# QuentinFuxa/WhisperLiveKit

Hardware: AMD Instinct MI355X
Metric: audio seconds transcribed per second (1/RTF), Whisper-base EN simul_whisper AlignAtt, 0.5 s chunks (higher is better)
Workload: dtype f32; 1 GPU; base.en simul_whisper, 1 stream(s) over 1 GPU(s) (1 per GPU), 30 s 16 kHz speech-like stream, 0.5 s chunks, beam 1, frame_threshold 25, seeded random weights, synthetic vocabulary; model=base.en, streams_total=1

## Files before the change

whisperlivekit_amd/csrc/api.hip:

```cpp
#include <cmath>
#include <cstdio>
#include <cstdlib>
#include <atomic>
#include <chrono>
#include <cstring>
#include <map>
#include <memory>
#include <mutex>
#include <string>
#include <vector>

#include "../../include/wlk_hip.h"
#include "common.h"
#include "internal.h"

namespace wlk {

namespace {
struct UtilStream {
    std::mutex mu;
    hipStream_t stream = nullptr;
};
UtilStream g_util[64];
UtilStream& util_of_current_device() {
// ... 284 lines not shown
        for (int i = 0; i < m->D.n_audio_layer; ++i) m->enc_layers.push_back(layer_weights(m, "enc", i, false));
        for (int i = 0; i < m->D.n_text_layer; ++i) m->dec_layers.push_back(layer_weights(m, "dec", i, true));
        {
            const size_t d = m->D.n_text_state, da = m->D.n_audio_state, Ld = m->D.n_text_layer;
            if (!m->xkv_all_w) m->xkv_all_w = dev_alloc<float>(Ld * 2 * d * da);
            if (!m->xkv_all_b) m->xkv_all_b = dev_alloc<float>(Ld * 2 * d);
            for (size_t i = 0; i < Ld; ++i) {
                copy_sync(m->xkv_all_w + i * 2 * d * da, m->dec_layers[i].xkvw, 2 * d * da * sizeof(float),
                                  hipMemcpyDeviceToDevice);
                copy_sync(m->xkv_all_b + i * 2 * d, m->dec_layers[i].xkvb, 2 * d * sizeof(float),
                                  hipMemcpyDeviceToDevice);
            }
        }
        {
            for (unsigned short* p : m->x3_owned) (void)hipFree(p);
            m->x3_owned.clear();
            m->xkv_all_w3 = nullptr;
            const int da = m->D.n_audio_state, T = m->D.n_audio_ctx;
            LaunchCtx c;
            c.stream = nullptr;
            hipStream_t st;
            WLK_HIP(hipStreamCreateWithFlags(&st, hipStreamNonBlocking));
            struct StreamGuard {
                hipStream_t s;
                ~StreamGuard() { (void)hipStreamDestroy(s); }
            } st_guard{st};
            c.stream = st;
            auto pack = [&](const float* w, int n_rows, int k = 0) -> unsigned short* {
                if (k == 0) k = da;
                unsigned short* p3 = dev_alloc<unsigned short>(x3_w_elems(n_rows, k));
                m->x3_owned.push_back(p3);
                launch_x3_pack_w(c, w, k, p3, n_rows, k);
                return p3;
            };
            static const bool narrow = [] { const char* e = getenv("WLK_X3_NARROW"); return !(e && e[0] == '0'); }();
            for (auto& L : m->enc_layers) {
                L.qkvw3 = gemm_x3_wide_applicable(T, 3 * da, da, da) ? pack(L.qkvw, 3 * da) : nullptr;
                L.fc1w3 = gemm_x3_wide_applicable(T, 4 * da, da, da) ? pack(L.fc1w, 4 * da) : nullptr;
                L.outw3 = narrow && gemm_x3_wide_applicable(T, da, da, da) ? pack(L.outw, da) : nullptr;
                L.fc2w3 = narrow && gemm_x3_wide_applicable(T, da, 4 * da, 4 * da) ? pack(L.fc2w, da, 4 * da) : nullptr;
            }
            const int n_xkv = m->D.n_text_layer * 2 * m->D.n_text_state;
            if (gemm_x3_wide_applicable(T, n_xkv, da, da)) m->xkv_all_w3 = pack(m->xkv_all_w, n_xkv);
            WLK_HIP(hipStreamSynchronize(st));
        }
        m->w_tok_emb = m->w("dec.tok_emb");
        m->w_dec_pos = m->w("dec.pos");
        m->w_ln_w = m->w("dec.ln.w");
        m->w_ln_b = m->w("dec.ln.b");
        m->finalized = true;
        return WLK_OK;
    });
}

int wlk_model_destroy(wlk_model* m) {
    if (!m) return WLK_OK;
    wlk_engine_destroy_for_model(m);
    (void)hipSetDevice(m->device);
    if (m->owns_arena) (void)hipFree(m->arena);
    if (m->xkv_all_w) (void)hipFree(m->xkv_all_w);
    if (m->xkv_all_b) (void)hipFree(m->xkv_all_b);
    for (unsigned short* p : m->x3_owned) (void)hipFree(p);
    (void)hipFree(m->twiddle);
    (void)hipFree(m->filt_lo);
    (void)hipFree(m->filt_hi);
    (void)hipFree(m->head_rank);
    (void)hipFree(m->layer_heads);
    (void)hipFree(m->layer_ranks);
    (void)hipFree(m->all_ranks);
    delete m;
    return WLK_OK;
}

int wlk_session_create(wlk_model* m, int beam, int max_audio_samples, wlk_session** out) {
    if (!m || !out) return fail(WLK_ERR_ARG, "NULL argument");
    if (!m->finalized) return fail(WLK_ERR_STATE, "model not finalized");
    if (beam < 1 || beam > 7) return fail(WLK_ERR_ARG, "beam must be in [1, 7]");
    if (max_audio_samples < kHop) return fail(WLK_ERR_ARG, "max_audio_samples too small");
    return guarded([&]() {
        WLK_HIP(hipSetDevice(m->device));
        auto s = std::make_unique<wlk_session>();
        s->m = m;
        s->beam = beam;
        s->audio_cap = max_audio_samples;
        WLK_HIP(hipStreamCreateWithFlags(&s->stream, hipStreamNonBlocking));
        if (const char* e = std::getenv("WLK_NO_GRAPH")) s->use_graph = !(e[0] == '1');
        hipStream_t st = s->stream;
        const wlk_dims& D = m->D;
        const size_t d = D.n_audio_state, T = D.n_audio_ctx, ctx = D.n_text_ctx, V = D.n_vocab;
        s->audio[0] = dev_alloc_zero<float>(s->audio_cap, st);
        s->audio[1] = dev_alloc_zero<float>(s->audio_cap, st);
        s->frame_cap = s->audio_cap / kHop + 4;
        s->logmel = dev_alloc<float>((size_t)s->frame_cap * D.n_mels);
        s->frame_max = dev_alloc<float>(s->frame_cap);
        s->logmel_alt = dev_alloc<float>((size_t)s->frame_cap * D.n_mels);
        s->frame_max_alt = dev_alloc<float>(s->frame_cap);
        if (const char* e = std::getenv("WLK_MEL_INCREMENTAL")) s->mel_incremental = !(e[0] == '0');
        s->mel_t = dev_alloc_zero<float>((size_t)(kMelFrames + 2) * D.n_mels, st);
        s->x1p = dev_alloc_zero<float>((size_t)(kMelFrames + 1) * d, st);
        s->ex = dev_alloc<float>(T * d);
        s->eh = dev_alloc<float>(T * d);
        s->eqkv = dev_alloc<float>(T * 3 * d);
        s->eatt = dev_alloc<float>(T * d);
        s->emlp = dev_alloc<float>(T * 4 * d);
        s->enc_out = dev_alloc<float>(T * d);
        {
            bool any_x3 = m->xkv_all_w3 != nullptr, qkv_x3 = false;
            bool fc2_x3 = false;
            for (const auto& L : m->enc_layers) {
                any_x3 |= L.qkvw3 || L.fc1w3 || L.outw3;
                qkv_x3 |= L.qkvw3 != nullptr;
                fc2_x3 |= L.fc2w3 != nullptr;
            }
            if (fc2_x3) s->emlp3 = dev_alloc<unsigned short>(T * 3 * 4 * d);
            const bool attn_x3 = qkv_x3 && enc_attention_x3_enabled() && d == (size_t)D.n_audio_head * 64 && T >= 64 && (2 * d) % 128 == 0;
            if (any_x3) s->eh3 = dev_alloc<unsigned short>(T * 3 * d);
            if (attn_x3) s->eqkv3 = dev_alloc_zero<unsigned short>(x3_attn_image_elems((int)T, (int)d), st);
            if (m->xkv_all_w3) s->enc_out3 = dev_alloc<unsigned short>(T * 3 * d);
        }
        s->cross_kv = dev_alloc<float>((size_t)D.n_text_layer * T * 2 * d);

        s->max_rows = beam * (int)ctx;
        const size_t R = s->max_rows;
        s->step_in = dev_alloc<int>(3 * R + 4);
        s->tokens_dev = s->step_in;
        s->dx = dev_alloc<float>(R * d);
        s->dh = dev_alloc<float>(R * d);
        s->dqkv = dev_alloc<float>(R * 3 * d);
        s->datt = dev_alloc<float>(R * d);
        s->dq = dev_alloc<float>(R * d);
        s->dmlp = dev_alloc<float>(R * 4 * d);
        const size_t cache = (size_t)D.n_text_layer * beam * ctx * d;
        s->kcache[0] = dev_alloc<float>(cache);
        s->vcache[0] = dev_alloc<float>(cache);
        s->hsel = dev_alloc<float>((size_t)2 * beam * d);
        s->logits_last = dev_alloc<float>((size_t)2 * beam * V);
        s->logits_sot = s->logits_last + (size_t)beam * V;
        s->ring_row = s->step_in + R;
        s->beam_of_row = s->step_in + 2 * R;
        s->d_offset = s->step_in + 3 * R;
        s->ring_rows = (int)ctx + kAlignWindow;
        if (m->n_align > 0) s->ring = dev_alloc<float>((size_t)m->n_align * beam * s->ring_rows * T);
        s->xsplit = dev_alloc<float>(cross_split_scratch_floats(8, D.n_text_head, (int)T));
        s->fsplit = dev_alloc<float>(flash_split_scratch_floats(s->max_rows, D.n_text_head, wlk_session::kFlashSplitsMax));
        s->z = dev_alloc<float>((size_t)beam * std::max(m->n_align, 1) * T + (size_t)beam * 128);
        s->attn_last = dev_alloc_zero<float>((size_t)beam * T, st);
        s->adj_row = dev_alloc<int>(3 * wlk_session::kAdjCap);
        s->src_rows = dev_alloc<int>(8);
        if (beam >= 2 && beam <= 7) s->anc = dev_alloc_zero<unsigned char>((size_t)beam * ctx, st);
        s->top_vals = dev_alloc<float>((size_t)beam * 18);
        s->top_ids = reinterpret_cast<int*>(s->top_vals) + (size_t)beam * 8;
        s->frames = s->top_ids + (size_t)beam * 8;
        WLK_HIP(hipMalloc(&s->topk_scratch, topk_scratch_bytes(beam)));
        s->probs = dev_alloc<float>(beam);
        WLK_HIP(hipHostMalloc(&s->pinned, wlk_session::kPinnedBytes, hipHostMallocDefault));
        WLK_HIP(hipHostMalloc(&s->dec_stage, 65536, hipHostMallocDefault));
        WLK_HIP(hipHostMalloc(&s->audio_stage, wlk_session::kPinnedBytes, hipHostMallocDefault));
        WLK_HIP(hipEventCreateWithFlags(&s->audio_stage_ev, hipEventDisableTiming));
        WLK_HIP(hipEventCreateWithFlags(&s->dec_stage_ev, hipEventDisableTiming));
        if (beam == 1) {
            void* hp = nullptr;
            WLK_HIP(hipHostMalloc(&hp, 4096, hipHostMallocMapped | hipHostMallocCoherent));
            std::memset(hp, 0, 4096);
            s->step_host = static_cast<StepBlock*>(hp);
            s->result_host = reinterpret_cast<StepResult*>(static_cast<char*>(hp) + 2048);
            void* dp = nullptr;
            WLK_HIP(hipHostGetDevicePointer(&dp, hp, 0));
            s->step_host_dev = static_cast<StepBlock*>(dp);
            s->result_host_dev = reinterpret_cast<StepResult*>(static_cast<char*>(dp) + 2048);
            s->step_dev = reinterpret_cast<StepBlock*>(dev_alloc<int>(sizeof(StepBlock) / 4));
        }
        WLK_HIP(hipStreamSynchronize(st));
        *out = s.release();
        return WLK_OK;
    });
}

int wlk_session_destroy(wlk_session* s) {
    if (!s) return WLK_OK;
    if (s->step_count && getenv("WLK_STEP_TIMING"))
        fprintf(stderr, "[wlk] one-replay steps: %llu, mean %.1f us per step (graph launch call %.1f us)\n",
                (unsigned long long)s->step_count, s->step_ns / 1e3 / s->step_count, s->step_launch_ns / 1e3 / s->step_count);
    (void)wlk_engine_detach(s);
    (void)hipSetDevice(s->m->device);
    (void)hipStreamSynchronize(s->stream);
    float* fl[] = {s->audio[0], s->audio[1], s->logmel, s->frame_max, s->logmel_alt, s->frame_max_alt, s->mel_t, s->x1p, s->ex, s->eh, s->eqkv,
                   s->eatt, s->emlp, s->enc_out, s->cross_kv, s->dx, s->dh, s->dqkv, s->datt, s->dq, s->dmlp,
                   s->kcache[0], s->kcache[1], s->vcache[0], s->vcache[1], s->hsel, s->logits_last,
                   s->ring, s->z, s->attn_last, s->qk_debug, s->xsplit, s->fsplit, s->top_vals, s->probs};
    for (float* p : fl)
        if (p) (void)hipFree(p);
    int* il[] = {s->step_in, s->adj_row, s->src_rows};
    for (int* p : il)
        if (p) (void)hipFree(p);
    for (auto& e : s->step_exec)
        if (e) (void)hipGraphExecDestroy(e);
    for (auto& e : s->bstep_exec)
        if (e) (void)hipGraphExecDestroy(e);
    if (s->anc) (void)hipFree(s->anc);
    if (s->topk_scratch) (void)hipFree(s->topk_scratch);
    if (s->pcm16_dev) (void)hipFree(s->pcm16_dev);
    if (s->eh3) (void)hipFree(s->eh3);
    if (s->eqkv3) (void)hipFree(s->eqkv3);
    if (s->enc_out3) (void)hipFree(s->enc_out3);
    if (s->emlp3) (void)hipFree(s->emlp3);
    if (s->wa_buf) (void)hipFree(s->wa_buf);
    if (s->pinned) (void)hipHostFree(s->pinned);
    if (s->dec_stage) (void)hipHostFree(s->dec_stage);
    if (s->audio_stage) (void)hipHostFree(s->audio_stage);
    if (s->rules_mask) (void)hipFree(s->rules_mask);
    if (s->pick_out) (void)hipFree(s->pick_out);
    if (s->audio_stage_ev) (void)hipEventDestroy(s->audio_stage_ev);
    if (s->dec_stage_ev) (void)hipEventDestroy(s->dec_stage_ev);
    if (s->step_host) (void)hipHostFree(s->step_host);
    if (s->step_dev) (void)hipFree(s->step_dev);
    if (s->step_align_dev) (void)hipFree(s->step_align_dev);
    for (auto& e : s->fstep_exec)
        if (e) (void)hipGraphExecDestroy(e);
    for (auto& r : s->prof.recs) {
        (void)hipEventDestroy(r.a);
        (void)hipEventDestroy(r.b);
    }
    for (auto e : s->prof.pool) (void)hipEventDestroy(e);
    (void)hipStreamDestroy(s->stream);
    delete s;
    return WLK_OK;
}

int wlk_session_set_debug(wlk_session* s, int on) {
    if (!s) return fail(WLK_ERR_ARG, "session is NULL");
    return guarded([&]() {
        WLK_HIP(hipSetDevice(s->m->device));
        s->debug = on != 0;
        if (s->debug && !s->qk_debug) {
            const wlk_dims& D = s->m->D;
            s->qk_debug = dev_alloc<float>((size_t)D.n_text_layer * s->max_rows * D.n_text_head * D.n_audio_ctx);
        }
        return WLK_OK;
    });
}

static bool drain_staging() {
    static const bool on = [] {
        const char* e = getenv("WLK_DRAIN_STAGING");
        return e && e[0] == '1';
    }();
    return on;
}

int wlk_audio_append(wlk_session* s, const float* pcm_host, int n) {
    if (!s || (n > 0 && !pcm_host) || n < 0) return fail(WLK_ERR_ARG, "bad audio chunk");
    if (s->audio_len + n > s->audio_cap)
        return fail(WLK_ERR_CAPACITY, "audio buffer capacity exceeded (" + std::to_string(s->audio_len + n) + " > " +
                                          std::to_string(s->audio_cap) + " samples)");
    if (n == 0) return WLK_OK;
    return guarded([&]() {
        WLK_HIP(hipSetDevice(s->m->device));
        float* dst = s->audio[s->audio_cur] + s->audio_len;
        size_t done = 0;
        while (done < (size_t)n) {
            const size_t chunk = std::min((size_t)n - done, wlk_session::kPinnedBytes / sizeof(float));
            if (s->audio_stage_used) WLK_HIP(hipEventSynchronize(s->audio_stage_ev));
            std::memcpy(s->audio_stage, pcm_host + done, chunk * sizeof(float));
            WLK_HIP(hipMemcpyAsync(dst + done, s->audio_stage, chunk * sizeof(float), hipMemcpyHostToDevice, s->stream));
            WLK_HIP(hipEventRecord(s->audio_stage_ev, s->stream));
            s->audio_stage_used = true;
            done += chunk;
        }
        if (drain_staging()) WLK_HIP(hipStreamSynchronize(s->stream));
        s->audio_len += n;
        s->encoded = false;
        return WLK_OK;
    });
}

int wlk_audio_append_pcm16(wlk_session* s, const int16_t* pcm_host, int n) {
    if (!s || (n > 0 && !pcm_host) || n < 0) return fail(WLK_ERR_ARG, "bad audio chunk");
    if (s->audio_len + n > s->audio_cap)
        return fail(WLK_ERR_CAPACITY, "audio buffer capacity exceeded (" + std::to_string(s->audio_len + n) + " > " +
                                          std::to_string(s->audio_cap) + " samples)");
    if (n == 0) return WLK_OK;
    return guarded([&]() {
        WLK_HIP(hipSetDevice(s->m->device));
        constexpr size_t kMax = wlk_session::kPinnedBytes / sizeof(int16_t);
        if (!s->pcm16_dev) WLK_HIP(hipMalloc(reinterpret_cast<void**>(&s->pcm16_dev), kMax * sizeof(int16_t)));
        float* dst = s->audio[s->audio_cur] + s->audio_len;
        const LaunchCtx c = s->ctx();
        size_t done = 0;
        while (done < (size_t)n) {
            const size_t chunk = std::min((size_t)n - done, kMax);
            if (s->audio_stage_used) WLK_HIP(hipEventSynchronize(s->audio_stage_ev));
            std::memcpy(s->audio_stage, pcm_host + done, chunk * sizeof(int16_t));
            WLK_HIP(hipMemcpyAsync(s->pcm16_dev, s->audio_stage, chunk * sizeof(int16_t), hipMemcpyHostToDevice, s->stream));
            launch_pcm16_to_float(c, s->pcm16_dev, dst + done, (int)chunk);
            WLK_HIP(hipEventRecord(s->audio_stage_ev, s->stream));
            s->audio_stage_used = true;
            done += chunk;
        }
        if (drain_staging()) WLK_HIP(hipStreamSynchronize(s->stream));
        s->audio_len += n;
        s->encoded = false;
        return WLK_OK;
    });
}

int wlk_audio_append_zeros(wlk_session* s, int n) {
    if (!s || n < 0) return fail(WLK_ERR_ARG, "bad zero run");
    if (s->audio_len + n > s->audio_cap) return fail(WLK_ERR_CAPACITY, "audio buffer capacity exceeded");
    if (n == 0) return WLK_OK;
    return guarded([&]() {
        WLK_HIP(hipSetDevice(s->m->device));
        WLK_HIP(hipMemsetAsync(s->audio[s->audio_cur] + s->audio_len, 0, (size_t)n * sizeof(float), s->stream));
        s->audio_len += n;
        s->encoded = false;
        return WLK_OK;
    });
}

int wlk_audio_drop_front(wlk_session* s, int n) {
    if (!s || n < 0 || n > s->audio_len) return fail(WLK_ERR_ARG, "bad eviction length");
    if (n == 0) return WLK_OK;
    return guarded([&]() {
        WLK_HIP(hipSetDevice(s->m->device));
        const int keep = s->audio_len - n;
        if (keep > 0)
            WLK_HIP(hipMemcpyAsync(s->audio[s->audio_cur ^ 1], s->audio[s->audio_cur] + n, (size_t)keep * sizeof(float),
                                   hipMemcpyDeviceToDevice, s->stream));
        s->audio_cur ^= 1;
        s->audio_len = keep;
        s->encoded = false;
        const int shift = n / kHop;
        if (s->mel_incremental && n % kHop == 0 && s->mel_cached_samples > n && shift < s->mel_cached_frames) {
            const int rows = s->mel_cached_frames - shift;
            const int nm = s->m->D.n_mels;
            WLK_HIP(hipMemcpyAsync(s->logmel_alt, s->logmel + (size_t)shift * nm, (size_t)rows * nm * sizeof(float),
// ... 145 lines not shown
                                    [](wlk_session* s) { return reinterpret_cast<float*>(s->eh3); }, none);
    const PtrTable z_eh3_qkv = table([](wlk_session* s) { return reinterpret_cast<const float*>(s->eh3); },
                                     [](wlk_session* s) { return s->eqkv; }, none);
    const PtrTable z_eh3_mlp = table([](wlk_session* s) { return reinterpret_cast<const float*>(s->eh3); },
                                     [](wlk_session* s) { return s->emlp; }, none);
    const PtrTable z_eh3_qkv3 = table([](wlk_session* s) { return reinterpret_cast<const float*>(s->eh3); },
                                      [](wlk_session* s) { return reinterpret_cast<float*>(s->eqkv3); }, none);
    const PtrTable z_qkv3_att = table([](wlk_session* s) { return reinterpret_cast<const float*>(s->eqkv3); },
                                      [](wlk_session* s) { return s->eatt; }, none);
    const PtrTable z_qkv3_eh3 = table([](wlk_session* s) { return reinterpret_cast<const float*>(s->eqkv3); },
                                      [](wlk_session* s) { return reinterpret_cast<float*>(s->eh3); }, none);
    const PtrTable z_eh3_ex_res = table([](wlk_session* s) { return reinterpret_cast<const float*>(s->eh3); }, [](wlk_session* s) { return s->ex; },
                                        [](wlk_session* s) { return (const float*)s->ex; });
    const PtrTable z_eh3_mlp3 = table([](wlk_session* s) { return reinterpret_cast<const float*>(s->eh3); },
                                      [](wlk_session* s) { return reinterpret_cast<float*>(s->emlp3); }, none);
    const PtrTable z_mlp3_ex_res = table([](wlk_session* s) { return reinterpret_cast<const float*>(s->emlp3); }, [](wlk_session* s) { return s->ex; },
                                         [](wlk_session* s) { return (const float*)s->ex; });
    const bool attn_x3 = enc_attention_x3_enabled() && d == D.n_audio_head * 64 && T >= 64 && (2 * d) % 128 == 0;
    auto gemm_x3 = [&](const GemmArgs& g, const unsigned short* w3, const PtrTable& z, const char* tag) {
        X3GemmArgs x;
        x.lda = g.lda; x.W3 = w3; x.bias = g.bias; x.ldc = g.ldc; x.ldr = g.ldr; x.M = g.M; x.N = g.N; x.K = g.K;
        x.flags = g.flags; x.scale = g.scale; x.scale_cols = g.scale_cols; x.scale_period = g.scale_period;
        x.batch = B;
        x.z = z;
        launch_gemm_x3(c, x, tag);
    };
    for (int i = 0; i < D.n_audio_layer; ++i) {
        const LayerW& L = m->enc_layers[i];
        GemmArgs g;
        g.lda = d; g.W = L.qkvw; g.bias = L.qkvb; g.ldc = 3 * d; g.M = T; g.N = 3 * d;
        g.K = d; g.flags = kGemmScaleCols; g.scale = scale; g.scale_cols = 2 * d;
        bool att_is_x3 = false;
        if (L.qkvw3 && attn_x3) {
            launch_layernorm_x3_batched(c, z_ex_eh3, B, d, L.ln1w, L.ln1b, d, T, d, "enc_ln1");
            X3GemmArgs x;
            x.lda = d; x.W3 = L.qkvw3; x.bias = g.bias; x.M = T; x.N = 3 * d; x.K = d; x.flags = g.flags; x.scale = g.scale;
            x.scale_cols = g.scale_cols; x.batch = B; x.z = z_eh3_qkv3;
            x.x3_out = true; x.ldc3 = 2 * d; x.vt_col0 = 2 * d; x.vt_off = x3_attn_vt_off(T, d); x.vt_ld = x3_attn_vt_ld(T);
            launch_gemm_x3(c, x, "enc_qkv_x3");
            att_is_x3 = L.outw3 != nullptr;
            launch_encoder_attention_x3(c, nullptr, 2L * d, x3_attn_vt_off(T, d), x3_attn_vt_ld(T), nullptr, d, T, d, D.n_audio_head,
                                        att_is_x3 ? &z_qkv3_eh3 : &z_qkv3_att, B, att_is_x3);
        } else {
            if (L.qkvw3) {
                launch_layernorm_x3_batched(c, z_ex_eh3, B, d, L.ln1w, L.ln1b, d, T, d, "enc_ln1");
                gemm_x3(g, L.qkvw3, z_eh3_qkv, "enc_qkv_x3");
            } else {
                launch_layernorm_batched(c, z_ex_eh, B, d, L.ln1w, L.ln1b, d, T, d, "enc_ln1");
                gemm(g, z_eh_qkv, "enc_qkv");
            }
            launch_encoder_attention_batched(c, z_qkv_att, B, T, d, D.n_audio_head);
        }
        GemmArgs o;
        o.lda = d; o.W = L.outw; o.bias = L.outb; o.ldc = d; o.M = T; o.N = d; o.K = d;
        o.flags = kGemmResidual; o.ldr = d;
        if (L.outw3) {
            if (!att_is_x3)
                for (int i = 0; i < B; ++i) launch_x3_pack(c, group[i]->eatt, d, group[i]->eh3, d, T, d);
            gemm_x3(o, L.outw3, z_eh3_ex_res, "enc_out_x3");
        } else {
            gemm(o, z_att_ex, "enc_out");
        }
        GemmArgs f1;
        f1.lda = d; f1.W = L.fc1w; f1.bias = L.fc1b; f1.ldc = 4 * d; f1.M = T; f1.N = 4 * d; f1.K = d; f1.flags = kGemmGelu;
        const bool mlp_x3 = L.fc1w3 && L.fc2w3 && (4 * d) % 128 == 0;
        if (mlp_x3) {
            launch_layernorm_x3_batched(c, z_ex_eh3, B, d, L.ln2w, L.ln2b, d, T, d, "enc_ln2");
            X3GemmArgs x;
            x.lda = d; x.W3 = L.fc1w3; x.bias = f1.bias; x.M = T; x.N = 4 * d; x.K = d; x.flags = kGemmGelu; x.batch = B; x.z = z_eh3_mlp3;
            x.x3_out = true; x.ldc3 = 4 * d; x.vt_col0 = 4 * d; x.vt_off = 0; x.vt_ld = (T + 31) / 32 * 32;
            launch_gemm_x3(c, x, "enc_fc1_x3");
        } else if (L.fc1w3) {
            launch_layernorm_x3_batched(c, z_ex_eh3, B, d, L.ln2w, L.ln2b, d, T, d, "enc_ln2");
            gemm_x3(f1, L.fc1w3, z_eh3_mlp, "enc_fc1_x3");
        } else {
            launch_layernorm_batched(c, z_ex_eh, B, d, L.ln2w, L.ln2b, d, T, d, "enc_ln2");
            gemm(f1, z_eh_mlp, "enc_fc1");
        }
        GemmArgs f2;
        f2.lda = 4 * d; f2.W = L.fc2w; f2.bias = L.fc2b; f2.ldc = d; f2.M = T; f2.N = d; f2.K = 4 * d;
        f2.flags = kGemmResidual; f2.ldr = d;
        if (L.fc2w3) {
            if (!mlp_x3)
                for (int i = 0; i < B; ++i) launch_x3_pack(c, group[i]->emlp, 4 * d, group[i]->emlp3, 4 * d, T, 4 * d);
            gemm_x3(f2, L.fc2w3, z_mlp3_ex_res, "enc_fc2_x3");
        } else {
            gemm(f2, z_mlp_ex, "enc_fc2");
        }
    }
    {
        GemmArgs g;
        g.lda = d; g.W = m->xkv_all_w; g.bias = m->xkv_all_b;
        g.ldc = (long)D.n_text_layer * 2 * d; g.M = T; g.N = D.n_text_layer * 2 * d; g.K = d;
        g.flags = kGemmScaleCols; g.scale = scale; g.scale_cols = d; g.scale_period = 2 * d;
        if (m->xkv_all_w3) {
            launch_layernorm_x3_batched(c, table([](wlk_session* s) { return (const float*)s->ex; },
                                                 [](wlk_session* s) { return reinterpret_cast<float*>(s->enc_out3); }, none),
                                        B, d, m->w("enc.ln_post.w"), m->w("enc.ln_post.b"), d, T, d, "enc_ln_post");
            gemm_x3(g, m->xkv_all_w3,
                    table([](wlk_session* s) { return reinterpret_cast<const float*>(s->enc_out3); }, [](wlk_session* s) { return s->cross_kv; }, none),
                    "dec_cross_kv_x3");
        } else {
            launch_layernorm_batched(c, table([](wlk_session* s) { return (const float*)s->ex; }, [](wlk_session* s) { return s->enc_out; }, none),
                                     B, d, m->w("enc.ln_post.w"), m->w("enc.ln_post.b"), d, T, d, "enc_ln_post");
            gemm(g, table([](wlk_session* s) { return (const float*)s->enc_out; }, [](wlk_session* s) { return s->cross_kv; }, none),
                 "dec_cross_kv");
        }
        for (int i = 0; i < B; ++i) group[i]->enc_out_is_x3 = m->xkv_all_w3 != nullptr;
    }
    for (int i = 0; i < B; ++i) {
        wlk_session* s = group[i];
        s->encoded = true;
        s->content_len = content_out[i];
        s->self_len = 0;
        s->n_steps = 0;
    }
}

int wlk_encode(wlk_session* s, int32_t* content_mel_len) {
    if (!s) return fail(WLK_ERR_ARG, "session is NULL");
    return guarded([&]() {
        WLK_HIP(hipSetDevice(s->m->device));
        int content = 0;
        struct Busy {
            wlk_session* s;
            explicit Busy(wlk_session* ss) : s(ss) { wlk_engine_loop_enter(s); }
            ~Busy() { wlk_engine_loop_exit(s); }
        } busy(s);
        if (wlk_engine_batches_encodes(s)) {
            if (int rc = wlk_engine_encode(s, &content)) return rc;
        } else {
            std::vector<int> out;
            wlk_encode_group({s}, s->ctx(), out);
            content = out[0];
        }
        if (content_mel_len) *content_mel_len = content;
        return WLK_OK;
    });
}

int wlk_session::flash_splits() {
    static const int n = [] {
        const char* e = getenv("WLK_FLASH_SPLITS");
        const int v = e ? atoi(e) : 6;
        return v < 1 ? 1 : (v > kFlashSplitsMax ? kFlashSplitsMax : v);
    }();
    return n;
}

constexpr size_t kAncStageOffset = 65536 - 64;

static void enqueue_decode(wlk_session* s, const LaunchCtx& c, int n_rows, int n_tok, bool first, int sot_index,
                           bool step_block = false, const AlignArgs* side_align = nullptr, int side_blocks = 0, int side_zf = 0,
                           bool ancestry = false) {
    wlk_model* m = s->m;
    const wlk_dims& D = m->D;
    const int ctx_len = D.n_text_ctx;
    const int R = n_rows * n_tok;
    const int d = D.n_text_state, T = D.n_audio_ctx, H = D.n_text_head, V = D.n_vocab;
    if (!step_block)
        WLK_HIP(hipMemcpyAsync(s->step_in, s->dec_stage, (size_t)(3 * s->max_rows + 1) * sizeof(int), hipMemcpyHostToDevice,
                               s->stream));
    const bool fused = gemv_applicable(R, d) && n_tok == 1;
    if (ancestry) {
        if (!fused || step_block || !s->anc) throw std::logic_error("decode: the ancestry step needs the fused beam step");
        WLK_HIP(hipMemcpyAsync(s->src_rows, static_cast<char*>(s->dec_stage) + kAncStageOffset, 8 * sizeof(int),
                               hipMemcpyHostToDevice, s->stream));
        launch_anc_update(c, s->anc, s->src_rows, s->d_offset, n_rows, ctx_len);
    }

    if (step_block)
        launch_embed_step(c, s->step_host_dev, s->step_dev, s->tokens_dev, s->ring_row, s->beam_of_row, s->d_offset,
                          m->w_tok_emb, m->w_dec_pos, s->dx, d);
    else
        launch_embed(c, s->tokens_dev, m->w_tok_emb, m->w_dec_pos, s->dx, n_rows, n_tok, s->d_offset, d);
    const float scale = std::pow((float)kHeadDim, -0.25f);
    const size_t cache_layer = (size_t)s->beam * ctx_len * d;
    bool scores_dumped = false;
    for (int i = 0; i < D.n_text_layer; ++i) {
        const LayerW& L = m->dec_layers[i];
        float* kc = s->kcache[s->kv_cur] + i * cache_layer;
        float* vc = s->vcache[s->kv_cur] + i * cache_layer;
        GemmArgs g;
        g.W = L.qkvw; g.bias = L.qkvb; g.C = s->dqkv; g.ldc = 3 * d; g.M = R; g.N = 3 * d;
        g.K = d; g.flags = kGemmScaleCols; g.scale = scale; g.scale_cols = 2 * d; g.lda = d;
        if (fused) {
            g.A = s->dx; g.ln_gamma = L.ln1w; g.ln_beta = L.ln1b;
            g.kcache = kc; g.vcache = vc; g.kv_pos = s->d_offset; g.kv_d = d; g.kv_ctx = ctx_len;
            launch_gemv(c, g, "dec_ln1_qkv_kv");
        } else {
            launch_layernorm(c, s->dx, d, L.ln1w, L.ln1b, s->dh, d, R, d, "dec_ln1");
            g.A = s->dh;
            if (!gemv_applicable(R, d) && gemm_takes_kwave(R, 3 * d, d)) {
                g.kcache = kc; g.vcache = vc; g.kv_pos = s->d_offset; g.kv_d = d; g.kv_ctx = ctx_len; g.kv_ntok = n_tok;
                launch_gemm(c, g, "dec_qkv");
            } else {
                launch_linear(c, g, "dec_qkv");
                launch_kv_append(c, s->dqkv, kc, vc, n_rows, n_tok, s->d_offset, d, ctx_len);
            }
        }
        if (ancestry)
            launch_decoder_self_attention_anc(c, s->dqkv, kc, vc, s->anc, s->datt, n_rows, s->d_offset, d, H, ctx_len);
        else
            launch_decoder_self_attention(c, s->dqkv, kc, vc, s->datt, n_rows, n_tok, s->d_offset, d, H, ctx_len);
        GemmArgs o;
        o.A = s->datt; o.lda = d; o.W = L.outw; o.bias = L.outb; o.C = s->dx; o.ldc = d; o.M = R; o.N = d; o.K = d;
        o.flags = kGemmResidual; o.R = s->dx; o.ldr = d;
        launch_linear(c, o, "dec_out");

        GemmArgs q;
        q.lda = d; q.W = L.xqw; q.bias = L.xqb; q.C = s->dq; q.ldc = d; q.M = R; q.N = d; q.K = d;
        q.flags = kGemmScaleCols; q.scale = scale; q.scale_cols = d;
        const bool fold_xq = fused && R == 1 && !s->debug && !s->align_raw_scores && cross_split_folds_query(d);
        if (fold_xq) {
        } else if (fused) {
            q.A = s->dx; q.ln_gamma = L.lnxw; q.ln_beta = L.lnxb;
            launch_gemv(c, q, "dec_lnx_xq");
        } else {
            launch_layernorm(c, s->dx, d, L.lnxw, L.lnxb, s->dh, d, R, d, "dec_lnx");
            q.A = s->dh;
            launch_linear(c, q, "dec_xq");
        }
        const int* ranks_l = m->n_align > 0 ? m->head_rank + (size_t)i * H : nullptr;
        bool merged_xout = false;
        GemmArgs xo_mg;
        if ((R > 8 || s->align_raw_scores) && !s->debug) {
            if (fold_xq) throw std::logic_error("decode: the folded query projection left no q for the flash kernel");
            FlashArgs fa;
            fa.q = s->dq; fa.ldq = d;
            fa.k = s->cross_kv + (size_t)i * 2 * d; fa.v = fa.k + d; fa.ldkv = (long)D.n_text_layer * 2 * d;
            fa.out = s->datt; fa.ldo = d; fa.Tq = R; fa.Tk = T; fa.n_head = H;
            fa.head_rank = ranks_l; fa.ring = s->ring; fa.ring_row = s->ring_row;
            fa.beam_of_row = s->beam_of_row; fa.ring_rows = s->ring_rows; fa.n_beam = s->beam;
            if (((R + 31) / 32) * H < 256) {
                fa.k_splits = wlk_session::flash_splits();
                fa.part_o = s->fsplit;
                fa.part_m = fa.part_o + (size_t)s->max_rows * H * fa.k_splits * 64;
                fa.part_l = fa.part_m + (size_t)s->max_rows * H * fa.k_splits;
            }
            launch_prefill_cross_attention(c, fa);
            scores_dumped = true;
        } else {
            CrossAttnArgs ca;
            ca.q = s->dq;
            ca.k = s->cross_kv + (size_t)i * 2 * d;
            ca.v = ca.k + d;
            ca.ldkv = (long)D.n_text_layer * 2 * d;
            ca.out = s->datt;
            ca.rows = R; ca.d = d; ca.n_head = H; ca.T = T;
            ca.head_rank = ranks_l;
            ca.ring = s->ring;
            ca.ring_row = s->ring_row;
            ca.beam_of_row = s->beam_of_row;
            ca.ring_rows = s->ring_rows;
            ca.n_beam = s->beam;
            ca.qk_debug = s->debug ? s->qk_debug + (size_t)i * s->max_rows * H * T : nullptr;
            if (fold_xq) {
                ca.xq_x = s->dx; ca.xq_w = L.xqw; ca.xq_b = L.xqb; ca.xq_gamma = L.lnxw; ca.xq_beta = L.lnxb; ca.xq_scale = scale;
            }
            if (R <= 8 && !s->debug) {
                float* sc = s->xsplit;
                float* pm = sc + (size_t)8 * H * T;
                float* pl = pm + (size_t)8 * H * 8;
                float* po = pl + (size_t)8 * H * 8;
                merged_xout = fused && R == 1 && gemv1_folds_merge(d);
                launch_decoder_cross_attention_split(c, ca, sc, pm, pl, po, !merged_xout);
                if (merged_xout) {
                    xo_mg.mg_pm = pm; xo_mg.mg_pl = pl; xo_mg.mg_po = po; xo_mg.mg_scores = sc;
                    xo_mg.mg_head_rank = ranks_l; xo_mg.mg_ring = s->ring; xo_mg.mg_ring_row = s->ring_row;
                    xo_mg.mg_side_heads = m->layer_heads + (size_t)i * H;
                    xo_mg.mg_beam_of_row = s->beam_of_row; xo_mg.mg_heads = H; xo_mg.mg_T = T;
                    xo_mg.mg_ring_rows = s->ring_rows; xo_mg.mg_n_beam = s->beam;
                    xo_mg.mg_side_blocks = ranks_l ? m->layer_rank_count[i] : 0;
                }
            } else {
                launch_decoder_cross_attention(c, ca);
            }
        }
        GemmArgs xo = xo_mg;
        xo.A = s->datt; xo.lda = d; xo.W = L.xoutw; xo.bias = L.xoutb; xo.C = s->dx; xo.ldc = d; xo.M = R; xo.N = d;
        xo.K = d; xo.flags = kGemmResidual; xo.R = s->dx; xo.ldr = d;
        launch_linear(c, xo, "dec_xout");
        transformer_mlp(c, L, s->dx, s->dh, s->dmlp, R, d, "dec_ln2", "dec_fc1", "dec_fc2");
    }
    if (scores_dumped && m->n_align > 0 && !s->align_raw_scores)
        launch_ring_softmax(c, s->ring, s->ring_row, s->beam_of_row, m->all_ranks, m->n_align, R, s->ring_rows, s->beam, T);
    GemmArgs lg;
    lg.lda = d; lg.W = m->w_tok_emb; lg.C = s->logits_last; lg.ldc = V; lg.M = n_rows; lg.N = V; lg.K = d;
    if (side_align && !fused) throw std::logic_error("decode: side workgroups need the fused step");
    if (fused) {
        lg.A = s->dx; lg.ln_gamma = m->w_ln_w; lg.ln_beta = m->w_ln_b;
        lg.side_align = side_align; lg.side_blocks = side_blocks; lg.side_zf = side_zf;
        launch_gemv(c, lg, "dec_lnf_logits");
    } else if (first && n_rows == 1 && gemv_applicable(2, d) && getenv("WLK_NO_PREFILL_MERGE") == nullptr) {
        launch_layernorm(c, s->dx + (size_t)(n_tok - 1) * d, (long)(sot_index - (n_tok - 1)) * d, m->w_ln_w, m->w_ln_b,
                         s->hsel, d, 2, d, "dec_ln_f");
        lg.A = s->hsel; lg.M = 2;
        launch_linear(c, lg, "dec_logits");
        return;
    } else {
        launch_layernorm(c, s->dx + (size_t)(n_tok - 1) * d, (long)n_tok * d, m->w_ln_w, m->w_ln_b, s->hsel, d,
                         n_rows, d, "dec_ln_f");
        lg.A = s->hsel;
        launch_linear(c, lg, "dec_logits");
    }
    if (first) {
        float* hs = s->hsel + (size_t)n_rows * d;
        launch_layernorm(c, s->dx + (size_t)sot_index * d, (long)n_tok * d, m->w_ln_w, m->w_ln_b, hs, d, n_rows, d,
                         "dec_ln_f");
        GemmArgs ls = lg;
        ls.ln_gamma = ls.ln_beta = nullptr;
        ls.A = hs; ls.C = s->logits_sot;
        launch_linear(c, ls, "dec_logits");
    }
}

extern "C++" void wlk_prefill_ws_alloc(const wlk_model* m, wlk_prefill_ws& ws, int max_sessions, int session_rows) {
    const wlk_dims& D = m->D;
    const size_t d = D.n_text_state, V = D.n_vocab, H = D.n_text_head;
    ws.cap_session_rows = session_rows;
    ws.cap_rows = max_sessions * ((session_rows + 31) / 32 * 32);
    const size_t R = ws.cap_rows;
    ws.dx = dev_alloc<float>(R * d);
    ws.dh = dev_alloc<float>(R * d);
    ws.dqkv = dev_alloc<float>(R * 3 * d);
    ws.datt = dev_alloc<float>(R * d);
    ws.dq = dev_alloc<float>(R * d);
    ws.dmlp = dev_alloc<float>(R * 4 * d);
    ws.hsel = dev_alloc<float>((size_t)2 * max_sessions * d);
    ws.logits = dev_alloc<float>((size_t)8 * V);
    ws.part = dev_alloc<float>(flash_split_scratch_floats((int)R, (int)H, wlk_session::kFlashSplitsMax));
    ws.rows_dev = reinterpret_cast<StepRow*>(dev_alloc<char>(R * sizeof(StepRow)));
    ws.tiles_dev = reinterpret_cast<StepRow*>(dev_alloc<char>(R / 32 * sizeof(StepRow)));
    ws.ring_row_dev = dev_alloc<int>(R);
    ws.zeros_dev = dev_alloc<int>(R);
    memset_sync(ws.zeros_dev, 0, R * sizeof(int));
    ws.pinned_bytes = R * sizeof(StepRow) + R / 32 * sizeof(StepRow) + R * sizeof(int);
    WLK_HIP(hipHostMalloc(reinterpret_cast<void**>(&ws.pinned), ws.pinned_bytes, hipHostMallocDefault));
}

extern "C++" void wlk_prefill_ws_free(wlk_prefill_ws& ws) {
    void* dev[] = {ws.dx, ws.dh, ws.dqkv, ws.datt, ws.dq, ws.dmlp, ws.hsel, ws.logits, ws.part, ws.rows_dev, ws.tiles_dev,
                   ws.ring_row_dev, ws.zeros_dev};
    for (void* p : dev)
        if (p) (void)hipFree(p);
    if (ws.pinned) (void)hipHostFree(ws.pinned);
    ws = wlk_prefill_ws{};
}

extern "C++" std::string wlk_prefill_precheck(const wlk_prefill_item& it, const wlk_prefill_ws& ws) {
    const wlk_session* s = it.s;
    if (!s || !it.tokens) return "prefill: NULL argument";
    const wlk_dims& D = s->m->D;
    const int P = it.n_tok, d = D.n_text_state;
    if (!s->encoded) return "wlk_decode before wlk_encode";
    if (s->beam != 1 || s->debug || s->prof_on || s->align_raw_scores) return "not a plain beam-1 session";
    if (it.sot_index < 0 || it.sot_index >= P) return "sot_index out of range";
    if (P > D.n_text_ctx) return "text context exceeded";
    for (int i = 0; i < P; ++i)
        if (it.tokens[i] < 0 || it.tokens[i] >= D.n_vocab) return "token id out of range";
    if (P <= 8 || P > ws.cap_session_rows) return "prompt length outside the stacked range";
    if (!gemm_takes_kwave(P, 3 * d, d) || !gemm_takes_kwave(P, d, d) || !gemm_takes_kwave(P, 4 * d, d) ||
        !gemm_takes_kwave(P, d, 4 * d))
        return "prompt too long for the k-wave GEMMs";
    if (((P + 31) / 32) * D.n_text_head >= 256) return "prompt too long for the key-split cross-attention";
    if (!gemv_applicable(8, d)) return "model too wide for the stacked vocabulary projection";
    return std::string();
}

extern "C++" void wlk_prefill_group(const std::vector<wlk_prefill_item*>& items, const LaunchCtx& c, wlk_prefill_ws& ws) {
    if (items.empty()) return;
    wlk_model* m = items[0]->s->m;
    const wlk_dims& D = m->D;
    const int d = D.n_text_state, T = D.n_audio_ctx, H = D.n_text_head, V = D.n_vocab, L = D.n_text_layer;
    const int B = (int)items.size();
    StepRow* rows_h = reinterpret_cast<StepRow*>(ws.pinned);
    std::vector<int> row0(B), padded(B);
    int R = 0;
    for (int i = 0; i < B; ++i) {
        row0[i] = R;
        padded[i] = (items[i]->n_tok + 31) / 32 * 32;
        R += padded[i];
    }
    if (R > ws.cap_rows) throw std::length_error("stacked prefill: more rows than the workspace holds");
    StepRow* tiles_h = rows_h + R;
    int* ring_row_h = reinterpret_cast<int*>(tiles_h + R / 32);
    for (int i = 0; i < B; ++i) {
        wlk_session* s = items[i]->s;
        for (int p = 0; p < padded[i]; ++p) {
            const int src = p < items[i]->n_tok ? p : 0;
            StepRow r{};
            r.kcache = s->kcache[s->kv_cur];
            r.vcache = s->vcache[s->kv_cur];
            r.cross_kv = s->cross_kv;
            r.ring = s->ring;
            r.token = (int)items[i]->tokens[src];
            r.offset = src;
            r.ring_row = src;
            rows_h[row0[i] + p] = r;
            ring_row_h[row0[i] + p] = src;
            if (p % 32 == 0) tiles_h[(row0[i] + p) / 32] = r;
        }
    }
    WLK_HIP(hipMemcpyAsync(ws.rows_dev, rows_h, (size_t)R * sizeof(StepRow), hipMemcpyHostToDevice, c.stream));
    WLK_HIP(hipMemcpyAsync(ws.tiles_dev, tiles_h, (size_t)(R / 32) * sizeof(StepRow), hipMemcpyHostToDevice, c.stream));
    WLK_HIP(hipMemcpyAsync(ws.ring_row_dev, ring_row_h, (size_t)R * sizeof(int), hipMemcpyHostToDevice, c.stream));

    launch_embed_rows(c, ws.rows_dev, m->w_tok_emb, m->w_dec_pos, ws.dx, R, d);
    const float scale = std::pow((float)kHeadDim, -0.25f);
    const size_t cache_layer = (size_t)D.n_text_ctx * d;
    auto linear = [&](const float* A, long lda, const float* W, const float* bias, float* C, long ldc, int N, int K, int flags,
                      const float* Rs, float sc, int sc_cols, const char* tag) {
        GemmArgs g;
        g.A = A; g.lda = lda; g.W = W; g.bias = bias; g.C = C; g.ldc = ldc; g.M = R; g.N = N; g.K = K;
        g.flags = flags; g.R = Rs; g.ldr = ldc; g.scale = sc; g.scale_cols = sc_cols;
        g.force_kwave = true;
        launch_gemm(c, g, tag);
    };
    auto ln_linear = [&](const float* gamma, const float* beta, const float* W, const float* bias, float* C, long ldc, int N,
                         int flags, float sc, int sc_cols, const char* t_ln, const char* tag) {
        launch_layernorm(c, ws.dx, d, gamma, beta, ws.dh, d, R, d, t_ln);
        linear(ws.dh, d, W, bias, C, ldc, N, d, flags, nullptr, sc, sc_cols, tag);
    };
    for (int i = 0; i < L; ++i) {
        const LayerW& W = m->dec_layers[i];
        ln_linear(W.ln1w, W.ln1b, W.qkvw, W.qkvb, ws.dqkv, 3 * d, 3 * d, kGemmScaleCols, scale, 2 * d, "dec_ln1", "dec_qkv");
        launch_kv_append_rows(c, ws.dqkv, ws.rows_dev, (long)(i * cache_layer), R, d);
        launch_decoder_self_attention_rows(c, ws.dqkv, ws.rows_dev, (long)(i * cache_layer), ws.datt, R, d, H, D.n_text_ctx);
        linear(ws.datt, d, W.outw, W.outb, ws.dx, d, d, d, kGemmResidual, ws.dx, 1.f, 0, "dec_out");
        ln_linear(W.lnxw, W.lnxb, W.xqw, W.xqb, ws.dq, d, d, kGemmScaleCols, scale, d, "dec_lnx", "dec_xq");
        FlashArgs fa;
        fa.q = ws.dq; fa.ldq = d;
        fa.k = nullptr; fa.v = nullptr; fa.ldkv = (long)L * 2 * d;
        fa.tile_rows = ws.tiles_dev; fa.tile_kv_off = (long)i * 2 * d; fa.tile_v_off = d;
        fa.out = ws.datt; fa.ldo = d; fa.Tq = R; fa.Tk = T; fa.n_head = H;
        fa.head_rank = m->n_align > 0 ? m->head_rank + (size_t)i * H : nullptr;
        fa.ring = nullptr; fa.ring_row = ws.ring_row_dev; fa.beam_of_row = ws.zeros_dev;
        fa.ring_rows = items[0]->s->ring_rows; fa.n_beam = 1;
        fa.k_splits = wlk_session::flash_splits();
        fa.part_o = ws.part;
        fa.part_m = fa.part_o + (size_t)R * H * fa.k_splits * 64;
        fa.part_l = fa.part_m + (size_t)R * H * fa.k_splits;
        launch_prefill_cross_attention(c, fa);
        linear(ws.datt, d, W.xoutw, W.xoutb, ws.dx, d, d, d, kGemmResidual, ws.dx, 1.f, 0, "dec_xout");
        ln_linear(W.ln2w, W.ln2b, W.fc1w, W.fc1b, ws.dmlp, 4 * d, 4 * d, kGemmGelu, 1.f, 0, "dec_ln2", "dec_fc1");
        linear(ws.dmlp, 4 * d, W.fc2w, W.fc2b, ws.dx, d, d, 4 * d, kGemmResidual, ws.dx, 1.f, 0, "dec_fc2");
// ... 108 lines not shown
        std::memcpy(probs_host, s->pinned, s->beam * sizeof(float));
        return WLK_OK;
    });
}

int wlk_rules_set(wlk_session* s, const int32_t* suppressed, int n_suppressed, const int32_t* blank, int n_blank) {
    if (!s || n_suppressed < 0 || n_blank < 0 || (n_suppressed > 0 && !suppressed) || (n_blank > 0 && !blank))
        return fail(WLK_ERR_ARG, "invalid rule lists");
    const int V = s->m->D.n_vocab;
    for (int i = 0; i < n_suppressed; ++i)
        if (suppressed[i] < 0 || suppressed[i] >= V) return fail(WLK_ERR_ARG, "suppressed token out of range");
    for (int i = 0; i < n_blank; ++i)
        if (blank[i] < 0 || blank[i] >= V) return fail(WLK_ERR_ARG, "blank token out of range");
    return guarded([&]() {
        WLK_HIP(hipSetDevice(s->m->device));
        std::vector<unsigned char> host((size_t)V, 0);
        for (int i = 0; i < n_suppressed; ++i) host[(size_t)suppressed[i]] |= 1;
        for (int i = 0; i < n_blank; ++i) host[(size_t)blank[i]] |= 2;
        if (!s->rules_mask) {
            s->rules_mask = dev_alloc<unsigned char>((size_t)V);
            s->pick_out = dev_alloc<int>(2 + 2 * kMaxPickRows * 8);
        }
        WLK_HIP(hipStreamSynchronize(s->stream));
        copy_sync(s->rules_mask, host.data(), host.size(), hipMemcpyHostToDevice);
        return WLK_OK;
    });
}

int wlk_pick_greedy(wlk_session* s, const wlk_pick_params* p, int32_t* token_host, float* logprob_host) {
    if (!s || !p || !token_host || !logprob_host) return fail(WLK_ERR_ARG, "NULL argument");
    if (s->beam != 1) return fail(WLK_ERR_ARG, "wlk_pick_greedy serves sessions of one row");
    if (s->n_steps == 0) return fail(WLK_ERR_STATE, "wlk_pick_greedy before wlk_decode");
    if (!s->rules_mask) return fail(WLK_ERR_STATE, "wlk_pick_greedy before wlk_rules_set");
    const int V = s->m->D.n_vocab;
    if (p->timestamp_begin < 0 || p->timestamp_begin > V || p->eot < 0 || p->eot >= V || p->ts_mode < 0 || p->ts_mode > 2)
        return fail(WLK_ERR_ARG, "rule parameters out of range");
    return guarded([&]() {
        WLK_HIP(hipSetDevice(s->m->device));
        const LaunchCtx c = s->ctx();
        const PickRules r{p->first_step, p->without_timestamps, p->timestamp_begin, p->eot, p->no_timestamps, p->ts_mode,
                          p->ts_bound, p->max_initial};
        launch_rules_pick(c, s->logits_last, V, s->rules_mask, r, s->pick_out, reinterpret_cast<float*>(s->pick_out + 1));
        WLK_HIP(hipMemcpyAsync(s->pinned, s->pick_out, 8, hipMemcpyDeviceToHost, s->stream));
        WLK_HIP(hipStreamSynchronize(s->stream));
        std::memcpy(token_host, s->pinned, 4);
        std::memcpy(logprob_host, static_cast<char*>(s->pinned) + 4, 4);
        return WLK_OK;
    });
}

int wlk_pick_topk(wlk_session* s, const wlk_pick_params* p, int n_rows, int k, float* logprobs_host, int32_t* ids_host) {
    if (!s || !p || !logprobs_host || !ids_host) return fail(WLK_ERR_ARG, "NULL argument");
    if (n_rows < 1 || n_rows > kMaxPickRows || n_rows != s->beam) return fail(WLK_ERR_ARG, "wlk_pick_topk: n_rows must be the session's beam, 1..8");
    if (k < 1 || k > 8) return fail(WLK_ERR_ARG, "k must be in [1, 8]");
    if (s->n_steps == 0) return fail(WLK_ERR_STATE, "wlk_pick_topk before wlk_decode");
    if (!s->rules_mask) return fail(WLK_ERR_STATE, "wlk_pick_topk before wlk_rules_set");
    const int V = s->m->D.n_vocab;
    PickRulesRows rules{};
    for (int b = 0; b < n_rows; ++b) {
        const wlk_pick_params& q = p[b];
        if (q.timestamp_begin < 0 || q.timestamp_begin > V || q.eot < 0 || q.eot >= V || q.ts_mode < 0 || q.ts_mode > 2)
            return fail(WLK_ERR_ARG, "rule parameters out of range");
        rules.r[b] = PickRules{q.first_step, q.without_timestamps, q.timestamp_begin, q.eot, q.no_timestamps, q.ts_mode, q.ts_bound,
                               q.max_initial};
    }
    return guarded([&]() {
        WLK_HIP(hipSetDevice(s->m->device));
        const LaunchCtx c = s->ctx();
        const size_t n = (size_t)n_rows * k;
        float* lp_dev = reinterpret_cast<float*>(s->pick_out + 2);
        int* ids_dev = s->pick_out + 2 + n;
        launch_rules_topk(c, s->logits_last, V, n_rows, s->rules_mask, rules, k, lp_dev, ids_dev);
        WLK_HIP(hipMemcpyAsync(s->pinned, lp_dev, 2 * n * 4, hipMemcpyDeviceToHost, s->stream));
        WLK_HIP(hipStreamSynchronize(s->stream));
        std::memcpy(logprobs_host, s->pinned, n * 4);
        std::memcpy(ids_host, static_cast<char*>(s->pinned) + n * 4, n * 4);
        return WLK_OK;
    });
}

static int select_impl(wlk_session* s, const int32_t* adj_row, const int32_t* adj_ids, const float* adj_deltas, int n_adj,
                       int k, int content_mel_len, float* top_logprobs_host, int32_t* top_ids_host, int32_t* frames_host,
                       int no_speech_token, float* no_speech_host) {
    if (!s || !top_logprobs_host || !top_ids_host || !frames_host) return fail(WLK_ERR_ARG, "NULL argument");
    if (s->n_steps == 0) return fail(WLK_ERR_STATE, "wlk_select before wlk_decode");
    if (n_adj < 0 || n_adj > wlk_session::kAdjCap) return fail(WLK_ERR_ARG, "too many logit adjustments");
    if (n_adj > 0 && (!adj_row || !adj_ids || !adj_deltas)) return fail(WLK_ERR_ARG, "NULL adjustment arrays");
    if (k < 1 || k > 8) return fail(WLK_ERR_ARG, "k must be in [1, 8]");
    if (content_mel_len < 0) return fail(WLK_ERR_ARG, "content_mel_len out of range");
    if (content_mel_len > s->m->D.n_audio_ctx) content_mel_len = s->m->D.n_audio_ctx;
    return guarded([&]() {
        wlk_model* m = s->m;
        const wlk_dims& D = m->D;
        WLK_HIP(hipSetDevice(m->device));
        const LaunchCtx c = s->ctx();
        const int B = s->beam, V = D.n_vocab;
        int* adj_rows_d = s->adj_row;
        int* adj_ids_d = s->adj_row + n_adj;
        float* adj_deltas_d = reinterpret_cast<float*>(s->adj_row + 2 * n_adj);
        if (n_adj > 0) {
            char* st = static_cast<char*>(s->pinned) + 131072;
            std::memcpy(st, adj_row, n_adj * sizeof(int));
            std::memcpy(st + n_adj * 4, adj_ids, n_adj * sizeof(int));
            std::memcpy(st + n_adj * 8, adj_deltas, n_adj * sizeof(float));
            WLK_HIP(hipMemcpyAsync(s->adj_row, st, (size_t)n_adj * 12, hipMemcpyHostToDevice, s->stream));
        }
        AlignArgs a;
        a.ring = s->ring; a.n_align = m->n_align; a.n_beam = B; a.ring_rows = s->ring_rows; a.T = D.n_audio_ctx;
        a.prefill_rows = s->n_steps <= kAlignWindow ? s->prefill_rows : 0;
        a.n_single = std::min(s->n_steps - 1, kAlignWindow);
        a.single_base = D.n_text_ctx;
        a.newest_row = s->n_steps == 1 ? s->prefill_rows - 1 : D.n_text_ctx + ((s->n_steps - 2) % kAlignWindow);
        a.content_len = content_mel_len;
        a.z = s->z; a.attn_last = s->attn_last; a.frames = s->frames;
        float* ns_dev = s->top_vals + (size_t)B * 17;
        if (!launch_select_fused(c, s->logits_last, V, B, k, s->top_vals, s->top_ids, s->topk_scratch, adj_rows_d,
                                 adj_ids_d, adj_deltas_d, n_adj, a, StepHostOut{}, no_speech_host ? s->logits_sot : nullptr,
                                 no_speech_token, ns_dev)) {
            if (no_speech_host) launch_token_prob(c, s->logits_sot, V, B, no_speech_token, ns_dev);
            launch_logsoftmax_topk(c, s->logits_last, V, B, k, s->top_vals, s->top_ids, s->topk_scratch, adj_rows_d,
                                   adj_ids_d, adj_deltas_d, n_adj);
            launch_alignatt(c, a);
        }

        char* out = static_cast<char*>(s->pinned) + 65536;
        WLK_HIP(hipMemcpyAsync(out, s->top_vals, (size_t)B * (no_speech_host ? 18 : 17) * 4, hipMemcpyDeviceToHost, s->stream));
        WLK_HIP(hipStreamSynchronize(s->stream));
        if (no_speech_host) std::memcpy(no_speech_host, out + (size_t)B * 68, B * sizeof(float));
        for (int b = 0; b < B; ++b) {
            std::memcpy(top_logprobs_host + (size_t)b * k, out + (size_t)b * k * 4, k * sizeof(float));
            std::memcpy(top_ids_host + (size_t)b * k, out + (size_t)B * 32 + (size_t)b * k * 4, k * sizeof(int));
        }
        std::memcpy(frames_host, out + (size_t)B * 64, B * sizeof(int));
        return WLK_OK;
    });
}

int wlk_select(wlk_session* s, const int32_t* adj_row, const int32_t* adj_ids, const float* adj_deltas, int n_adj, int k,
               int content_mel_len, float* top_logprobs_host, int32_t* top_ids_host, int32_t* frames_host) {
    return select_impl(s, adj_row, adj_ids, adj_deltas, n_adj, k, content_mel_len, top_logprobs_host, top_ids_host,
                       frames_host, -1, nullptr);
}

extern "C++" int wlk_select_first(wlk_session* s, int no_speech_token, const int32_t* adj_row, const int32_t* adj_ids,
                                  const float* adj_deltas, int n_adj, int k, int content_mel_len, float* no_speech_host,
                                  float* top_logprobs_host, int32_t* top_ids_host, int32_t* frames_host) {
    if (!s || !no_speech_host) return fail(WLK_ERR_ARG, "NULL argument");
    if (!s->have_sot) return fail(WLK_ERR_STATE, "no sot-row logits: call after the first decode of an infer");
    if (no_speech_token < 0 || no_speech_token >= s->m->D.n_vocab) return fail(WLK_ERR_ARG, "token out of range");
    return select_impl(s, adj_row, adj_ids, adj_deltas, n_adj, k, content_mel_len, top_logprobs_host, top_ids_host,
                       frames_host, no_speech_token, no_speech_host);
}

extern "C++" int wlk_step_select(wlk_session* s, int64_t token, const int32_t* adj_ids, const float* adj_deltas, int n_adj,
                                 int content_mel_len, float* top_logprobs2, int32_t* top_ids2, int32_t* frame) {
    static const bool enabled = [] {
        const char* e = getenv("WLK_FUSED_STEP");
        return !(e && e[0] == '0');
    }();
    wlk_model* m = s->m;
    const wlk_dims& D = m->D;
    if (!enabled || s->beam != 1 || !s->step_host || s->debug || s->prof_on || !s->use_graph || s->n_steps < 1 ||
        n_adj > kStepMaxAdj || !gemv_applicable(1, D.n_text_state) || !s->encoded)
        return 1;
    AlignArgs a;
    a.ring = nullptr; a.n_align = m->n_align; a.n_beam = 1; a.ring_rows = s->ring_rows; a.T = D.n_audio_ctx;
    a.prefill_rows = 0; a.n_single = 0; a.newest_row = 0; a.single_base = D.n_text_ctx; a.content_len = 0;
    a.z = s->z; a.attn_last = s->attn_last; a.frames = s->frames;
    if (!select_fused_applicable(1, 2, a)) return 1;
    if (token < 0 || token >= D.n_vocab) return fail(WLK_ERR_ARG, "token id out of range");
    if (s->self_len + 1 > D.n_text_ctx) return fail(WLK_ERR_CAPACITY, "text context exceeded");
    if (content_mel_len < 0) return fail(WLK_ERR_ARG, "content_mel_len out of range");
    if (content_mel_len > D.n_audio_ctx) content_mel_len = D.n_audio_ctx;
    return guarded([&]() {
        WLK_HIP(hipSetDevice(m->device));
        const LaunchCtx c = s->ctx();
        StepBlock& b = *s->step_host;
        b.row = next_step_row(s, (int)token, content_mel_len);
        b.n_adj = n_adj;
        for (int i = 0; i < n_adj; ++i) {
            b.adj_row[i] = -1;
            b.adj_ids[i] = adj_ids[i];
            b.adj_deltas[i] = adj_deltas[i];
        }
        const unsigned seq = ++s->step_seq ? s->step_seq : ++s->step_seq;
        b.seq = seq;
        std::atomic_thread_fence(std::memory_order_release);

        const auto t_enter = std::chrono::steady_clock::now();
        hipGraphExec_t& exec = s->fstep_exec[s->kv_cur];
        if (!exec) {
            const int zf_blocks = (a.T + 63) / 64;
            if (!s->step_align_dev) {
                AlignArgs ad = a;
                ad.rows = &s->step_dev->row;
                s->step_align_dev = reinterpret_cast<AlignArgs*>(dev_alloc<char>(sizeof(AlignArgs)));
                WLK_HIP(hipMemcpyAsync(s->step_align_dev, &ad, sizeof(AlignArgs), hipMemcpyHostToDevice, s->stream));
            }
            WLK_HIP(hipStreamSynchronize(s->stream));
            capture_step_graph(s->stream, exec, [&] {
                a.rows = &s->step_dev->row;
                a.part = s->z + (size_t)s->beam * std::max(m->n_align, 1) * D.n_audio_ctx;
                const bool early_z = select_early_z_enabled() && D.n_vocab >= 16384;
                if (early_z) enqueue_decode(s, c, 1, 1, false, 0, true, s->step_align_dev, zf_blocks * a.n_align * a.n_beam, zf_blocks);
                else enqueue_decode(s, c, 1, 1, false, 0, true);
                StepHostOut ho;
                ho.result = s->result_host_dev;
                ho.n_adj = &s->step_dev->n_adj;
                ho.seq = &s->step_dev->seq;
                if (!launch_select_fused(c, s->logits_last, D.n_vocab, 1, 2, s->top_vals, s->top_ids, s->topk_scratch,
                                         s->step_dev->adj_row, s->step_dev->adj_ids, s->step_dev->adj_deltas, 0, a, ho, nullptr, 0,
                                         nullptr, early_z))
                    throw std::runtime_error("fused step: read-out not available");
            });
        }
        WLK_HIP(hipGraphLaunch(exec, s->stream));

        volatile StepResult* r = s->result_host;
        const auto t_start = std::chrono::steady_clock::now();
        s->step_launch_ns += (uint64_t)std::chrono::duration_cast<std::chrono::nanoseconds>(t_start - t_enter).count();
        try {
            wlk_wait_step_flags(s->stream, s->result_host, 1, seq);
        } catch (...) {
            s->encoded = false;
            s->n_steps = 0;
            s->self_len = 0;
            throw;
        }
        s->have_sot = false;
        s->self_len += 1;
        s->n_steps += 1;
        s->last_rows = 1;
        s->last_ntok = 1;
        s->step_ns += (uint64_t)std::chrono::duration_cast<std::chrono::nanoseconds>(std::chrono::steady_clock::now() - t_enter).count();
        s->step_count += 1;
        top_logprobs2[0] = r->top_vals[0]; top_logprobs2[1] = r->top_vals[1];
        top_ids2[0] = r->top_ids[0]; top_ids2[1] = r->top_ids[1];
        *frame = r->frame;
        return WLK_OK;
    });
}

int wlk_kv_reorder(wlk_session* s, const int32_t* source_rows, int n_rows) {
    if (!s || !source_rows || n_rows != s->beam) return fail(WLK_ERR_ARG, "bad reorder request");
    if (s->anc_live)
        return fail(WLK_ERR_STATE, "wlk_kv_reorder after an ancestry beam step: the cache rows are not the hypotheses");
    bool identity = true;
    for (int i = 0; i < n_rows; ++i) {
        if (source_rows[i] < 0 || source_rows[i] >= n_rows) return fail(WLK_ERR_ARG, "source row out of range");
        identity &= source_rows[i] == i;
    }
    if (identity || s->self_len == 0) return WLK_OK;
    return guarded([&]() {
        const wlk_dims& D = s->m->D;
        WLK_HIP(hipSetDevice(s->m->device));
        const LaunchCtx c = s->ctx();
        const size_t cache = (size_t)D.n_text_layer * s->beam * D.n_text_ctx * D.n_text_state;
        if (!s->kcache[1]) {
            s->kcache[1] = dev_alloc<float>(cache);
            s->vcache[1] = dev_alloc<float>(cache);
        }
        WLK_HIP(hipStreamSynchronize(s->stream));
        std::memcpy(s->pinned, source_rows, n_rows * sizeof(int));
        WLK_HIP(hipMemcpyAsync(s->src_rows, s->pinned, n_rows * sizeof(int), hipMemcpyHostToDevice, s->stream));
        const int cur = s->kv_cur;
        launch_kv_gather(c, s->kcache[cur], s->kcache[cur ^ 1], s->src_rows, n_rows, s->self_len, D.n_text_state,
                         D.n_text_ctx, D.n_text_layer);
        launch_kv_gather(c, s->vcache[cur], s->vcache[cur ^ 1], s->src_rows, n_rows, s->self_len, D.n_text_state,
                         D.n_text_ctx, D.n_text_layer);
        s->kv_cur ^= 1;
        return WLK_OK;
    });
}

extern "C++" int wlk_beam_step(wlk_session* s, const int64_t* tokens, const int32_t* source_rows) {
    if (!s || !tokens || !source_rows) return fail(WLK_ERR_ARG, "NULL argument");
    wlk_model* m = s->m;
    const wlk_dims& D = m->D;
    const int B = s->beam;
    if (!s->anc || B < 2 || B > 7 || s->debug || s->prof_on || !s->use_graph || s->n_steps < 1 || !s->encoded ||
        !gemv_applicable(B, D.n_text_state) || D.n_text_ctx > 512 || D.n_text_state != D.n_text_head * kHeadDim ||
        (size_t)(s->max_rows * 3 + 4) * sizeof(int) > kAncStageOffset)
        return 1;
    if (s->self_len + 1 > D.n_text_ctx) return fail(WLK_ERR_CAPACITY, "text context exceeded");
    for (int b = 0; b < B; ++b) {
        if (tokens[b] < 0 || tokens[b] >= D.n_vocab) return fail(WLK_ERR_ARG, "token id out of range");
        if (source_rows[b] < 0 || source_rows[b] >= B) return fail(WLK_ERR_ARG, "source row out of range");
    }
    return guarded([&]() {
        WLK_HIP(hipSetDevice(m->device));
        const LaunchCtx c = s->ctx();
        if (s->dec_stage_used) WLK_HIP(hipEventSynchronize(s->dec_stage_ev));
        if (drain_staging()) WLK_HIP(hipStreamSynchronize(s->stream));
        int* stage = static_cast<int*>(s->dec_stage);
        const int MR = s->max_rows;
        const int slot_row = D.n_text_ctx + ((s->n_steps - 1) % kAlignWindow);
        for (int b = 0; b < B; ++b) {
            stage[b] = (int)tokens[b];
            stage[MR + b] = slot_row;
            stage[2 * MR + b] = b;
        }
        stage[3 * MR] = s->self_len;
        int* ctl = reinterpret_cast<int*>(static_cast<char*>(s->dec_stage) + kAncStageOffset);
        for (int b = 0; b < 7; ++b) ctl[b] = b < B ? source_rows[b] : 0;
        ctl[7] = s->anc_live ? 0 : 1;
        hipGraphExec_t& exec = s->bstep_exec[s->kv_cur];
        if (!exec) capture_step_graph(s->stream, exec, [&] { enqueue_decode(s, c, B, 1, false, 0, false, nullptr, 0, 0, true); });
        WLK_HIP(hipGraphLaunch(exec, s->stream));
        WLK_HIP(hipEventRecord(s->dec_stage_ev, s->stream));
        s->dec_stage_used = true;
        s->have_sot = false;
        s->anc_live = true;
        s->anc_steps += 1;
        s->self_len += 1;
        s->n_steps += 1;
        s->last_rows = B;
        s->last_ntok = 1;
        return WLK_OK;
    });
}

int wlk_diag_beam_step(wlk_session* s, const int64_t* tokens, const int32_t* source_rows, int n_rows) {
    if (!s || n_rows != s->beam) return fail(WLK_ERR_ARG, "n_rows must equal the session's beam size");
    const int rc = wlk_beam_step(s, tokens, source_rows);
    return rc == 1 ? fail(WLK_ERR_STATE, "the session does not qualify for the ancestry step") : rc;
}

int wlk_decode_ancestry(wlk_session* s, const int64_t* tokens, const int32_t* source_rows, int n_rows) {
    if (!s || !tokens || !source_rows) return fail(WLK_ERR_ARG, "NULL argument");
    if (n_rows != s->beam) return fail(WLK_ERR_ARG, "n_rows must equal the session's beam size");
    if (!s->encoded) return fail(WLK_ERR_STATE, "wlk_decode_ancestry before wlk_encode");
    if (s->n_steps == 0) return fail(WLK_ERR_STATE, "wlk_decode_ancestry before the prefill (wlk_decode with first=1)");
    const int rc = wlk_beam_step(s, tokens, source_rows);
    if (rc != 1) return rc;
    if (s->anc_live) return fail(WLK_ERR_STATE, "wlk_decode_ancestry: the session stopped qualifying for the ancestry step inside an infer");
    if (int rc2 = wlk_kv_reorder(s, source_rows, n_rows)) return rc2;
    return wlk_decode(s, tokens, n_rows, 1, 0, 0);
}

int wlk_session_beam_stats(wlk_session* s, uint64_t* ancestry_steps) {
    if (!s || !ancestry_steps) return fail(WLK_ERR_ARG, "NULL argument");
    *ancestry_steps = s->anc_steps;
    return WLK_OK;
}

int wlk_sync(wlk_session* s) {
    if (!s) return fail(WLK_ERR_ARG, "session is NULL");
    return guarded([&]() {
        WLK_HIP(hipSetDevice(s->m->device));
        WLK_HIP(hipStreamSynchronize(s->stream));
        return WLK_OK;
// ... 222 lines not shown
```

whisperlivekit_amd/csrc/common.h:

```cpp
#pragma once
#include <hip/hip_runtime.h>

#include <cstdint>
#include <stdexcept>
#include <mutex>
#include <string>

namespace wlk {

constexpr int kNFft = 400;
constexpr int kHop = 160;
constexpr int kNFreq = 201;
constexpr int kMelFrames = 3000;
constexpr int kPadSamples = 480000;
constexpr int kHeadDim = 64;
constexpr int kAlignWindow = 16;

struct HipError : std::runtime_error {
    using std::runtime_error::runtime_error;
};

inline void hip_check(hipError_t e, const char* what, const char* file, int line) {
    if (e != hipSuccess) {
        throw HipError(std::string(what) + " failed: " + hipGetErrorString(e) + " (" + file + ":" +
                       std::to_string(line) + ")");
    }
}
#define WLK_HIP(expr) ::wlk::hip_check((expr), #expr, __FILE__, __LINE__)

void set_last_error(const std::string& msg);

struct Profiler;
void copy_sync(void* dst, const void* src, size_t bytes, hipMemcpyKind kind);
void memset_sync(void* dst, int value, size_t bytes);

struct LaunchCtx {
    hipStream_t stream = nullptr;
    Profiler* prof = nullptr;
};
void prof_before(const LaunchCtx& ctx, const char* name, double flops, double bytes);
void prof_after(const LaunchCtx& ctx);

struct KernelScope {
    const LaunchCtx& ctx;
    KernelScope(const LaunchCtx& c, const char* name, double flops = 0.0, double bytes = 0.0) : ctx(c) {
        if (ctx.prof) prof_before(ctx, name, flops, bytes);
    }
    ~KernelScope() {
        if (ctx.prof) prof_after(ctx);
    }
};

template <typename F>
void capture_step_graph(hipStream_t stream, hipGraphExec_t& exec, F&& enqueue) {
    if (exec) throw std::logic_error("capture_step_graph: the executable graph is already recorded");
    hipGraph_t graph = nullptr;
    WLK_HIP(hipStreamBeginCapture(stream, hipStreamCaptureModeThreadLocal));
    try {
        enqueue();
    } catch (...) {
        (void)hipStreamEndCapture(stream, &graph);
        if (graph) (void)hipGraphDestroy(graph);
        throw;
    }
    hipError_t e = hipStreamEndCapture(stream, &graph);
    if (e == hipSuccess) e = hipGraphInstantiate(&exec, graph, nullptr, nullptr, 0);
    if (graph) (void)hipGraphDestroy(graph);
    if (e != hipSuccess) exec = nullptr;
    hip_check(e, "recording a step graph", __FILE__, __LINE__);
}

struct StepRow {
    float* kcache;
    float* vcache;
    const float* cross_kv;
    float* ring;
    int token;
    int offset;
    int ring_row;
    int prefill_rows, n_single, newest_row, content_len;
    int pad;
};

constexpr int kStepMaxAdj = 160;
struct StepBlock {
    StepRow row;
    int n_adj;
    unsigned seq;
    int pad[2];
    int adj_row[kStepMaxAdj];
    int adj_ids[kStepMaxAdj];
    float adj_deltas[kStepMaxAdj];
};
struct StepResult {
    float top_vals[2];
    int top_ids[2];
    int frame;
    unsigned flag_topk, flag_align;
    int pad;
};
struct StepHostOut {
    StepResult* result = nullptr;
    const int* n_adj = nullptr;
    const unsigned* seq = nullptr;
};
constexpr int kEngineFusedAdj = 1024;
struct EngineBlock {
    int n_adj;
    unsigned seq;
    int pad[2];
    StepRow rows[8];
    int adj_row[kEngineFusedAdj];
    int adj_ids[kEngineFusedAdj];
    float adj_deltas[kEngineFusedAdj];
};
void launch_embed_rows_step(const LaunchCtx& ctx, const EngineBlock* host_block, EngineBlock* dev_block, const float* tok_emb,
                            const float* pos_emb, float* x, int n_rows, int d);
void launch_embed_step(const LaunchCtx& ctx, const StepBlock* host_block, StepBlock* dev_block, int* tokens_dev,
                       int* ring_row, int* beam_of_row, int* d_offset, const float* tok_emb, const float* pos_emb, float* x,
                       int d);

constexpr int kMaxBatch = 8;
struct PtrTable {
    const float* in[kMaxBatch];
    float* out[kMaxBatch];
    const float* res[kMaxBatch];
};
template <typename T>
__device__ __forceinline__ T table_at(T const (&t)[kMaxBatch], unsigned z) {
    T v = t[0];
#pragma unroll
    for (int i = 1; i < kMaxBatch; ++i) v = (z == (unsigned)i) ? t[i] : v;
    return v;
}

enum GemmFlags : int {
    kGemmGelu = 1,
    kGemmResidual = 2,
    kGemmScaleCols = 4,
    kGemmRelu = 8,
    kGemmSwish = 16,
};
struct AlignArgs;
struct GemmArgs {
    const float* A = nullptr;
    long lda = 0;
    const float* W = nullptr;
    const float* bias = nullptr;
    float* C = nullptr;
    long ldc = 0;
    const float* R = nullptr;
    long ldr = 0;
    int M = 0, N = 0, K = 0;
    int flags = 0;
    float scale = 1.f;
    int scale_cols = 0;
    int scale_period = 0;
    int batch = 0;
    long long* dbg_clock = nullptr;
    const float* ln_gamma = nullptr;
    const float* ln_beta = nullptr;
    float* kcache = nullptr;
    float* vcache = nullptr;
    const int* kv_pos = nullptr;
    int kv_d = 0, kv_ctx = 0;
    int kv_ntok = 1;
    const StepRow* kv_rows = nullptr;
    long kv_layer_off = 0;
    const float* mg_pm = nullptr;
    const float* mg_pl = nullptr;
    const float* mg_po = nullptr;
    const float* mg_scores = nullptr;
    const int* mg_head_rank = nullptr;
    const int* mg_side_heads = nullptr;
    float* mg_ring = nullptr;
    const int* mg_ring_row = nullptr;
    const int* mg_beam_of_row = nullptr;
    int mg_heads = 0, mg_T = 0, mg_ring_rows = 0, mg_n_beam = 1, mg_side_blocks = 0;
    PtrTable z;
    const AlignArgs* side_align = nullptr;
    int side_blocks = 0, side_zf = 0;
    bool force_kwave = false;
    int force_kernel = 0;
    bool gemm_plain_loop = false;
};
#define WLK_PIN_S(x) asm volatile("" ::"s"(x))
#define WLK_PIN_GEMM_ARGS(g)                                                                                                \
    do {                                                                                                                    \
        asm volatile("" ::"s"((g).A), "s"((g).lda), "s"((g).W), "s"((g).bias), "s"((g).C), "s"((g).ldc), "s"((g).R),        \
                     "s"((g).ldr), "s"((g).M), "s"((g).N), "s"((g).K), "s"((g).flags), "s"((g).scale), "s"((g).scale_cols), \
                     "s"((g).scale_period), "s"((g).batch), "s"((g).dbg_clock));                                            \
        __builtin_amdgcn_sched_barrier(0);     \
    } while (0)
void launch_gemm(const LaunchCtx& ctx, const GemmArgs& g, const char* tag);
void launch_gemm_kp(const LaunchCtx& ctx, const GemmArgs& g, const char* tag);
bool gemm_kp_takes_kpipe(int M, int N, int K);
bool gemm_takes_kwave(int M, int N, int K);
bool gemm_takes_ksplit(int M, int N, int K);
void launch_gemv(const LaunchCtx& ctx, const GemmArgs& g, const char* tag);
inline int gemv_row_bucket(int M) { return M <= 1 ? 1 : M <= 2 ? 2 : M <= 4 ? 4 : 8; }
inline bool gemv_applicable(int M, int K) {
    return M <= 8 && (long)gemv_row_bucket(M) * K * 4 <= 64 * 1024 && K % 4 == 0;
}
bool gemv1_folds_merge(int K);
void refresh_env_switches();
inline void launch_linear(const LaunchCtx& ctx, const GemmArgs& g, const char* tag) {
    if (gemv_applicable(g.M, g.K)) launch_gemv(ctx, g, tag);
    else launch_gemm(ctx, g, tag);
}

struct X3GemmArgs {
    const unsigned short* A3 = nullptr;
    long lda = 0;
    const unsigned short* W3 = nullptr;
    const float* bias = nullptr;
    float* C = nullptr;
    long ldc = 0;
    const float* R = nullptr;
    long ldr = 0;
    int M = 0, N = 0, K = 0;
    int flags = 0;
    float scale = 1.f;
    int scale_cols = 0;
    int scale_period = 0;
    int batch = 0;
    int walk_banded = 0;
    int walk_colmajor = 0;
    int walk_slots = 0;
    unsigned short* C3 = nullptr;
    long ldc3 = 0;
    int vt_col0 = 0;
    long vt_off = 0;
    long vt_ld = 0;
    bool x3_out = false;
    PtrTable z;
};
bool gemm_x3_wide_applicable(int M, int N, int K, long lda);
void launch_gemm_x3(const LaunchCtx& ctx, const X3GemmArgs& g, const char* tag);
size_t x3_w_elems(int n, int k);
void launch_x3_pack_w(const LaunchCtx& ctx, const float* src, long ld_src, unsigned short* dst, int n, int k);
void launch_x3_pack(const LaunchCtx& ctx, const float* src, long ld_src, unsigned short* dst, long ld_dst, int rows, int cols);
void launch_x3_unpack(const LaunchCtx& ctx, const unsigned short* src, long ld_src, float* dst, long ld_dst, int rows, int cols);

inline long x3_attn_vt_ld(int T) { return ((long)T + 31) / 32 * 32; }
inline long x3_attn_vt_off(int T, int d) { return (long)T * 3 * 2 * d; }
inline size_t x3_attn_image_elems(int T, int d) { return (size_t)x3_attn_vt_off(T, d) + (size_t)d * 3 * x3_attn_vt_ld(T); }
bool enc_attention_x3_enabled();
void launch_encoder_attention_x3(const LaunchCtx& ctx, const unsigned short* qk3, long ldqk, long vt_off, long vt_ld, float* out,
                                 long ldo, int T, int d, int n_head, const PtrTable* z, int batch, bool x3_out = false);
void launch_x3_pack_qkv(const LaunchCtx& ctx, const float* qkv, unsigned short* out, int T, int d, long vt_off, long vt_ld);

void launch_layernorm(const LaunchCtx& ctx, const float* x, long ldx, const float* gamma, const float* beta,
                      float* y, long ldy, int rows, int d, const char* tag);
void launch_layernorm_batched(const LaunchCtx& ctx, const PtrTable& z, int batch, long ldx, const float* gamma,
                              const float* beta, long ldy, int rows, int d, const char* tag);
void launch_layernorm_x3(const LaunchCtx& ctx, const float* x, long ldx, const float* gamma, const float* beta,
                         unsigned short* y3, long ldy3, int rows, int d, const char* tag);
void launch_layernorm_x3_batched(const LaunchCtx& ctx, const PtrTable& z, int batch, long ldx, const float* gamma,
                                 const float* beta, long ldy3, int rows, int d, const char* tag);

struct MelArgs {
    const float* audio;
    int n_samples;
    const float* window;
    const double* twiddle;
    const float* filters;
    const int* filt_lo;
    const int* filt_hi;
    int n_mels;
    float* logmel;
    float* frame_max;
    float* mel_t;
    int n_active;
// ... 69 lines not shown
void launch_embed(const LaunchCtx& ctx, const int* tokens, const float* tok_emb, const float* pos_emb,
                  float* x, int n_rows, int n_tok, const int* offset_dev, int d);
void launch_embed_rows(const LaunchCtx& ctx, const StepRow* rows, const float* tok_emb, const float* pos_emb, float* x,
                       int n_rows, int d);
void launch_decoder_self_attention_rows(const LaunchCtx& ctx, const float* qkv, const StepRow* rows, long layer_off,
                                        float* out, int n_rows, int d, int n_head, int ctx_len);
void launch_kv_append(const LaunchCtx& ctx, const float* qkv, float* kc, float* vc, int n_rows, int n_tok,
                      const int* offset_dev, int d, int ctx_len);
void launch_kv_append_rows(const LaunchCtx& ctx, const float* qkv, const StepRow* rows, long layer_off, int n_rows, int d);
void launch_decoder_self_attention_anc(const LaunchCtx& ctx, const float* qkv, const float* kc, const float* vc,
                                       const unsigned char* anc, float* out, int n_rows, const int* offset, int d,
                                       int n_head, int ctx_len);
void launch_anc_update(const LaunchCtx& ctx, unsigned char* anc, const int* ctl, const int* offset, int n_rows, int ctx_len);
void launch_anc_update_block(const LaunchCtx& ctx, unsigned char* anc, const int* block, int n_rows, int ctx_len);
void launch_decoder_self_attention(const LaunchCtx& ctx, const float* qkv, const float* kc, const float* vc,
                                   float* out, int n_rows, int n_tok, const int* offset_dev, int d, int n_head,
                                   int ctx_len);
struct CrossAttnArgs {
    const float* q;
    const float* k;
    const float* v;
    long ldkv;
    float* out;
    int rows, d, n_head, T;
    const int* head_rank;
    float* ring;
    const int* ring_row;
    const int* beam_of_row;
    int ring_rows, n_beam;
    float* qk_debug;
    const StepRow* step_rows = nullptr;
    long kv_off = 0;
    const float* xq_x = nullptr;
    const float* xq_w = nullptr;
    const float* xq_b = nullptr;
    const float* xq_gamma = nullptr;
    const float* xq_beta = nullptr;
    float xq_scale = 1.f;
};
void launch_decoder_cross_attention(const LaunchCtx& ctx, const CrossAttnArgs& a);
bool cross_split_folds_query(int d);
void launch_decoder_cross_attention_split(const LaunchCtx& ctx, const CrossAttnArgs& a, float* scores, float* pm,
                                          float* pl, float* po, bool merge = true);
constexpr int kCrossSplitWays = 8;
size_t cross_split_scratch_floats(int rows, int n_head, int T);
void launch_kv_gather(const LaunchCtx& ctx, const float* src, float* dst, const int* source_rows, int n_rows,
                      int len, int d, int ctx_len, int n_layer);

inline int sf_sub_len(int n) { return (n - 1) / 2 + 1; }
void launch_sf_scale_copy(const LaunchCtx& ctx, const float* src, float* dst, long n, float scale);
constexpr int kSfMaxSegments = 8;
struct SfSegments {
    int n = 0;
    int start[kSfMaxSegments] = {0}, len[kSfMaxSegments] = {0};
};
struct SfConvSegs {
    int n = 0, in_total = 0, out_total = 0;
    int in_start[kSfMaxSegments] = {0}, in_len[kSfMaxSegments] = {0}, out_start[kSfMaxSegments] = {0};
};
SfConvSegs sf_conv_segs_next(const SfConvSegs& prev);
void launch_sf_conv0(const LaunchCtx& ctx, const float* in, const float* w, const float* b, float* out, const SfConvSegs& sg, int F,
                     int C);
void launch_sf_dwconv2d(const LaunchCtx& ctx, const float* in, const float* w, const float* b, float* out, const SfConvSegs& sg,
                        int Fi, int C);
void launch_sf_assemble(const LaunchCtx& ctx, const float* ctx_rows, const float* chunk_rows, float* x, const SfSegments& rows,
                        const SfSegments& chunks, int d, float scale);
struct SfAttnArgs {
    const float* q = nullptr; const float* k = nullptr; const float* v = nullptr;
    long ldq = 0, ldk = 0, ldv = 0;
    float* out = nullptr; long ldo = 0;
    int T = 0, n_head = 0, dh = 0;
    float scale = 1.f;
    const float* pos = nullptr; long ldp = 0; int pos_row0 = 0;
    const float* bias_u = nullptr; const float* bias_v = nullptr;
    int n_seg = 0;
    int seg_start[kSfMaxSegments] = {0}, seg_T[kSfMaxSegments] = {0};
};
constexpr int kSfMaxFrames = 512;
void launch_sf_attention(const LaunchCtx& ctx, const SfAttnArgs& a);
void launch_sf_glu_dwconv(const LaunchCtx& ctx, const float* in, const float* w, const float* b, const float* bn_mean,
                          const float* bn_invstd, const float* bn_w, const float* bn_b, float* out, const SfSegments& rows, int d,
                          int taps);
void launch_sf_head(const LaunchCtx& ctx, const float* x, const float* w1t, const float* b1, const float* w2,
                    const float* b2, float* out, int T, int d, int n_spk);
void launch_sf_transpose(const LaunchCtx& ctx, const float* src, float* dst, int rows, int cols);

constexpr int kSfStateMaxKeys = 4096;
constexpr int kSfStateMaxRows = 1024;
struct SfStateParams {
    int S = 0, F = 0, sil_per_spk = 0, max_index = 0, d = 0, n_spk = 0;
    int strong_k = 0, weak_k = 0, min_pos = 0;
    float thr = 0.f, boost_latest = 0.f, sil_thr = 0.f, log_half = 0.f, strong_boost = 0.f, weak_boost = 0.f;
};
struct SfStateJob {
    SfStateParams p;
    const float* chunk = nullptr;
    const float* preds = nullptr;
    const float *cache_in = nullptr, *cache_p_in = nullptr, *fifo_in = nullptr, *mean_in = nullptr;
    const int* lens_in = nullptr;
    float *cache_out = nullptr, *cache_p_out = nullptr, *fifo_out = nullptr, *fifo_p_out = nullptr, *mean_out = nullptr;
    int* lens_out = nullptr;
    float *up = nullptr, *up_p = nullptr;
    int s_len = 0, f_len = 0, lc = 0, chunk_len = 0, pop = 0, N = 0, compress = 0;
};
struct SfStateBatch {
    int n = 0;
    SfStateJob job[kSfMaxSegments];
};
void launch_sf_state_update(const LaunchCtx& ctx, const SfStateBatch& b);
void launch_sf_state_compress(const LaunchCtx& ctx, const SfStateBatch& b);

void launch_logsoftmax_topk(const LaunchCtx& ctx, float* logits, int n_vocab, int n_rows, int k,
                            float* top_vals, int* top_ids, void* scratch, const int* adj_row, const int* adj_ids,
                            const float* adj_deltas, int n_adj);
size_t topk_scratch_bytes(int n_rows);
void launch_logsoftmax_topk_wide(const LaunchCtx& ctx, const float* logits, int n_vocab, int n_rows, int k, float* top_vals,
                                 int* top_ids, void* scratch);
size_t topk_wide_scratch_bytes(int n_rows);
constexpr int kTopkWideMaxK = 16;
constexpr int kTopkWideMaxVocab = 64 * 4096;
inline bool topk_wide_applicable(int n_vocab, int k) { return n_vocab >= 1 && n_vocab <= kTopkWideMaxVocab && k >= 1 && k <= kTopkWideMaxK; }
void launch_token_prob(const LaunchCtx& ctx, const float* logits, int n_vocab, int n_rows, int token, float* probs);
struct PickRules {
    int first_step, without_timestamps, timestamp_begin, eot, no_timestamps, ts_mode, ts_bound, max_initial;
};
void launch_rules_pick(const LaunchCtx& ctx, const float* logits, int n_vocab, const unsigned char* mask, const PickRules& p,
                       int* out_token, float* out_logprob);
constexpr int kMaxPickRows = 8;
struct PickRulesRows {
    PickRules r[kMaxPickRows];
};
void launch_rules_topk(const LaunchCtx& ctx, const float* logits, int n_vocab, int n_rows, const unsigned char* mask,
                       const PickRulesRows& rules, int k, float* out_lp, int* out_ids);
struct AlignArgs {
    const float* ring;
    int n_align, n_beam, ring_rows, T;
    int prefill_rows;
    int n_single;
    int newest_row;
    int single_base;
    int content_len;
    float* z;
    float* attn_last;
    int* frames;
    const StepRow* rows = nullptr;
    float* part = nullptr;
};
void launch_alignatt(const LaunchCtx& ctx, const AlignArgs& a);
void launch_align_zscore(const LaunchCtx& ctx, const AlignArgs& a);
void launch_align_argmax_plain(const LaunchCtx& ctx, const AlignArgs& a);
bool launch_select_fused(const LaunchCtx& ctx, float* logits, int n_vocab, int n_rows, int k, float* top_vals, int* top_ids,
                         void* scratch, const int* adj_row, const int* adj_ids, const float* adj_deltas, int n_adj,
                         const AlignArgs& a, const StepHostOut& host = StepHostOut{}, const float* ns_logits = nullptr,
                         int ns_token = 0, float* ns_probs = nullptr, bool early_z = false);
bool select_early_z_enabled();
bool select_fused_applicable(int n_rows, int k, const AlignArgs& a);
void launch_alignatt_rows(const LaunchCtx& ctx, const AlignArgs& a, const StepRow* rows);

}
```

whisperlivekit_amd/csrc/internal.h:

```cpp
#pragma once
#include <algorithm>
#include <map>
#include <memory>
#include <chrono>
#include <cstdlib>
#include <thread>
#include <mutex>
#include <stdexcept>
#include <string>
#include <vector>

#include "../../include/wlk_hip.h"
#include "common.h"

namespace wlk {

const std::string& get_last_error();

template <typename F>
inline int guarded(F&& f) {
    try {
        return f();
    } catch (const HipError& e) {
        set_last_error(e.what());
// ... 47 lines not shown
struct LayerW {
    const float *ln1w, *ln1b, *qkvw, *qkvb, *outw, *outb, *ln2w, *ln2b, *fc1w, *fc1b, *fc2w, *fc2b;
    const float *lnxw = nullptr, *lnxb = nullptr, *xqw = nullptr, *xqb = nullptr, *xkvw = nullptr, *xkvb = nullptr,
                *xoutw = nullptr, *xoutb = nullptr;
    const unsigned short *qkvw3 = nullptr, *fc1w3 = nullptr;
    const unsigned short *outw3 = nullptr, *fc2w3 = nullptr;
};

template <typename T>
inline T* dev_alloc(size_t n) {
    T* p = nullptr;
    WLK_HIP(hipMalloc(reinterpret_cast<void**>(&p), n * sizeof(T)));
    return p;
}
template <typename T>
inline T* dev_alloc_zero(size_t n, hipStream_t s) {
    T* p = dev_alloc<T>(n);
    WLK_HIP(hipMemsetAsync(p, 0, n * sizeof(T), s));
    return p;
}

}

struct wlk_engine;
struct wlk_session;
struct wlk_model;

struct wlk_prefill_ws {
    int cap_rows = 0;
    int cap_session_rows = 0;
    float *dx = nullptr, *dh = nullptr, *dqkv = nullptr, *datt = nullptr, *dq = nullptr, *dmlp = nullptr, *hsel = nullptr,
          *logits = nullptr, *part = nullptr;
    wlk::StepRow *rows_dev = nullptr, *tiles_dev = nullptr;
    int *ring_row_dev = nullptr, *zeros_dev = nullptr;
    char* pinned = nullptr;
    size_t pinned_bytes = 0;
};
struct wlk_prefill_item {
    wlk_session* s = nullptr;
    const int64_t* tokens = nullptr;
    int n_tok = 0, sot_index = 0;
    int rc = 0;
    std::string err;
};

struct wlk_model {
    wlk_dims D{};
    int device = 0;
    float* arena = nullptr;
    bool owns_arena = false;
    uint64_t arena_floats = 0;
    std::vector<wlk::TensorSlot> slots;
    std::map<std::string, const wlk::TensorSlot*> by_name;
    double* twiddle = nullptr;
    float* xkv_all_w = nullptr;
    float* xkv_all_b = nullptr;
    unsigned short* xkv_all_w3 = nullptr;
    std::vector<unsigned short*> x3_owned;
    int* filt_lo = nullptr;
    int* filt_hi = nullptr;
    int* head_rank = nullptr;
    int* layer_ranks = nullptr;
    int* layer_heads = nullptr;
    int* all_ranks = nullptr;
    std::vector<int> layer_rank_count;
    std::vector<int> align_pairs;
    int n_align = 0;
    bool finalized = false;
    std::vector<wlk::LayerW> enc_layers, dec_layers;
    const float *w_tok_emb = nullptr, *w_dec_pos = nullptr, *w_ln_w = nullptr, *w_ln_b = nullptr;
    wlk_engine* engine = nullptr;
    std::mutex engine_mu;

    const float* w(const std::string& name) const {
        auto it = by_name.find(name);
        if (it == by_name.end()) throw std::invalid_argument("unknown tensor " + name);
        return arena + it->second->offset;
    }
};


struct wlk_session {
    wlk_model* m = nullptr;
    int beam = 1;
    int audio_cap = 0;
    hipStream_t stream = nullptr;
    wlk::Profiler prof;
    bool prof_on = false;
    bool debug = false;
    bool use_graph = true;
    hipGraphExec_t step_exec[2] = {nullptr, nullptr};
    short* pcm16_dev = nullptr;

    float* audio[2] = {nullptr, nullptr};
    int audio_cur = 0;
    int audio_len = 0;

    float *logmel = nullptr, *frame_max = nullptr, *mel_t = nullptr;
    float *logmel_alt = nullptr, *frame_max_alt = nullptr;
    int mel_cached_samples = 0, mel_cached_frames = 0, mel_dirty_head = 0;
    bool mel_incremental = true;
    int frame_cap = 0;
    float *x1p = nullptr, *ex = nullptr, *eh = nullptr, *eqkv = nullptr, *eatt = nullptr, *emlp = nullptr,
          *enc_out = nullptr, *cross_kv = nullptr;
    unsigned short *eh3 = nullptr, *enc_out3 = nullptr;
    unsigned short* emlp3 = nullptr;
    bool enc_out_is_x3 = false;
    unsigned short* eqkv3 = nullptr;
    bool encoded = false;
    int content_len = 0;

    int max_rows = 0;
    int* tokens_dev = nullptr;
    float *dx = nullptr, *dh = nullptr, *dqkv = nullptr, *datt = nullptr, *dq = nullptr, *dmlp = nullptr;
    float* kcache[2] = {nullptr, nullptr};
    float* vcache[2] = {nullptr, nullptr};
    int kv_cur = 0;
    int self_len = 0;
    int n_steps = 0;
    int prefill_rows = 0;
    int last_rows = 0, last_ntok = 0;
    float *hsel = nullptr, *logits_last = nullptr, *logits_sot = nullptr;
    bool have_sot = false;
    int* step_in = nullptr;
    int *ring_row = nullptr, *beam_of_row = nullptr, *d_offset = nullptr;
    float* ring = nullptr;
    int ring_rows = 0;
    float *z = nullptr, *attn_last = nullptr;
    float* qk_debug = nullptr;
    float* xsplit = nullptr;
    float* fsplit = nullptr;
    static constexpr int kFlashSplitsMax = 16;
    static int flash_splits();

    int *adj_row = nullptr, *src_rows = nullptr;
    float* top_vals = nullptr;
    void* topk_scratch = nullptr;
    int *top_ids = nullptr, *frames = nullptr;
    float* probs = nullptr;
    static constexpr int kAdjCap = 4096;
    void* pinned = nullptr;
    static constexpr size_t kPinnedBytes = 1 << 20;
    void* dec_stage = nullptr;
    hipEvent_t dec_stage_ev = nullptr;
    bool dec_stage_used = false;
    void* audio_stage = nullptr;
    hipEvent_t audio_stage_ev = nullptr;
    unsigned char* rules_mask = nullptr;
    int* pick_out = nullptr;
    bool audio_stage_used = false;
    wlk::StepBlock *step_host = nullptr, *step_host_dev = nullptr, *step_dev = nullptr;
    wlk::StepResult *result_host = nullptr, *result_host_dev = nullptr;
    hipGraphExec_t fstep_exec[2] = {nullptr, nullptr};
    wlk::AlignArgs* step_align_dev = nullptr;
    unsigned step_seq = 0;
    uint64_t step_ns = 0, step_launch_ns = 0, step_count = 0;

    unsigned char* anc = nullptr;
    hipGraphExec_t bstep_exec[2] = {nullptr, nullptr};
    bool anc_live = false;
    uint64_t anc_steps = 0;

    wlk::LaunchCtx ctx() { return wlk::LaunchCtx{stream, prof_on ? &prof : nullptr}; }
    bool align_raw_scores = false;
    float* wa_buf = nullptr;
    size_t wa_cap = 0;
    wlk_engine* engine = nullptr;
};


inline wlk::StepRow next_step_row(const wlk_session* s, int token, int content_len) {
    const int ctx_len = s->m->D.n_text_ctx;
    const int after = s->n_steps + 1;
    wlk::StepRow r;
    r.kcache = s->kcache[s->kv_cur];
    r.vcache = s->vcache[s->kv_cur];
    r.cross_kv = s->cross_kv;
    r.ring = s->ring;
    r.token = token;
    r.offset = s->self_len;
    r.ring_row = ctx_len + ((s->n_steps - 1) % wlk::kAlignWindow);
    r.prefill_rows = after <= wlk::kAlignWindow ? s->prefill_rows : 0;
    r.n_single = std::min(after - 1, wlk::kAlignWindow);
    r.newest_row = ctx_len + ((after - 2) % wlk::kAlignWindow);
    r.content_len = content_len;
    r.pad = 0;
    return r;
}

inline void wlk_wait_step_flags(hipStream_t stream, const wlk::StepResult* res, int n, unsigned seq) {
    static const long spin_us = [] {
        const char* e = getenv("WLK_STEP_SPIN_US");
        return e ? atol(e) : 400L;
    }();
    const auto t_start = std::chrono::steady_clock::now();
    auto all_set = [&]() {
        for (int i = 0; i < n; ++i)
            if (__atomic_load_n(&res[i].flag_topk, __ATOMIC_ACQUIRE) != seq || __atomic_load_n(&res[i].flag_align, __ATOMIC_ACQUIRE) != seq)
                return false;
        return true;
    };
    bool spinning = true;
    for (unsigned looks = 0;; ++looks) {
        if (all_set()) return;
        if ((looks & 0x3ff) == 0x3ff) {
            const hipError_t q = hipStreamQuery(stream);
            if (q == hipSuccess) {
                if (all_set()) return;
                throw std::runtime_error("graph step: the replay finished without delivering its result");
            }
            if (q != hipErrorNotReady) WLK_HIP(q);
        }
        if (spinning) {
            __builtin_ia32_pause();
            if ((looks & 0x3f) == 0x3f &&
                std::chrono::steady_clock::now() - t_start > std::chrono::microseconds(spin_us))
                spinning = false;
            continue;
        }
        const auto waited = std::chrono::steady_clock::now() - t_start;
        if (waited > std::chrono::seconds(30)) throw std::runtime_error("graph step: no result after 30 s");
        if (waited > std::chrono::milliseconds(2)) std::this_thread::sleep_for(std::chrono::microseconds(50));
        else std::this_thread::yield();
    }
}

int wlk_step_select(wlk_session* s, int64_t token, const int32_t* adj_ids, const float* adj_deltas, int n_adj,
                    int content_mel_len, float* top_logprobs2, int32_t* top_ids2, int32_t* frame);
int wlk_beam_step(wlk_session* s, const int64_t* tokens, const int32_t* source_rows);
int wlk_select_first(wlk_session* s, int no_speech_token, const int32_t* adj_row, const int32_t* adj_ids,
                     const float* adj_deltas, int n_adj, int k, int content_mel_len, float* no_speech_host,
                     float* top_logprobs_host, int32_t* top_ids_host, int32_t* frames_host);
void wlk_encode_group(const std::vector<wlk_session*>& group, const wlk::LaunchCtx& c, std::vector<int>& content_out,
                      bool mel_given = false);
std::string wlk_encode_precheck(const wlk_session* s, const wlk_model* m);

std::string wlk_prefill_precheck(const wlk_prefill_item& it, const wlk_prefill_ws& ws);
void wlk_prefill_group(const std::vector<wlk_prefill_item*>& items, const wlk::LaunchCtx& c, wlk_prefill_ws& ws);
void wlk_prefill_ws_alloc(const wlk_model* m, wlk_prefill_ws& ws, int max_sessions, int session_rows);
void wlk_prefill_ws_free(wlk_prefill_ws& ws);

int wlk_engine_prefill(wlk_session* s, const int64_t* tokens, int n_tok, int sot_index);
bool wlk_engine_batches_encodes(const wlk_session* s);
int wlk_engine_encode(wlk_session* s, int* content_mel_len);
namespace wlk { struct DecodeJob; }
void wlk_engine_destroy_for_model(wlk_model* m);
bool wlk_engine_wants(const wlk_session* s);
void wlk_engine_loop_enter(wlk_session* s);
void wlk_engine_loop_exit(wlk_session* s);
int wlk_engine_run_job(wlk_session* s, wlk::DecodeJob* job);
```

whisperlivekit_amd/csrc/layernorm.hip:

```cpp
#include "common.h"
#include "wave_ops.h"
#include "x3.h"

namespace wlk {

constexpr int kLnMaxPerLane = 24;

template <int NPL>
__global__ __launch_bounds__(256) void layernorm_kernel(const float* __restrict__ x, long ldx,
                                                        const float* __restrict__ gamma,
                                                        const float* __restrict__ beta, float* __restrict__ y,
                                                        long ldy, int rows, int d, PtrTable z, int batch) {
    const int lane = threadIdx.x & 63;
    const int row = blockIdx.x * 4 + (threadIdx.x >> 6);
    if (row >= rows) return;
    if (x == nullptr) {
        x = table_at(z.in, blockIdx.y);
        y = table_at(z.out, blockIdx.y);
    }
    const float* xr = x + (long)row * ldx;
    float v[NPL], g[NPL], b[NPL];
#pragma unroll
    for (int i = 0; i < NPL; ++i) {
        const int c = lane + 64 * i;
        const int cc = c < d ? c : 0;
        v[i] = xr[cc];
        g[i] = gamma[cc];
        b[i] = beta[cc];
    }
#pragma unroll
    for (int i = 0; i < NPL; ++i) { pin_loaded(g[i]); pin_loaded(b[i]); }
    __builtin_amdgcn_sched_barrier(0);
    float sum = 0.f;
#pragma unroll
    for (int i = 0; i < NPL; ++i) {
        v[i] = (lane + 64 * i) < d ? v[i] : 0.f;
        sum += v[i];
    }
    sum = wave_sum(sum);
    const float mean = sum / (float)d;
    float sq = 0.f;
#pragma unroll
    for (int i = 0; i < NPL; ++i) {
        const int c = lane + 64 * i;
        const float t = c < d ? v[i] - mean : 0.f;
        sq += t * t;
    }
    sq = wave_sum(sq);
    const float rstd = 1.0f / sqrtf(sq / (float)d + 1e-5f);
    float* yr = y + (long)row * ldy;
#pragma unroll
    for (int i = 0; i < NPL; ++i) {
        const int c = lane + 64 * i;
        if (c < d) yr[c] = (v[i] - mean) * rstd * g[i] + b[i];
    }
}

template <int NPL>
__global__ __launch_bounds__(256) void layernorm_x3_kernel(const float* __restrict__ x, long ldx,
                                                           const float* __restrict__ gamma,
                                                           const float* __restrict__ beta, unsigned short* __restrict__ y3,
                                                           long ldy3, int rows, int d, PtrTable z) {
    constexpr int NCH = (NPL + 7) / 8;
    const int lane = threadIdx.x & 63;
    const int row = blockIdx.x * 4 + (threadIdx.x >> 6);
    if (row >= rows) return;
    if (x == nullptr) {
        x = table_at(z.in, blockIdx.y);
        y3 = reinterpret_cast<unsigned short*>(table_at(z.out, blockIdx.y));
    }
    const float* xr = x + (long)row * ldx;
    const int n_chunks = d >> 3;
    float v[NPL];
    float4 xc[NCH][2], gc[NCH][2], bc[NCH][2];
#pragma unroll
    for (int i = 0; i < NPL; ++i) {
        const int c = lane + 64 * i;
        v[i] = xr[c < d ? c : 0];
    }
#pragma unroll
    for (int j = 0; j < NCH; ++j) {
        const int q = lane + 64 * j;
        const int at = (q < n_chunks ? q : 0) * 8;
        xc[j][0] = *reinterpret_cast<const float4*>(xr + at);
        xc[j][1] = *reinterpret_cast<const float4*>(xr + at + 4);
        gc[j][0] = *reinterpret_cast<const float4*>(gamma + at);
        gc[j][1] = *reinterpret_cast<const float4*>(gamma + at + 4);
        bc[j][0] = *reinterpret_cast<const float4*>(beta + at);
        bc[j][1] = *reinterpret_cast<const float4*>(beta + at + 4);
    }
#pragma unroll
    for (int j = 0; j < NCH; ++j) {
        pin_loaded(xc[j][0]); pin_loaded(xc[j][1]);
        pin_loaded(gc[j][0]); pin_loaded(gc[j][1]);
        pin_loaded(bc[j][0]); pin_loaded(bc[j][1]);
    }
    __builtin_amdgcn_sched_barrier(0);
    float sum = 0.f;
#pragma unroll
    for (int i = 0; i < NPL; ++i) {
        v[i] = (lane + 64 * i) < d ? v[i] : 0.f;
        sum += v[i];
    }
    sum = wave_sum(sum);
    const float mean = sum / (float)d;
    float sq = 0.f;
#pragma unroll
    for (int i = 0; i < NPL; ++i) {
        const float t = (lane + 64 * i) < d ? v[i] - mean : 0.f;
        sq += t * t;
    }
    sq = wave_sum(sq);
    const float rstd = 1.0f / sqrtf(sq / (float)d + 1e-5f);
    unsigned short* yr = y3 + (long)row * 3 * ldy3;
#pragma unroll
    for (int j = 0; j < NCH; ++j) {
        const int q = lane + 64 * j;
        const float o[8] = {(xc[j][0].x - mean) * rstd * gc[j][0].x + bc[j][0].x, (xc[j][0].y - mean) * rstd * gc[j][0].y + bc[j][0].y,
                            (xc[j][0].z - mean) * rstd * gc[j][0].z + bc[j][0].z, (xc[j][0].w - mean) * rstd * gc[j][0].w + bc[j][0].w,
                            (xc[j][1].x - mean) * rstd * gc[j][1].x + bc[j][1].x, (xc[j][1].y - mean) * rstd * gc[j][1].y + bc[j][1].y,
                            (xc[j][1].z - mean) * rstd * gc[j][1].z + bc[j][1].z, (xc[j][1].w - mean) * rstd * gc[j][1].w + bc[j][1].w};
        if (q < n_chunks) x3_store_chunk(yr + (long)q * 24, o);
    }
}

template <typename... Args>
static void launch_ln_x3_by_width(int d, dim3 grid, hipStream_t stream, Args... args) {
    const int npl = (d + 63) / 64;
    if (npl <= 8) hipLaunchKernelGGL(layernorm_x3_kernel<8>, grid, dim3(256), 0, stream, args...);
    else if (npl <= 12) hipLaunchKernelGGL(layernorm_x3_kernel<12>, grid, dim3(256), 0, stream, args...);
    else if (npl <= 16) hipLaunchKernelGGL(layernorm_x3_kernel<16>, grid, dim3(256), 0, stream, args...);
    else if (npl <= 20) hipLaunchKernelGGL(layernorm_x3_kernel<20>, grid, dim3(256), 0, stream, args...);
    else hipLaunchKernelGGL(layernorm_x3_kernel<kLnMaxPerLane>, grid, dim3(256), 0, stream, args...);
}

template <typename... Args>
static void launch_ln_by_width(int d, dim3 grid, hipStream_t stream, Args... args) {
    const int npl = (d + 63) / 64;
    if (npl <= 8) hipLaunchKernelGGL(layernorm_kernel<8>, grid, dim3(256), 0, stream, args...);
    else if (npl <= 12) hipLaunchKernelGGL(layernorm_kernel<12>, grid, dim3(256), 0, stream, args...);
    else if (npl <= 16) hipLaunchKernelGGL(layernorm_kernel<16>, grid, dim3(256), 0, stream, args...);
    else if (npl <= 20) hipLaunchKernelGGL(layernorm_kernel<20>, grid, dim3(256), 0, stream, args...);
    else hipLaunchKernelGGL(layernorm_kernel<kLnMaxPerLane>, grid, dim3(256), 0, stream, args...);
}

void launch_layernorm(const LaunchCtx& ctx, const float* x, long ldx, const float* gamma, const float* beta,
                      float* y, long ldy, int rows, int d, const char* tag) {
    if (rows <= 0) return;
    if (d > 64 * kLnMaxPerLane) throw std::invalid_argument("layernorm: d too large");
    KernelScope ks(ctx, tag);
    launch_ln_by_width(d, dim3((rows + 3) / 4), ctx.stream, x, ldx, gamma, beta, y, ldy, rows, d, PtrTable{}, 0);
    WLK_HIP(hipGetLastError());
}

void launch_layernorm_batched(const LaunchCtx& ctx, const PtrTable& z, int batch, long ldx, const float* gamma,
                              const float* beta, long ldy, int rows, int d, const char* tag) {
    if (rows <= 0 || batch <= 0) return;
    if (d > 64 * kLnMaxPerLane || batch > kMaxBatch) throw std::invalid_argument("layernorm: d or batch too large");
    KernelScope ks(ctx, tag);
    launch_ln_by_width(d, dim3((rows + 3) / 4, batch), ctx.stream, (const float*)nullptr, ldx, gamma, beta, (float*)nullptr,
                       ldy, rows, d, z, batch);
    WLK_HIP(hipGetLastError());
}


void launch_layernorm_x3(const LaunchCtx& ctx, const float* x, long ldx, const float* gamma, const float* beta,
                         unsigned short* y3, long ldy3, int rows, int d, const char* tag) {
    if (rows <= 0) return;
    if (d > 64 * kLnMaxPerLane || d % 8 != 0 || ldx % 4 != 0 || ldy3 % 8 != 0) throw std::invalid_argument("layernorm (x3): unsupported width");
    KernelScope ks(ctx, tag);
    launch_ln_x3_by_width(d, dim3((rows + 3) / 4), ctx.stream, x, ldx, gamma, beta, y3, ldy3, rows, d, PtrTable{});
    WLK_HIP(hipGetLastError());
}

void launch_layernorm_x3_batched(const LaunchCtx& ctx, const PtrTable& z, int batch, long ldx, const float* gamma,
                                 const float* beta, long ldy3, int rows, int d, const char* tag) {
    if (rows <= 0 || batch <= 0) return;
    if (d > 64 * kLnMaxPerLane || d % 8 != 0 || ldx % 4 != 0 || ldy3 % 8 != 0 || batch > kMaxBatch)
        throw std::invalid_argument("layernorm (x3): unsupported width or batch");
    KernelScope ks(ctx, tag);
    launch_ln_x3_by_width(d, dim3((rows + 3) / 4, batch), ctx.stream, (const float*)nullptr, ldx, gamma, beta,
                          (unsigned short*)nullptr, ldy3, rows, d, z);
    WLK_HIP(hipGetLastError());
}

}
```

whisperlivekit_amd/csrc/loop.hip:

```cpp
#include <algorithm>
#include <cmath>
#include <cstring>
#include <map>
#include <string>
#include <utility>
#include <vector>

#include "../../include/wlk_hip.h"
#include "common.h"
#include "internal.h"
#include <cstdlib>

#include "loop.h"

namespace wlk {

DecodeJob::DecodeJob(const wlk_loop_params& p, const int64_t* tokens, int n_tok, const int32_t* suppress, int n_sup,
                     const int32_t* blank, int n_blank)
    : P(p), seq(tokens, tokens + n_tok), n_before(n_tok), suppress_ids(suppress, suppress + n_sup),
      blank_ids(blank, blank + n_blank), last_attend(p.last_attend_frame) {}

bool DecodeJob::begin_step() {
    if (stop != WLK_STOP_NONE) return false;
    if ((int)seq.size() >= P.max_text_len) {
// ... 386 lines not shown
    return WLK_OK;
}

int wlk_beam_job_begin_step(wlk_beam_job* j, int32_t* n_feed) {
    if (!j || !n_feed) return loop_fail(WLK_ERR_ARG, "decode loop: NULL argument");
    const bool first = j->job.fresh;
    if (!j->job.begin_step()) {
        *n_feed = 0;
        return WLK_OK;
    }
    *n_feed = first ? (int32_t)j->job.rows[0].size() : 1;
    return WLK_OK;
}

int wlk_beam_job_no_speech(wlk_beam_job* j, float prob, int32_t* stops) {
    if (!j || !stops) return loop_fail(WLK_ERR_ARG, "decode loop: NULL argument");
    *stops = j->job.no_speech(prob) ? 1 : 0;
    return WLK_OK;
}

int wlk_beam_job_adjustments(wlk_beam_job* j, const int32_t** ids, const float** deltas, int32_t* n) {
    if (!j || !ids || !deltas || !n) return loop_fail(WLK_ERR_ARG, "decode loop: NULL argument");
    j->job.adjustments(j->ids, j->deltas);
    *ids = j->ids.data();
    *deltas = j->deltas.data();
    *n = (int32_t)j->ids.size();
    return WLK_OK;
}

int wlk_beam_job_consume(wlk_beam_job* j, const float* top_logprobs, const int32_t* top_ids, const int32_t* frames,
                         int32_t* goes_on) {
    if (!j || !top_logprobs || !top_ids || !frames || !goes_on) return loop_fail(WLK_ERR_ARG, "decode loop: NULL argument");
    if (j->job.stop != WLK_STOP_NONE) return loop_fail(WLK_ERR_STATE, "beam decode loop: the loop is over");
    const int rc = j->job.consume(top_logprobs, top_ids, frames);
    if (rc < 0) return loop_fail(WLK_ERR_ARG, "beam decode loop: fewer live candidates than beams");
    *goes_on = rc;
    return WLK_OK;
}

int wlk_beam_job_state(wlk_beam_job* j, int64_t* rows, int cap, int32_t* row_len, float* sum_logprobs, int32_t* source_rows,
                       int32_t* completed) {
    if (!j || !row_len) return loop_fail(WLK_ERR_ARG, "decode loop: NULL argument");
    const BeamJob& job = j->job;
    const int n = (int)job.rows[0].size();
    *row_len = n;
    if (rows) {
        if (cap < job.B * n) return loop_fail(WLK_ERR_CAPACITY, "beam decode loop: row buffer too small");
        for (int b = 0; b < job.B; ++b)
            for (int i = 0; i < n; ++i) rows[(size_t)b * n + i] = job.rows[(size_t)b][(size_t)i];
    }
    for (int b = 0; b < job.B; ++b) {
        if (sum_logprobs) sum_logprobs[b] = job.sums[(size_t)b];
        if (source_rows) source_rows[b] = job.src[(size_t)b];
    }
    if (completed) *completed = job.completed ? 1 : 0;
    return WLK_OK;
}

int wlk_beam_job_result(wlk_beam_job* j, wlk_loop_result* result, int64_t* new_tokens, int32_t* step_tokens,
                        int32_t* step_frames, float* step_sum_logprobs, int cap) {
    if (!j) return loop_fail(WLK_ERR_ARG, "decode loop: job is NULL");
    return copy_beam_result(j->job, result, new_tokens, step_tokens, step_frames, step_sum_logprobs, cap);
}

int wlk_beam_job_destroy(wlk_beam_job* j) {
    delete j;
    return WLK_OK;
}

int wlk_decode_beam_until_stop(wlk_session* s, const int64_t* tokens, int n_tok, const wlk_loop_params* p,
                               const int32_t* suppress_ids, int n_suppress, const int32_t* blank_ids, int n_blank,
                               wlk_loop_result* result, int64_t* new_tokens, int32_t* step_tokens, int32_t* step_frames,
                               float* step_sum_logprobs, int cap) {
    if (!s) return loop_fail(WLK_ERR_ARG, "decode loop: session is NULL");
    if (int rc = check_loop_args(p, tokens, n_tok, suppress_ids, n_suppress, blank_ids, n_blank)) return rc;
    const int B = s->beam, K = B + 1;
    if (B < 2 || B > 7) return loop_fail(WLK_ERR_ARG, "beam decode loop: the session's beam must be in 2..7");
    if (p->n_force != 0) return loop_fail(WLK_ERR_ARG, "beam decode loop: teacher forcing is defined for beam 1 only");
    BeamJob job(*p, B, tokens, n_tok, suppress_ids, n_suppress, blank_ids, n_blank);
    std::vector<int32_t> ids, adj_rows, top((size_t)B * K), frames((size_t)B);
    std::vector<float> deltas, lp((size_t)B * K), prob((size_t)B);
    std::vector<int64_t> feed;
    while (job.begin_step()) {
        const bool first = job.fresh;
        if (first) {
            feed.clear();
            for (int b = 0; b < B; ++b) feed.insert(feed.end(), tokens, tokens + n_tok);
            if (int rc = wlk_decode(s, feed.data(), B, n_tok, 1, p->sot_index)) return rc;
        } else {
            feed.resize((size_t)B);
            for (int b = 0; b < B; ++b) feed[(size_t)b] = job.rows[(size_t)b].back();
            const int rc = wlk_beam_step(s, feed.data(), job.src.data());
            if (rc == 1) {
                if (int rc2 = wlk_kv_reorder(s, job.src.data(), B)) return rc2;
                if (int rc2 = wlk_decode(s, feed.data(), B, 1, 0, p->sot_index)) return rc2;
            } else if (rc != WLK_OK) {
                return rc;
            }
        }
        job.adjustments(ids, deltas);
        adj_rows.assign(ids.size(), -1);
        if (first && p->no_speech_token >= 0) {
            if (int rc = wlk_select_first(s, p->no_speech_token, adj_rows.data(), ids.data(), deltas.data(), (int)ids.size(), K,
                                          p->content_mel_len, prob.data(), lp.data(), top.data(), frames.data()))
                return rc;
            if (job.no_speech(prob[0])) break;
        } else if (int rc = wlk_select(s, adj_rows.data(), ids.data(), deltas.data(), (int)ids.size(), K, p->content_mel_len,
                                       lp.data(), top.data(), frames.data())) {
            return rc;
        }
        const int go = job.consume(lp.data(), top.data(), frames.data());
        if (go < 0) return loop_fail(WLK_ERR_STATE, "beam decode loop: fewer live candidates than beams");
        if (go == 0) break;
    }
    return copy_beam_result(job, result, new_tokens, step_tokens, step_frames, step_sum_logprobs, cap);
}

int wlk_decode_until_stop(wlk_session* s, const int64_t* tokens, int n_tok, const wlk_loop_params* p,
                          const int32_t* suppress_ids, int n_suppress, const int32_t* blank_ids, int n_blank,
                          wlk_loop_result* result, int64_t* new_tokens, int32_t* step_tokens, int32_t* step_frames,
                          float* step_sum_logprobs, int cap) {
    if (!s) return loop_fail(WLK_ERR_ARG, "decode loop: session is NULL");
    if (int rc = check_loop_args(p, tokens, n_tok, suppress_ids, n_suppress, blank_ids, n_blank)) return rc;
    if (s->beam != 1) return loop_fail(WLK_ERR_ARG, "decode loop: the session's beam must be 1");
    DecodeJob job(*p, tokens, n_tok, suppress_ids, n_suppress, blank_ids, n_blank);
    std::vector<int32_t> ids, rows;
    std::vector<float> deltas;
    struct InLoop {
        wlk_session* s;
        explicit InLoop(wlk_session* ss) : s(ss) { wlk_engine_loop_enter(s); }
        ~InLoop() { wlk_engine_loop_exit(s); }
    } in_loop(s);
    while (job.begin_step()) {
        const bool first = job.fresh;
        const int64_t* feed = first ? job.seq.data() : job.seq.data() + job.seq.size() - 1;
        float lp[2];
        int32_t top[2], frame = 0;
        if (!first) {
            job.adjustments(ids, deltas);
            const int rc = wlk_step_select(s, feed[0], ids.data(), deltas.data(), (int)ids.size(), p->content_mel_len, lp,
                                           top, &frame);
            if (rc == WLK_OK) {
                if (!job.consume(lp, top, frame)) break;
                if (wlk_engine_wants(s)) {
                    if (int rc2 = wlk_engine_run_job(s, &job)) return rc2;
                    break;
                }
                continue;
            }
            if (rc != 1) return rc;
        }
        int taken = first ? wlk_engine_prefill(s, feed, (int)job.seq.size(), p->sot_index) : 1;
        if (taken != WLK_OK && taken != 1) return taken;
        if (taken == 1)
            if (int rc = wlk_decode(s, feed, 1, first ? (int)job.seq.size() : 1, first ? 1 : 0, p->sot_index)) return rc;
        job.adjustments(ids, deltas);
        rows.assign(ids.size(), -1);
        static const bool merged_first = getenv("WLK_NO_FIRST_MERGE") == nullptr;
        if (first && p->no_speech_token >= 0 && !merged_first) {
            float prob = 0.f;
            if (int rc = wlk_no_speech_prob(s, p->no_speech_token, &prob)) return rc;
            if (job.no_speech(prob)) break;
            if (int rc = wlk_select(s, rows.data(), ids.data(), deltas.data(), (int)ids.size(), 2, p->content_mel_len, lp, top,
                                    &frame))
                return rc;
        } else if (first && p->no_speech_token >= 0) {
            float prob = 0.f;
            if (int rc = wlk_select_first(s, p->no_speech_token, rows.data(), ids.data(), deltas.data(), (int)ids.size(), 2,
                                          p->content_mel_len, &prob, lp, top, &frame))
                return rc;
            if (job.no_speech(prob)) break;
        } else if (int rc = wlk_select(s, rows.data(), ids.data(), deltas.data(), (int)ids.size(), 2, p->content_mel_len, lp,
                                       top, &frame)) {
            return rc;
        }
        if (!job.consume(lp, top, frame)) break;
        if (wlk_engine_wants(s)) {
            if (int rc = wlk_engine_run_job(s, &job)) return rc;
            break;
        }
    }
    return copy_result(job, result, new_tokens, step_tokens, step_frames, step_sum_logprobs, cap);
}

}
```

whisperlivekit_amd/csrc/select.hip:

```cpp
#include <atomic>
#include <cstdlib>

#include "common.h"
#include "wave_ops.h"
#include "align_body.h"

namespace wlk {

constexpr int kSelThreads = 1024;
constexpr int kMaxTopK = 8;

__device__ __forceinline__ float block_max(float v, float* red) {
    v = wave_max(v);
    const int wave = threadIdx.x >> 6, lane = threadIdx.x & 63;
    __syncthreads();
    if (lane == 0) red[wave] = v;
    __syncthreads();
    float r = red[0];
    for (int w = 1; w < (int)(blockDim.x >> 6); ++w) r = fmaxf(r, red[w]);
    return r;
}

__device__ __forceinline__ float block_sum(float v, float* red) {
    v = wave_sum(v);
    const int wave = threadIdx.x >> 6, lane = threadIdx.x & 63;
    __syncthreads();
    if (lane == 0) red[wave] = v;
    __syncthreads();
    float r = 0.f;
    for (int w = 0; w < (int)(blockDim.x >> 6); ++w) r += red[w];
    return r;
}

constexpr int kSelBlocks = 64;
struct SelPartial {
    float mx, sum;
    float v[kMaxTopK];
    int i[kMaxTopK];
};

struct TopkArgs {
    float* logits;
    int n_vocab, k, n_rows;
    SelPartial* parts;
    const int* adj_row;
    const int* adj_ids;
    const float* adj_deltas;
    int n_adj;
    float* top_vals;
    int* top_ids;
    StepHostOut host;
    const float* ns_logits = nullptr;
    int ns_token = 0;
    float* ns_probs = nullptr;
};

__device__ __forceinline__ void topk_stage1_stream(float* __restrict__ logits, int n_vocab, int k,
                                                 SelPartial* __restrict__ parts, const int* __restrict__ adj_row,
                                                 const int* __restrict__ adj_ids, const float* __restrict__ adj_deltas,
                                                 int n_adj, int slice, int row) {
    __shared__ float red[16];
    __shared__ float cand_v[4];
    __shared__ int cand_i[4];
    __shared__ int taken[kMaxTopK];
    const int tid = threadIdx.x;
    const int per = (n_vocab + kSelBlocks - 1) / kSelBlocks;
    const int lo = slice * per;
    const int hi = min(n_vocab, lo + per);
    float* x = logits + (long)row * n_vocab;
    for (int i = tid; i < n_adj; i += 256) {
        const int id = adj_ids[i];
        const int r = adj_row[i];
        if (id >= lo && id < hi && (r < 0 || r == row)) x[id] += adj_deltas[i];
    }
    __syncthreads();
    float mx = -INFINITY;
    for (int i = lo + tid; i < hi; i += 256) mx = fmaxf(mx, x[i]);
    mx = block_max(mx, red);
    float sum = 0.f;
    if (mx > -INFINITY)
        for (int i = lo + tid; i < hi; i += 256) sum += expf(x[i] - mx);
    sum = block_sum(sum, red);
    SelPartial* out = parts + (long)row * kSelBlocks + slice;
    if (tid == 0) { out->mx = mx; out->sum = sum; }
    for (int round = 0; round < k; ++round) {
        float bv = -INFINITY;
        int bi = 0x7fffffff;
        for (int i = lo + tid; i < hi; i += 256) {
            bool skip = false;
            for (int t = 0; t < round; ++t) skip |= (taken[t] == i);
            const float v = x[i];
            if (!skip && (v > bv || (v == bv && i < bi))) { bv = v; bi = i; }
        }
        wave_argmax(bv, bi);
        __syncthreads();
        if ((tid & 63) == 0) { cand_v[tid >> 6] = bv; cand_i[tid >> 6] = bi; }
        __syncthreads();
        if (tid == 0) {
            for (int w = 1; w < 4; ++w)
                if (cand_v[w] > bv || (cand_v[w] == bv && cand_i[w] < bi)) { bv = cand_v[w]; bi = cand_i[w]; }
            taken[round] = bi;
            out->v[round] = bv;
            out->i[round] = bi;
        }
        __syncthreads();
    }
}

constexpr int kSelKeep = 4;
__device__ __forceinline__ void topk_stage1_body(float* __restrict__ logits, int n_vocab, int k,
                                                 SelPartial* __restrict__ parts, const int* __restrict__ adj_row,
                                                 const int* __restrict__ adj_ids, const float* __restrict__ adj_deltas,
                                                 int n_adj, int slice, int row) {
    const int per = (n_vocab + kSelBlocks - 1) / kSelBlocks;
    if (per > 256 * kSelKeep) {
        topk_stage1_stream(logits, n_vocab, k, parts, adj_row, adj_ids, adj_deltas, n_adj, slice, row);
        return;
    }
    __shared__ float red[16];
    __shared__ float cand_v[4];
    __shared__ int cand_i[4];
    __shared__ float adj_buf[256 * kSelKeep];
    const int tid = threadIdx.x;
    const int lo = slice * per;
    const int hi = min(n_vocab, lo + per);
    float* x = logits + (long)row * n_vocab;
    float xv[kSelKeep];
    const int lo_safe = lo < n_vocab ? lo : n_vocab - 1;
#pragma unroll
    for (int j = 0; j < kSelKeep; ++j) {
        const int i = lo + tid + 256 * j;
        xv[j] = x[i < hi ? i : lo_safe];
        adj_buf[tid + 256 * j] = 0.f;
    }
    __syncthreads();
    for (int i0 = 0; i0 < n_adj; i0 += 256) {
        const int i = i0 + tid, ic = i < n_adj ? i : 0;
        const int id = adj_ids[ic];
        const int r = adj_row[ic];
        const float dl = adj_deltas[ic];
        if (i < n_adj && id >= lo && id < hi && (r < 0 || r == row)) adj_buf[id - lo] = dl;
    }
    __syncthreads();
#pragma unroll
    for (int j = 0; j < kSelKeep; ++j) {
        const int i = lo + tid + 256 * j;
        const float a = adj_buf[tid + 256 * j];
        if (a != 0.f && i < hi) {
            xv[j] += a;
            x[i] = xv[j];
        }
    }
    float mx = -INFINITY;
#pragma unroll
    for (int j = 0; j < kSelKeep; ++j)
        if (lo + tid + 256 * j < hi) mx = fmaxf(mx, xv[j]);
    mx = block_max(mx, red);
    float sum = 0.f;
    if (mx > -INFINITY) {
#pragma unroll
        for (int j = 0; j < kSelKeep; ++j)
            if (lo + tid + 256 * j < hi) sum += expf(xv[j] - mx);
    }
    sum = block_sum(sum, red);
    SelPartial* out = parts + (long)row * kSelBlocks + slice;
    if (tid == 0) { out->mx = mx; out->sum = sum; }
    int taken = -1;
    int taken_all[kMaxTopK];
#pragma unroll
    for (int t = 0; t < kMaxTopK; ++t) taken_all[t] = -1;
    for (int round = 0; round < k; ++round) {
        float bv = -INFINITY;
        int bi = 0x7fffffff;
#pragma unroll
        for (int j = 0; j < kSelKeep; ++j) {
            const int i = lo + tid + 256 * j;
            if (i < hi) {
                bool skip = false;
#pragma unroll
                for (int t = 0; t < kMaxTopK; ++t) skip |= (t < round && taken_all[t] == i);
                const float v = xv[j];
                if (!skip && (v > bv || (v == bv && i < bi))) { bv = v; bi = i; }
            }
        }
        wave_argmax(bv, bi);
        __syncthreads();
        if ((tid & 63) == 0) { cand_v[tid >> 6] = bv; cand_i[tid >> 6] = bi; }
        __syncthreads();
        bv = cand_v[0];
        bi = cand_i[0];
#pragma unroll
        for (int w = 1; w < 4; ++w)
            if (cand_v[w] > bv || (cand_v[w] == bv && cand_i[w] < bi)) { bv = cand_v[w]; bi = cand_i[w]; }
        taken = bi;
#pragma unroll
        for (int t = 0; t < kMaxTopK; ++t)
            if (t == round) taken_all[t] = taken;
        if (tid == 0) {
            out->v[round] = bv;
            out->i[round] = bi;
        }
    }
}

__global__ __launch_bounds__(256) void topk_stage1_kernel(float* __restrict__ logits, int n_vocab, int k,
                                                          SelPartial* __restrict__ parts, const int* __restrict__ adj_row,
                                                          const int* __restrict__ adj_ids,
// ... 85 lines not shown
    const int per = (n_vocab + kSelBlocks - 1) / kSelBlocks;
    const int lo = slice * per;
    const int hi = min(n_vocab, lo + per);
    const float* x = logits + (long)row * n_vocab;
    const int lo_safe = lo < n_vocab ? lo : n_vocab - 1;
    float xv[kWideKeep];
#pragma unroll
    for (int j = 0; j < kWideKeep; ++j) {
        const int i = lo + tid + 256 * j;
        xv[j] = x[i < hi ? i : lo_safe];
    }
#pragma unroll
    for (int j = 0; j < kWideKeep; ++j) pin_loaded(xv[j]);
    __builtin_amdgcn_sched_barrier(0);
#pragma unroll
    for (int j = 0; j < kWideKeep; ++j)
        if (lo + tid + 256 * j >= hi) xv[j] = -INFINITY;
    float mx = -INFINITY;
#pragma unroll
    for (int j = 0; j < kWideKeep; ++j)
        if (lo + tid + 256 * j < hi) mx = fmaxf(mx, xv[j]);
    mx = block_max(mx, red);
    float sum = 0.f;
    if (mx > -INFINITY) {
#pragma unroll
        for (int j = 0; j < kWideKeep; ++j)
            if (lo + tid + 256 * j < hi) sum += expf(xv[j] - mx);
    }
    sum = block_sum(sum, red);
    WidePartial* out = parts + (long)row * kSelBlocks + slice;
    if (tid == 0) { out->mx = mx; out->sum = sum; }
    auto best_after = [&](float wv, int wi, float& bv, int& bi) {
        bv = -INFINITY;
        bi = kWideNone;
#pragma unroll
        for (int j = 0; j < kWideKeep; ++j) {
            const int i = lo + tid + 256 * j;
            const float v = xv[j];
            const bool after = v < wv || (v == wv && i > wi);
            if (v > -INFINITY && after && (v > bv || (v == bv && i < bi))) { bv = v; bi = i; }
        }
    };
    float mv;
    int mi;
    best_after(INFINITY, -1, mv, mi);
    for (int round = 0; round < k; ++round) {
        float bv = mv;
        int bi = mi;
        wave_argmax(bv, bi);
        __syncthreads();
        if ((tid & 63) == 0) { cand_v[tid >> 6] = bv; cand_i[tid >> 6] = bi; }
        __syncthreads();
        bv = cand_v[0];
        bi = cand_i[0];
#pragma unroll
        for (int w = 1; w < 4; ++w)
            if (cand_v[w] > bv || (cand_v[w] == bv && cand_i[w] < bi)) { bv = cand_v[w]; bi = cand_i[w]; }
        if (tid == 0) {
            out->v[round] = bv;
            out->i[round] = bi;
        }
        if (bi != kWideNone && mi == bi) best_after(bv, bi, mv, mi);
    }
}

__global__ __launch_bounds__(64) void topk_wide_stage2_kernel(const WidePartial* __restrict__ parts, int k,
                                                              float* __restrict__ top_vals, int* __restrict__ top_ids) {
    __shared__ float list_v[kWideTopK * 64];
    __shared__ int list_i[kWideTopK * 64];
    const int lane = threadIdx.x, row = blockIdx.x;
    const WidePartial* p = parts + (long)row * kSelBlocks + lane;
    const float pmx = p->mx, psum = p->sum;
#pragma unroll
    for (int t = 0; t < kWideTopK; ++t) {
        list_v[t * 64 + lane] = t < k ? p->v[t] : -INFINITY;
        list_i[t * 64 + lane] = t < k ? p->i[t] : kWideNone;
    }
    const float mx = wave_max(pmx);
    float sum = pmx > -INFINITY ? psum * expf(pmx - mx) : 0.f;
    sum = wave_sum(sum);
    const float lse = logf(sum);
    int head = 0;
    float cv = list_v[lane];
    int ci = list_i[lane];
    for (int round = 0; round < k; ++round) {
        float wv = cv;
        int wi = ci;
        wave_argmax(wv, wi);
        const bool some = wi != kWideNone;
        if (some && wi == ci) {
            ++head;
            const int h = head < kWideTopK ? head : kWideTopK - 1;
            cv = head < k ? list_v[h * 64 + lane] : -INFINITY;
            ci = head < k ? list_i[h * 64 + lane] : kWideNone;
        }
        if (lane == 0) {
            top_ids[row * k + round] = some ? wi : -1;
            top_vals[row * k + round] = some ? (wv - mx) - lse : -INFINITY;
        }
    }
}

void launch_logsoftmax_topk_wide(const LaunchCtx& ctx, const float* logits, int n_vocab, int n_rows, int k, float* top_vals,
                                 int* top_ids, void* scratch) {
    if (k < 1 || k > kWideTopK) throw std::invalid_argument("wide top-k: k must be in [1, 16]");
    if (n_rows < 1 || n_vocab < 1) throw std::invalid_argument("wide top-k: at least one row and one logit");
    if (!topk_wide_applicable(n_vocab, k))
        throw std::invalid_argument("wide top-k: rows of at most 262144 logits (a slice of 4096 held in registers)");
    WidePartial* parts = static_cast<WidePartial*>(scratch);
    {
        KernelScope ks(ctx, "sel_topk_wide_stage1", 0.0, 4.0 * n_rows * (double)n_vocab);
        hipLaunchKernelGGL(topk_wide_stage1_kernel, dim3(kSelBlocks, n_rows), dim3(256), 0, ctx.stream, logits, n_vocab, k,
                           parts);
        WLK_HIP(hipGetLastError());
    }
    {
        KernelScope ks(ctx, "sel_topk_wide_stage2");
        hipLaunchKernelGGL(topk_wide_stage2_kernel, dim3(n_rows), dim3(64), 0, ctx.stream, parts, k, top_vals, top_ids);
        WLK_HIP(hipGetLastError());
    }
}

size_t topk_wide_scratch_bytes(int n_rows) { return sizeof(WidePartial) * kSelBlocks * (size_t)n_rows; }

__device__ __forceinline__ void token_prob_body(const float* __restrict__ logits, int n_vocab, int token,
                                                float* __restrict__ probs, int row) {
    __shared__ float red[16];
    constexpr int kKeep = 64;
    const int tid = threadIdx.x;
    const float* x = logits + (long)row * n_vocab;
    float mx = -INFINITY, sum = 0.f;
    if (n_vocab <= kKeep * kSelThreads) {
        float v[kKeep];
#pragma unroll
        for (int j = 0; j < kKeep; ++j) {
            const int i = tid + j * kSelThreads;
            v[j] = i < n_vocab ? x[i] : -INFINITY;
        }
#pragma unroll
        for (int j = 0; j < kKeep; ++j) mx = fmaxf(mx, v[j]);
        mx = block_max(mx, red);
#pragma unroll
        for (int j = 0; j < kKeep; ++j)
            if (tid + j * kSelThreads < n_vocab) sum += expf(v[j] - mx);
    } else {
        for (int i = tid; i < n_vocab; i += kSelThreads) mx = fmaxf(mx, x[i]);
        mx = block_max(mx, red);
        for (int i = tid; i < n_vocab; i += kSelThreads) sum += expf(x[i] - mx);
    }
    sum = block_sum(sum, red);
    if (tid == 0) probs[row] = expf(x[token] - mx) / sum;
}

__global__ __launch_bounds__(kSelThreads) void token_prob_kernel(const float* __restrict__ logits, int n_vocab,
                                                                 int token, float* __restrict__ probs) {
    token_prob_body(logits, n_vocab, token, probs, blockIdx.x);
}

void launch_token_prob(const LaunchCtx& ctx, const float* logits, int n_vocab, int n_rows, int token, float* probs) {
    KernelScope ks(ctx, "sel_token_prob");
    hipLaunchKernelGGL(token_prob_kernel, dim3(n_rows), dim3(kSelThreads), 0, ctx.stream, logits, n_vocab, token,
                       probs);
    WLK_HIP(hipGetLastError());
}

__global__ __launch_bounds__(256) void align_zscore_kernel(AlignArgs a) {
    align_zscore_body(a, blockIdx.x, blockIdx.y, blockIdx.z);
}

__device__ __forceinline__ float median7(float v0, float v1, float v2, float v3, float v4, float v5, float v6) {
    float v[7] = {v0, v1, v2, v3, v4, v5, v6};
#pragma unroll
    for (int i = 1; i < 7; ++i) {
#pragma unroll
        for (int j = i; j > 0; --j) {
            const float lo = fminf(v[j - 1], v[j]);
            const float hi = fmaxf(v[j - 1], v[j]);
            v[j - 1] = lo;
            v[j] = hi;
        }
    }
    return v[3];
}

__global__ __launch_bounds__(256) void align_argmax_kernel(AlignArgs a) {
    __shared__ float bestv[256];
    __shared__ int besti[256];
    const int tid = threadIdx.x;
    const int b = blockIdx.x;
    if (a.rows) a.content_len = a.rows[b].content_len;
    const float* zb = a.z + (long)b * a.n_align * a.T;
    float bv = -INFINITY;
    int bi = 0x7fffffff;
    for (int f = tid; f < a.T; f += 256) {
        float acc = 0.f;
        for (int al = 0; al < a.n_align; ++al) {
            const float* z = zb + (long)al * a.T;
            float v[7];
#pragma unroll
            for (int o = -3; o <= 3; ++o) {
                int idx = f + o;
                if (idx < 0) idx = -idx;
                if (idx >= a.T) idx = 2 * (a.T - 1) - idx;
                v[o + 3] = z[idx];
            }
            acc += a.T > 3 ? median7(v[0], v[1], v[2], v[3], v[4], v[5], v[6]) : z[f];
        }
        const float m = acc / (float)a.n_align;
        a.attn_last[(long)b * a.T + f] = m;
        if (f < a.content_len && (m > bv || (m == bv && f < bi))) { bv = m; bi = f; }
    }
    bestv[tid] = bv;
    besti[tid] = bi;
    __syncthreads();
    for (int s = 128; s >= 1; s >>= 1) {
        if (tid < s) {
            const float ov = bestv[tid + s];
            const int oi = besti[tid + s];
            if (ov > bestv[tid] || (ov == bestv[tid] && oi < besti[tid])) { bestv[tid] = ov; besti[tid] = oi; }
        }
        __syncthreads();
    }
    if (tid == 0) a.frames[b] = besti[0] == 0x7fffffff ? 0 : besti[0];
}

__device__ __forceinline__ void align_argmax_lds_body(AlignArgs a, int b, const StepHostOut host = StepHostOut{}, unsigned seq = 0) {
    extern __shared__ __attribute__((aligned(16))) float zs[];
    __shared__ float bestv[16];
    __shared__ int besti[16];
    const int tid = threadIdx.x;
    if (a.rows) a.content_len = a.rows[b].content_len;
    const float* zb = a.z + (long)b * a.n_align * a.T;
    for (int i = tid; i < a.n_align * a.T; i += 1024) zs[i] = zb[i];
    asm volatile("" : "+v"(seq));
    __syncthreads();
    float bv = -INFINITY;
    int bi = 0x7fffffff;
    for (int f = tid; f < a.T; f += 1024) {
        float acc = 0.f;
        for (int al = 0; al < a.n_align; ++al) {
            const float* z = zs + al * a.T;
            float v[7];
#pragma unroll
            for (int o = -3; o <= 3; ++o) {
                int idx = f + o;
                if (idx < 0) idx = -idx;
                if (idx >= a.T) idx = 2 * (a.T - 1) - idx;
                v[o + 3] = z[idx];
            }
            acc += a.T > 3 ? median7(v[0], v[1], v[2], v[3], v[4], v[5], v[6]) : z[f];
        }
        const float m = acc / (float)a.n_align;
        a.attn_last[(long)b * a.T + f] = m;
        if (f < a.content_len && (m > bv || (m == bv && f < bi))) { bv = m; bi = f; }
    }
    wave_argmax(bv, bi);
    if ((tid & 63) == 0) { bestv[tid >> 6] = bv; besti[tid >> 6] = bi; }
    __syncthreads();
    if (tid == 0) {
        for (int w = 1; w < 16; ++w)
            if (bestv[w] > bestv[0] || (bestv[w] == bestv[0] && besti[w] < besti[0])) { bestv[0] = bestv[w]; besti[0] = besti[w]; }
    }
    if (tid == 0) {
        const int frame = besti[0] == 0x7fffffff ? 0 : besti[0];
        a.frames[b] = frame;
        if (host.result) {
            host.result[b].frame = frame;
            publish_flag(&host.result[b].flag_align, seq);
        }
    }
}

__global__ __launch_bounds__(1024) void align_argmax_lds_kernel(AlignArgs a) { align_argmax_lds_body(a, blockIdx.x); }

#define WLK_PIN_SELECT_ARGS(t, a)                                                                                           \
    do {                                                                                                                    \
        asm volatile("" ::"s"((t).logits), "s"((t).n_vocab), "s"((t).k), "s"((t).n_rows), "s"((t).parts), "s"((t).adj_row), \
                     "s"((t).adj_ids), "s"((t).adj_deltas), "s"((t).n_adj), "s"((t).top_vals), "s"((t).top_ids),            \
                     "s"((t).host.result), "s"((t).host.n_adj), "s"((t).host.seq));                                         \
        asm volatile("" ::"s"((a).ring), "s"((a).n_align), "s"((a).n_beam), "s"((a).ring_rows), "s"((a).T),                 \
                     "s"((a).prefill_rows), "s"((a).n_single), "s"((a).newest_row), "s"((a).single_base),                   \
                     "s"((a).content_len), "s"((a).z), "s"((a).attn_last), "s"((a).frames), "s"((a).rows));                 \
        __builtin_amdgcn_sched_barrier(0);                                                                                  \
    } while (0)

__global__ __launch_bounds__(256) void select_stage1_kernel(TopkArgs t, AlignArgs a, int zf_blocks) {
    WLK_PIN_SELECT_ARGS(t, a);
    const int n_topk = kSelBlocks * t.n_rows;
    if ((int)blockIdx.x < n_topk) {
        const int n_adj = t.host.n_adj ? *t.host.n_adj : t.n_adj;
        topk_stage1_body(t.logits, t.n_vocab, t.k, t.parts, t.adj_row, t.adj_ids, t.adj_deltas, n_adj,
                         blockIdx.x % kSelBlocks, blockIdx.x / kSelBlocks);
    } else {
        const int i = blockIdx.x - n_topk;
        const int fblock = i % zf_blocks, rest = i / zf_blocks;
        align_zscore_body(a, fblock, rest % a.n_align, rest / a.n_align);
    }
}

__global__ __launch_bounds__(1024) void select_stage2_kernel(TopkArgs t, AlignArgs a) {
    WLK_PIN_SELECT_ARGS(t, a);
    unsigned seq = 0;
    if (t.host.result) seq = *t.host.seq;
    if ((int)blockIdx.x < a.n_beam) {
        align_argmax_lds_body(a, blockIdx.x, t.host, seq);
    } else if ((int)blockIdx.x < a.n_beam + t.n_rows) {
        if (threadIdx.x < 64) topk_stage2_body(t.parts, t.k, t.top_vals, t.top_ids, blockIdx.x - a.n_beam, t.host, seq);
    } else {
        token_prob_body(t.ns_logits, t.n_vocab, t.ns_token, t.ns_probs, blockIdx.x - a.n_beam - t.n_rows);
    }
}

constexpr int kAlignPartFrames = 256;
__device__ __forceinline__ void align_median_part_body(AlignArgs a, int b, int blk, int n_blk) {
    __shared__ float bestv[4];
    __shared__ int besti[4];
    const int tid = threadIdx.x;
    if (a.rows) a.content_len = a.rows[b].content_len;
    const float* zb = a.z + (long)b * a.n_align * a.T;
    const int f = blk * kAlignPartFrames + tid;
    float bv = -INFINITY;
    int bi = 0x7fffffff;
    if (f < a.T) {
        float acc = 0.f;
        for (int al = 0; al < a.n_align; ++al) {
            const float* z = zb + (long)al * a.T;
            float v[7];
#pragma unroll
            for (int o = -3; o <= 3; ++o) {
                int idx = f + o;
                if (idx < 0) idx = -idx;
                if (idx >= a.T) idx = 2 * (a.T - 1) - idx;
                v[o + 3] = z[idx];
            }
            acc += a.T > 3 ? median7(v[0], v[1], v[2], v[3], v[4], v[5], v[6]) : z[f];
        }
        const float m = acc / (float)a.n_align;
        a.attn_last[(long)b * a.T + f] = m;
        if (f < a.content_len && (m > bv || (m == bv && f < bi))) { bv = m; bi = f; }
    }
    wave_argmax(bv, bi);
    if ((tid & 63) == 0) { bestv[tid >> 6] = bv; besti[tid >> 6] = bi; }
    __syncthreads();
    if (tid == 0) {
        for (int w = 1; w < 4; ++w)
            if (bestv[w] > bestv[0] || (bestv[w] == bestv[0] && besti[w] < besti[0])) { bestv[0] = bestv[w]; besti[0] = besti[w]; }
        float* slot = a.part + ((long)b * 64 + blk) * 2;
        slot[0] = bestv[0];
        slot[1] = __int_as_float(besti[0]);
    }
}

__global__ __launch_bounds__(256) void select_stage1_early_kernel(TopkArgs t, AlignArgs a, int n_blk) {
    WLK_PIN_SELECT_ARGS(t, a);
    const int n_topk = kSelBlocks * t.n_rows;
    if ((int)blockIdx.x < n_topk) {
        const int n_adj = t.host.n_adj ? *t.host.n_adj : t.n_adj;
        topk_stage1_body(t.logits, t.n_vocab, t.k, t.parts, t.adj_row, t.adj_ids, t.adj_deltas, n_adj,
                         blockIdx.x % kSelBlocks, blockIdx.x / kSelBlocks);
    } else {
        const int i = blockIdx.x - n_topk;
        align_median_part_body(a, i / n_blk, i % n_blk, n_blk);
    }
}

__global__ __launch_bounds__(64) void select_stage2_early_kernel(TopkArgs t, AlignArgs a, int n_blk) {
    asm volatile("" ::"s"(t.parts), "s"(t.k), "s"(t.top_vals), "s"(t.top_ids), "s"(t.host.result), "s"(t.host.seq), "s"(a.part),
                 "s"(a.frames));
    __builtin_amdgcn_sched_barrier(0);
    const int row = blockIdx.x, lane = threadIdx.x;
    unsigned seq = 0;
    if (t.host.result) seq = *t.host.seq;
    const float* slot = a.part + ((long)row * 64 + (lane < n_blk ? lane : 0)) * 2;
    float bv = slot[0];
    int bi = __float_as_int(slot[1]);
    if (lane >= n_blk) { bv = -INFINITY; bi = 0x7fffffff; }
    topk_stage2_body(t.parts, t.k, t.top_vals, t.top_ids, row, t.host, seq, false);
    wave_argmax(bv, bi);
    if (lane == 0) {
        const int frame = bi == 0x7fffffff ? 0 : bi;
        a.frames[row] = frame;
        if (t.host.result) {
            t.host.result[row].frame = frame;
            __threadfence_system();
            __hip_atomic_store(&t.host.result[row].flag_topk, seq, __ATOMIC_RELEASE, __HIP_MEMORY_SCOPE_SYSTEM);
            __hip_atomic_store(&t.host.result[row].flag_align, seq, __ATOMIC_RELEASE, __HIP_MEMORY_SCOPE_SYSTEM);
        }
    }
}

bool select_early_z_enabled() {
    const char* e = getenv("WLK_EARLY_Z");
    return !(e && e[0] == '0');
}

bool select_fused_applicable(int n_rows, int k, const AlignArgs& a) {
    static const bool enabled = [] {
        const char* e = getenv("WLK_SELECT_FUSED");
        return !(e && e[0] == '0');
    }();
    const size_t lds = (size_t)a.n_align * a.T * sizeof(float);
    return enabled && a.n_align > 0 && a.n_beam == n_rows && lds + 8192 + 1024 <= 150 * 1024 && k >= 1 && k <= kMaxTopK;
}

bool launch_select_fused(const LaunchCtx& ctx, float* logits, int n_vocab, int n_rows, int k, float* top_vals, int* top_ids,
                         void* scratch, const int* adj_row, const int* adj_ids, const float* adj_deltas, int n_adj,
                         const AlignArgs& a, const StepHostOut& host, const float* ns_logits, int ns_token, float* ns_probs,
                         bool early_z) {
    const size_t lds = (size_t)a.n_align * a.T * sizeof(float);
    if (!select_fused_applicable(n_rows, k, a)) return false;
    static std::atomic<bool> attr_set[64];
    int dev = 0;
    WLK_HIP(hipGetDevice(&dev));
    if (dev < 64 && !attr_set[dev].load(std::memory_order_acquire)) {
        WLK_HIP(hipFuncSetAttribute(reinterpret_cast<const void*>(select_stage2_kernel),
                                    hipFuncAttributeMaxDynamicSharedMemorySize, 150 * 1024));
        attr_set[dev].store(true, std::memory_order_release);
    }
    TopkArgs t{logits, n_vocab, k, n_rows, static_cast<SelPartial*>(scratch), adj_row, adj_ids, adj_deltas, n_adj, top_vals, top_ids,
               host, ns_logits, ns_token, ns_probs};
    const int zf = (a.T + 63) / 64;
    if (early_z) {
        const int n_blk = (a.T + kAlignPartFrames - 1) / kAlignPartFrames;
        if (ns_logits || !a.part || n_blk > 64) throw std::invalid_argument("select: the early z-score form needs a.part, T <= 16384 and no no-speech block");
        {
            KernelScope ks(ctx, "sel_stage1", 0.0, 4.0 * 3.0 * n_rows * (double)n_vocab);
            hipLaunchKernelGGL(select_stage1_early_kernel, dim3(kSelBlocks * n_rows + n_blk * a.n_beam), dim3(256), 0, ctx.stream, t, a, n_blk);
            WLK_HIP(hipGetLastError());
        }
        {
            KernelScope ks(ctx, "sel_stage2");
            hipLaunchKernelGGL(select_stage2_early_kernel, dim3(n_rows), dim3(64), 0, ctx.stream, t, a, n_blk);
            WLK_HIP(hipGetLastError());
        }
        return true;
    }
    {
        KernelScope ks(ctx, "sel_stage1", 0.0, 4.0 * 3.0 * n_rows * (double)n_vocab);
        hipLaunchKernelGGL(select_stage1_kernel, dim3(kSelBlocks * n_rows + zf * a.n_align * a.n_beam), dim3(256), 0,
                           ctx.stream, t, a, zf);
        WLK_HIP(hipGetLastError());
    }
    {
        KernelScope ks(ctx, "sel_stage2");
        hipLaunchKernelGGL(select_stage2_kernel, dim3(a.n_beam + n_rows + (ns_logits ? n_rows : 0)), dim3(1024), lds,
                           ctx.stream, t, a);
        WLK_HIP(hipGetLastError());
    }
    return true;
}

namespace {
struct PickBest {
    float v;
    int i;
};
__device__ __forceinline__ PickBest pick_better(PickBest a, PickBest b) {
    return (b.v > a.v || (b.v == a.v && b.i < a.i)) ? b : a;
}
__device__ __forceinline__ PickBest pick_wave_best(PickBest x) {
#pragma unroll
    for (int off = 32; off >= 1; off >>= 1) {
        PickBest o;
        o.v = __shfl_xor(x.v, off);
        o.i = __shfl_xor(x.i, off);
        x = pick_better(x, o);
    }
    return x;
}
__device__ __forceinline__ bool rules_allowed(const unsigned char* __restrict__ mask, const PickRules& p, int v) {
    const int tb = p.timestamp_begin;
    const unsigned char m = mask[v];
    if ((m & 1) || (p.first_step && (m & 2))) return false;
    if (p.without_timestamps) return true;
    if (v == p.no_timestamps) return false;
    if (p.ts_mode == 1 && v >= tb) return false;
    if (p.ts_mode == 2 && v < p.eot) return false;
    if (v >= tb && v < p.ts_bound) return false;
    if (p.first_step && (v < tb || (p.max_initial >= 0 && v >= tb + p.max_initial + 1))) return false;
    return true;
}
}

__global__ __launch_bounds__(1024) void rules_pick_kernel(const float* __restrict__ logits, int n_vocab,
                                                          const unsigned char* __restrict__ mask, PickRules p,
                                                          int* __restrict__ out_token, float* __restrict__ out_logprob) {
    __shared__ PickBest s_all[16], s_ts[16];
    __shared__ float s_text[16], s_sum_all[16], s_sum_ts[16];
    const int tid = threadIdx.x, lane = tid & 63, wave = tid >> 6;
    const int tb = p.timestamp_begin;
    auto allowed = [&](int v) -> bool { return rules_allowed(mask, p, v); };
    PickBest all{-INFINITY, 0x7fffffff}, ts{-INFINITY, 0x7fffffff};
    float text = -INFINITY;
    for (int v = tid; v < n_vocab; v += 1024) {
        if (!allowed(v)) continue;
        const float x = logits[v];
        all = pick_better(all, PickBest{x, v});
        if (v >= tb) ts = pick_better(ts, PickBest{x, v});
        else text = fmaxf(text, x);
    }
    all = pick_wave_best(all);
    ts = pick_wave_best(ts);
    text = wave_max(text);
    if (lane == 0) {
        s_all[wave] = all;
        s_ts[wave] = ts;
        s_text[wave] = text;
    }
    __syncthreads();
    all = s_all[0];
    ts = s_ts[0];
    text = s_text[0];
#pragma unroll
    for (int w = 1; w < 16; ++w) {
        all = pick_better(all, s_all[w]);
        ts = pick_better(ts, s_ts[w]);
        text = fmaxf(text, s_text[w]);
    }
    float sum_all = 0.f, sum_ts = 0.f;
    for (int v = tid; v < n_vocab; v += 1024) {
        if (!allowed(v)) continue;
        const float x = logits[v];
        sum_all += expf(x - all.v);
        if (v >= tb) sum_ts += expf(x - ts.v);
    }
    sum_all = wave_sum(sum_all);
    sum_ts = wave_sum(sum_ts);
    if (lane == 0) {
        s_sum_all[wave] = sum_all;
        s_sum_ts[wave] = sum_ts;
    }
    __syncthreads();
    if (tid == 0) {
        sum_all = 0.f;
        sum_ts = 0.f;
        for (int w = 0; w < 16; ++w) {
            sum_all += s_sum_all[w];
            sum_ts += s_sum_ts[w];
        }
        const float lse_all = all.v + logf(sum_all);
        const bool ts_wins = !p.without_timestamps && ts.i != 0x7fffffff && (ts.v + logf(sum_ts)) - lse_all > text - lse_all;
        const PickBest pick = ts_wins ? ts : all;
        out_token[0] = pick.i == 0x7fffffff ? 0 : pick.i;
        out_logprob[0] = -logf(ts_wins ? sum_ts : sum_all);
    }
}

void launch_rules_pick(const LaunchCtx& ctx, const float* logits, int n_vocab, const unsigned char* mask, const PickRules& p,
                       int* out_token, float* out_logprob) {
    KernelScope ks(ctx, "rules_pick", 0.0, 8.0 * n_vocab);
    hipLaunchKernelGGL(rules_pick_kernel, dim3(1), dim3(1024), 0, ctx.stream, logits, n_vocab, mask, p, out_token, out_logprob);
    WLK_HIP(hipGetLastError());
}

constexpr int kRulesKeep = 52;
namespace {
__device__ __forceinline__ bool pick_after(float xv, int xi, PickBest w) { return xv < w.v || (xv == w.v && xi > w.i); }
}

template <bool kRegs>
__device__ __forceinline__ void rules_topk_body(const float* __restrict__ x, int n_vocab, const unsigned char* __restrict__ mask,
                                                const PickRules& p, int k, float* __restrict__ out_lp,
                                                int* __restrict__ out_ids) {
    __shared__ PickBest s_best[16];
    __shared__ float s_a[16], s_b[16], s_c[16];
    const int tid = threadIdx.x, lane = tid & 63, wave = tid >> 6;
    const int tb = p.timestamp_begin;
    float xv[kRegs ? kRulesKeep : 1];
    if constexpr (kRegs) {
#pragma unroll
        for (int j = 0; j < kRulesKeep; ++j) {
            const int v = tid + 1024 * j, vc = v < n_vocab ? v : 0;
            const float raw = x[vc];
            xv[j] = (v < n_vocab && rules_allowed(mask, p, vc)) ? raw : -INFINITY;
        }
    }
    auto sweep = [&](auto&& f) {
        if constexpr (kRegs) {
#pragma unroll
            for (int j = 0; j < kRulesKeep; ++j) f(tid + 1024 * j, xv[j]);
        } else {
            for (int v = tid; v < n_vocab; v += 1024) f(v, rules_allowed(mask, p, v) ? x[v] : -INFINITY);
        }
    };
    float m_ts = -INFINITY, m_text = -INFINITY;
// ... 138 lines not shown
```

Before: 203.9 audio_s/s.

## Add fused beam-1 prefill path with mapped host tokens and early-z no-speech select

Adds a dedicated beam-1 prefill entry point. It reads tokens and step parameters straight from mapped pinned host memory, fuses embedding with the first layer's LN1, and merges the final LN and logits GEMV for the last and SOT rows. The selection kernels gain an early-z variant that also computes the no-speech probability in split partial form, and the host waits on a result flag instead of issuing memcpys and syncs. The aim is to cut launches, H2D copies and host round-trips per prefill, at the cost of more specialised kernels and a new code path to keep correct.

```diff
diff --git a/whisperlivekit_amd/csrc/api.hip b/whisperlivekit_amd/csrc/api.hip
--- a/whisperlivekit_amd/csrc/api.hip
+++ b/whisperlivekit_amd/csrc/api.hip
@@ -460,7 +460,7 @@
         s->top_ids = reinterpret_cast<int*>(s->top_vals) + (size_t)beam * 8;
         s->frames = s->top_ids + (size_t)beam * 8;
         WLK_HIP(hipMalloc(&s->topk_scratch, topk_scratch_bytes(beam)));
-        s->probs = dev_alloc<float>(beam);
+        s->probs = dev_alloc<float>((size_t)beam * (1 + kSelectNsPartFloats));
         WLK_HIP(hipHostMalloc(&s->pinned, wlk_session::kPinnedBytes, hipHostMallocDefault));
         WLK_HIP(hipHostMalloc(&s->dec_stage, 65536, hipHostMallocDefault));
         WLK_HIP(hipHostMalloc(&s->audio_stage, wlk_session::kPinnedBytes, hipHostMallocDefault));
@@ -468,8 +468,9 @@
         WLK_HIP(hipEventCreateWithFlags(&s->dec_stage_ev, hipEventDisableTiming));
         if (beam == 1) {
             void* hp = nullptr;
-            WLK_HIP(hipHostMalloc(&hp, 4096, hipHostMallocMapped | hipHostMallocCoherent));
-            std::memset(hp, 0, 4096);
+            const size_t block_bytes = 4096 + ctx * sizeof(int);
+            WLK_HIP(hipHostMalloc(&hp, block_bytes, hipHostMallocMapped | hipHostMallocCoherent));
+            std::memset(hp, 0, block_bytes);
             s->step_host = static_cast<StepBlock*>(hp);
             s->result_host = reinterpret_cast<StepResult*>(static_cast<char*>(hp) + 2048);
             void* dp = nullptr;
@@ -477,6 +478,10 @@
             s->step_host_dev = static_cast<StepBlock*>(dp);
             s->result_host_dev = reinterpret_cast<StepResult*>(static_cast<char*>(dp) + 2048);
             s->step_dev = reinterpret_cast<StepBlock*>(dev_alloc<int>(sizeof(StepBlock) / 4));
+            s->prefill_tokens = reinterpret_cast<int*>(static_cast<char*>(hp) + 4096);
+            s->prefill_tokens_dev = reinterpret_cast<const int*>(static_cast<char*>(dp) + 4096);
+            const char* pf = getenv("WLK_PREFILL_FUSED");
+            s->prefill_fused = !(pf && pf[0] == '0');
         }
         WLK_HIP(hipStreamSynchronize(st));
         *out = s.release();
@@ -489,6 +494,10 @@
     if (s->step_count && getenv("WLK_STEP_TIMING"))
         fprintf(stderr, "[wlk] one-replay steps: %llu, mean %.1f us per step (graph launch call %.1f us)\n",
                 (unsigned long long)s->step_count, s->step_ns / 1e3 / s->step_count, s->step_launch_ns / 1e3 / s->step_count);
+    if (s->prefill_count && getenv("WLK_STEP_TIMING"))
+        fprintf(stderr, "[wlk] one-enqueue prefills: %llu, mean %.1f us per prefill (enqueue %.1f us)\n",
+                (unsigned long long)s->prefill_count, s->prefill_ns / 1e3 / s->prefill_count,
+                s->prefill_launch_ns / 1e3 / s->prefill_count);
     (void)wlk_engine_detach(s);
     (void)hipSetDevice(s->m->device);
     (void)hipStreamSynchronize(s->stream);
@@ -940,13 +949,15 @@
 
 static void enqueue_decode(wlk_session* s, const LaunchCtx& c, int n_rows, int n_tok, bool first, int sot_index,
                            bool step_block = false, const AlignArgs* side_align = nullptr, int side_blocks = 0, int side_zf = 0,
-                           bool ancestry = false) {
+                           bool ancestry = false, bool prefill_block = false) {
     wlk_model* m = s->m;
     const wlk_dims& D = m->D;
     const int ctx_len = D.n_text_ctx;
     const int R = n_rows * n_tok;
     const int d = D.n_text_state, T = D.n_audio_ctx, H = D.n_text_head, V = D.n_vocab;
-    if (!step_block)
+    if (prefill_block && (!first || n_rows != 1 || step_block || ancestry || !gemv_applicable(2, d)))
+        throw std::logic_error("decode: the prefill block serves beam-1 prefills");
+    if (!step_block && !prefill_block)
         WLK_HIP(hipMemcpyAsync(s->step_in, s->dec_stage, (size_t)(3 * s->max_rows + 1) * sizeof(int), hipMemcpyHostToDevice,
                                s->stream));
     const bool fused = gemv_applicable(R, d) && n_tok == 1;
@@ -960,6 +971,10 @@
     if (step_block)
         launch_embed_step(c, s->step_host_dev, s->step_dev, s->tokens_dev, s->ring_row, s->beam_of_row, s->d_offset,
                           m->w_tok_emb, m->w_dec_pos, s->dx, d);
+    else if (prefill_block)
+        launch_embed_ln_prefill(c, s->step_host_dev, s->prefill_tokens_dev, s->step_dev, s->tokens_dev, s->ring_row,
+                                s->beam_of_row, s->d_offset, m->w_tok_emb, m->w_dec_pos, m->dec_layers[0].ln1w,
+                                m->dec_layers[0].ln1b, s->dx, s->dh, n_tok, d);
     else
         launch_embed(c, s->tokens_dev, m->w_tok_emb, m->w_dec_pos, s->dx, n_rows, n_tok, s->d_offset, d);
     const float scale = std::pow((float)kHeadDim, -0.25f);
@@ -977,7 +992,7 @@
             g.kcache = kc; g.vcache = vc; g.kv_pos = s->d_offset; g.kv_d = d; g.kv_ctx = ctx_len;
             launch_gemv(c, g, "dec_ln1_qkv_kv");
         } else {
-            launch_layernorm(c, s->dx, d, L.ln1w, L.ln1b, s->dh, d, R, d, "dec_ln1");
+            if (!(prefill_block && i == 0)) launch_layernorm(c, s->dx, d, L.ln1w, L.ln1b, s->dh, d, R, d, "dec_ln1");
             g.A = s->dh;
             if (!gemv_applicable(R, d) && gemm_takes_kwave(R, 3 * d, d)) {
                 g.kcache = kc; g.vcache = vc; g.kv_pos = s->d_offset; g.kv_d = d; g.kv_ctx = ctx_len; g.kv_ntok = n_tok;
@@ -1075,11 +1090,17 @@
         launch_ring_softmax(c, s->ring, s->ring_row, s->beam_of_row, m->all_ranks, m->n_align, R, s->ring_rows, s->beam, T);
     GemmArgs lg;
     lg.lda = d; lg.W = m->w_tok_emb; lg.C = s->logits_last; lg.ldc = V; lg.M = n_rows; lg.N = V; lg.K = d;
-    if (side_align && !fused) throw std::logic_error("decode: side workgroups need the fused step");
+    if (side_align && !fused && !prefill_block) throw std::logic_error("decode: side workgroups need the fused step");
     if (fused) {
         lg.A = s->dx; lg.ln_gamma = m->w_ln_w; lg.ln_beta = m->w_ln_b;
         lg.side_align = side_align; lg.side_blocks = side_blocks; lg.side_zf = side_zf;
         launch_gemv(c, lg, "dec_lnf_logits");
+    } else if (prefill_block) {
+        lg.A = s->dx + (size_t)(n_tok - 1) * d; lg.lda = (sot_index - (n_tok - 1)) * d; lg.M = 2;
+        lg.ln_gamma = m->w_ln_w; lg.ln_beta = m->w_ln_b;
+        lg.side_align = side_align; lg.side_blocks = side_blocks; lg.side_zf = side_zf;
+        launch_gemv(c, lg, "dec_lnf_logits");
+        return;
     } else if (first && n_rows == 1 && gemv_applicable(2, d) && getenv("WLK_NO_PREFILL_MERGE") == nullptr) {
         launch_layernorm(c, s->dx + (size_t)(n_tok - 1) * d, (long)(sot_index - (n_tok - 1)) * d, m->w_ln_w, m->w_ln_b,
                          s->hsel, d, 2, d, "dec_ln_f");
@@ -1494,6 +1515,97 @@
                        frames_host, no_speech_token, no_speech_host);
 }
 
+static void ensure_step_align_dev(wlk_session* s, const AlignArgs& a) {
+    if (s->step_align_dev) return;
+    AlignArgs ad = a;
+    ad.rows = &s->step_dev->row;
+    s->step_align_dev = reinterpret_cast<AlignArgs*>(dev_alloc<char>(sizeof(AlignArgs)));
+    WLK_HIP(hipMemcpyAsync(s->step_align_dev, &ad, sizeof(AlignArgs), hipMemcpyHostToDevice, s->stream));
+    WLK_HIP(hipStreamSynchronize(s->stream));
+}
+
+extern "C++" int wlk_prefill_select(wlk_session* s, const int64_t* tokens, int n_tok, int sot_index, int no_speech_token,
+                                    const int32_t* adj_ids, const float* adj_deltas, int n_adj, int content_mel_len,
+                                    float* no_speech, float* top_logprobs2, int32_t* top_ids2, int32_t* frame) {
+    const bool merged = getenv("WLK_NO_PREFILL_MERGE") == nullptr && getenv("WLK_NO_FIRST_MERGE") == nullptr;
+    wlk_model* m = s->m;
+    const wlk_dims& D = m->D;
+    if (!merged || !s->prefill_fused || s->beam != 1 || !s->step_host || s->debug || s->prof_on || !s->use_graph ||
+        s->align_raw_scores || n_adj > kStepMaxAdj || !gemv_applicable(2, D.n_text_state) || !s->encoded)
+        return 1;
+    AlignArgs a;
+    a.ring = nullptr; a.n_align = m->n_align; a.n_beam = 1; a.ring_rows = s->ring_rows; a.T = D.n_audio_ctx;
+    a.prefill_rows = 0; a.n_single = 0; a.newest_row = 0; a.single_base = D.n_text_ctx; a.content_len = 0;
+    a.z = s->z; a.attn_last = s->attn_last; a.frames = s->frames;
+    if (!select_fused_applicable(1, 2, a)) return 1;
+    if (!(select_early_z_enabled() && D.n_vocab >= 16384)) return 1;
+    if (n_tok < 1 || n_tok > D.n_text_ctx || sot_index < 0 || sot_index >= n_tok || no_speech_token >= D.n_vocab) return 1;
+    for (int p = 0; p < n_tok; ++p)
+        if (tokens[p] < 0 || tokens[p] >= D.n_vocab) return fail(WLK_ERR_ARG, "token id out of range");
+    if (content_mel_len < 0) return fail(WLK_ERR_ARG, "content_mel_len out of range");
+    if (content_mel_len > D.n_audio_ctx) content_mel_len = D.n_audio_ctx;
+    return guarded([&]() {
+        WLK_HIP(hipSetDevice(m->device));
+        const LaunchCtx c = s->ctx();
+        StepBlock& b = *s->step_host;
+        StepRow& r = b.row;
+        r.kcache = s->kcache[s->kv_cur]; r.vcache = s->vcache[s->kv_cur]; r.cross_kv = s->cross_kv; r.ring = s->ring;
+        r.token = (int)tokens[n_tok - 1]; r.offset = 0; r.ring_row = 0;
+        r.prefill_rows = n_tok; r.n_single = 0; r.newest_row = n_tok - 1; r.content_len = content_mel_len; r.pad = 0;
+        b.n_adj = n_adj;
+        for (int i = 0; i < n_adj; ++i) {
+            b.adj_row[i] = -1;
+            b.adj_ids[i] = adj_ids[i];
+            b.adj_deltas[i] = adj_deltas[i];
+        }
+        for (int p = 0; p < n_tok; ++p) s->prefill_tokens[p] = (int)tokens[p];
+        const unsigned seq = ++s->step_seq ? s->step_seq : ++s->step_seq;
+        b.seq = seq;
+        std::atomic_thread_fence(std::memory_order_release);
+
+        ensure_step_align_dev(s, a);
+        a.rows = &s->step_dev->row;
+        a.part = s->z + (size_t)s->beam * std::max(m->n_align, 1) * D.n_audio_ctx;
+        const int zf_blocks = (a.T + 63) / 64;
+        const auto t_enter = std::chrono::steady_clock::now();
+        try {
+            enqueue_decode(s, c, 1, n_tok, true, sot_index, false, s->step_align_dev, zf_blocks * a.n_align * a.n_beam, zf_blocks,
+                           false, true);
+            StepHostOut ho;
+            ho.result = s->result_host_dev;
+            ho.n_adj = &s->step_dev->n_adj;
+            ho.seq = &s->step_dev->seq;
+            const bool ns = no_speech_token >= 0;
+            if (!launch_select_fused(c, s->logits_last, D.n_vocab, 1, 2, s->top_vals, s->top_ids, s->topk_scratch,
+                                     s->step_dev->adj_row, s->step_dev->adj_ids, s->step_dev->adj_deltas, 0, a, ho,
+                                     ns ? s->logits_sot : nullptr, no_speech_token, ns ? s->top_vals + 17 : nullptr, true, s->probs + s->beam))
+                throw std::runtime_error("fused prefill: read-out not available");
+            s->prefill_launch_ns += (uint64_t)std::chrono::duration_cast<std::chrono::nanoseconds>(std::chrono::steady_clock::now() - t_enter).count();
+            wlk_wait_step_flags(s->stream, s->result_host, 1, seq);
+        } catch (...) {
+            s->encoded = false;
+            s->n_steps = 0;
+            s->self_len = 0;
+            throw;
+        }
+        volatile StepResult* res = s->result_host;
+        s->anc_live = false;
+        s->self_len = n_tok;
+        s->n_steps = 1;
+        s->have_sot = true;
+        s->prefill_rows = n_tok;
+        s->last_rows = 1;
+        s->last_ntok = n_tok;
+        s->prefill_ns += (uint64_t)std::chrono::duration_cast<std::chrono::nanoseconds>(std::chrono::steady_clock::now() - t_enter).count();
+        s->prefill_count += 1;
+        top_logprobs2[0] = res->top_vals[0]; top_logprobs2[1] = res->top_vals[1];
+        top_ids2[0] = res->top_ids[0]; top_ids2[1] = res->top_ids[1];
+        *frame = res->frame;
+        *no_speech = no_speech_token >= 0 ? res->no_speech : 0.f;
+        return WLK_OK;
+    });
+}
+
 extern "C++" int wlk_step_select(wlk_session* s, int64_t token, const int32_t* adj_ids, const float* adj_deltas, int n_adj,
                                  int content_mel_len, float* top_logprobs2, int32_t* top_ids2, int32_t* frame) {
     static const bool enabled = [] {
@@ -1533,12 +1645,7 @@
         hipGraphExec_t& exec = s->fstep_exec[s->kv_cur];
         if (!exec) {
             const int zf_blocks = (a.T + 63) / 64;
-            if (!s->step_align_dev) {
-                AlignArgs ad = a;
-                ad.rows = &s->step_dev->row;
-                s->step_align_dev = reinterpret_cast<AlignArgs*>(dev_alloc<char>(sizeof(AlignArgs)));
-                WLK_HIP(hipMemcpyAsync(s->step_align_dev, &ad, sizeof(AlignArgs), hipMemcpyHostToDevice, s->stream));
-            }
+            ensure_step_align_dev(s, a);
             WLK_HIP(hipStreamSynchronize(s->stream));
             capture_step_graph(s->stream, exec, [&] {
                 a.rows = &s->step_dev->row;
diff --git a/whisperlivekit_amd/csrc/common.h b/whisperlivekit_amd/csrc/common.h
--- a/whisperlivekit_amd/csrc/common.h
+++ b/whisperlivekit_amd/csrc/common.h
@@ -97,7 +97,7 @@
     int top_ids[2];
     int frame;
     unsigned flag_topk, flag_align;
-    int pad;
+    float no_speech;
 };
 struct StepHostOut {
     StepResult* result = nullptr;
@@ -119,6 +119,9 @@
 void launch_embed_step(const LaunchCtx& ctx, const StepBlock* host_block, StepBlock* dev_block, int* tokens_dev,
                        int* ring_row, int* beam_of_row, int* d_offset, const float* tok_emb, const float* pos_emb, float* x,
                        int d);
+void launch_embed_ln_prefill(const LaunchCtx& ctx, const StepBlock* host_block, const int* host_tokens, StepBlock* dev_block,
+                             int* tokens_dev, int* ring_row, int* beam_of_row, int* d_offset, const float* tok_emb,
+                             const float* pos_emb, const float* gamma, const float* beta, float* x, float* h, int n_tok, int d);
 
 constexpr int kMaxBatch = 8;
 struct PtrTable {
@@ -494,7 +497,8 @@
 bool launch_select_fused(const LaunchCtx& ctx, float* logits, int n_vocab, int n_rows, int k, float* top_vals, int* top_ids,
                          void* scratch, const int* adj_row, const int* adj_ids, const float* adj_deltas, int n_adj,
                          const AlignArgs& a, const StepHostOut& host = StepHostOut{}, const float* ns_logits = nullptr,
-                         int ns_token = 0, float* ns_probs = nullptr, bool early_z = false);
+                         int ns_token = 0, float* ns_probs = nullptr, bool early_z = false, float* ns_part = nullptr);
+constexpr int kSelectNsPartFloats = 17;
 bool select_early_z_enabled();
 bool select_fused_applicable(int n_rows, int k, const AlignArgs& a);
 void launch_alignatt_rows(const LaunchCtx& ctx, const AlignArgs& a, const StepRow* rows);
diff --git a/whisperlivekit_amd/csrc/internal.h b/whisperlivekit_amd/csrc/internal.h
--- a/whisperlivekit_amd/csrc/internal.h
+++ b/whisperlivekit_amd/csrc/internal.h
@@ -223,6 +223,10 @@
     wlk::StepBlock *step_host = nullptr, *step_host_dev = nullptr, *step_dev = nullptr;
     wlk::StepResult *result_host = nullptr, *result_host_dev = nullptr;
     hipGraphExec_t fstep_exec[2] = {nullptr, nullptr};
+    int* prefill_tokens = nullptr;
+    const int* prefill_tokens_dev = nullptr;
+    bool prefill_fused = false;
+    uint64_t prefill_ns = 0, prefill_launch_ns = 0, prefill_count = 0;
     wlk::AlignArgs* step_align_dev = nullptr;
     unsigned step_seq = 0;
     uint64_t step_ns = 0, step_launch_ns = 0, step_count = 0;
@@ -298,6 +302,9 @@
 
 int wlk_step_select(wlk_session* s, int64_t token, const int32_t* adj_ids, const float* adj_deltas, int n_adj,
                     int content_mel_len, float* top_logprobs2, int32_t* top_ids2, int32_t* frame);
+int wlk_prefill_select(wlk_session* s, const int64_t* tokens, int n_tok, int sot_index, int no_speech_token,
+                       const int32_t* adj_ids, const float* adj_deltas, int n_adj, int content_mel_len, float* no_speech,
+                       float* top_logprobs2, int32_t* top_ids2, int32_t* frame);
 int wlk_beam_step(wlk_session* s, const int64_t* tokens, const int32_t* source_rows);
 int wlk_select_first(wlk_session* s, int no_speech_token, const int32_t* adj_row, const int32_t* adj_ids,
                      const float* adj_deltas, int n_adj, int k, int content_mel_len, float* no_speech_host,
diff --git a/whisperlivekit_amd/csrc/layernorm.hip b/whisperlivekit_amd/csrc/layernorm.hip
--- a/whisperlivekit_amd/csrc/layernorm.hip
+++ b/whisperlivekit_amd/csrc/layernorm.hip
@@ -124,6 +124,90 @@
     }
 }
 
+template <int NPL>
+__global__ __launch_bounds__(64) void embed_ln_prefill_kernel(const StepBlock* __restrict__ host_block,
+                                                              const int* __restrict__ host_tokens,
+                                                              StepBlock* __restrict__ dev_block, int* __restrict__ tokens_dev,
+                                                              int* __restrict__ ring_row, int* __restrict__ beam_of_row,
+                                                              int* __restrict__ d_offset, const float* __restrict__ tok_emb,
+                                                              const float* __restrict__ pos_emb,
+                                                              const float* __restrict__ gamma, const float* __restrict__ beta,
+                                                              float* __restrict__ x, float* __restrict__ y, int d) {
+    constexpr int kWords = sizeof(StepBlock) / 4;
+    const int lane = threadIdx.x, row = blockIdx.x, n_rows = gridDim.x;
+    const int token = __hip_atomic_load(host_tokens + row, __ATOMIC_RELAXED, __HIP_MEMORY_SCOPE_SYSTEM);
+    const unsigned* src = reinterpret_cast<const unsigned*>(host_block);
+    unsigned* dst = reinterpret_cast<unsigned*>(dev_block);
+    for (int w = row * 64 + lane; w < kWords; w += n_rows * 64)
+        dst[w] = __hip_atomic_load(src + w, __ATOMIC_RELAXED, __HIP_MEMORY_SCOPE_SYSTEM);
+    if (lane == 0) {
+        tokens_dev[row] = token;
+        ring_row[row] = row;
+        beam_of_row[row] = 0;
+        if (row == 0) d_offset[0] = 0;
+    }
+    const float* e = tok_emb + (long)token * d;
+    const float* pe = pos_emb + (long)row * d;
+    float v[NPL], g[NPL], b[NPL];
+#pragma unroll
+    for (int i = 0; i < NPL; ++i) {
+        const int c = lane + 64 * i;
+        const int cc = c < d ? c : 0;
+        v[i] = e[cc] + pe[cc];
+        g[i] = gamma[cc];
+        b[i] = beta[cc];
+    }
+#pragma unroll
+    for (int i = 0; i < NPL; ++i) { pin_loaded(g[i]); pin_loaded(b[i]); }
+    __builtin_amdgcn_sched_barrier(0);
+    float sum = 0.f;
+#pragma unroll
+    for (int i = 0; i < NPL; ++i) {
+        v[i] = (lane + 64 * i) < d ? v[i] : 0.f;
+        sum += v[i];
+    }
+    sum = wave_sum(sum);
+    const float mean = sum / (float)d;
+    float sq = 0.f;
+#pragma unroll
+    for (int i = 0; i < NPL; ++i) {
+        const int c = lane + 64 * i;
+        const float t = c < d ? v[i] - mean : 0.f;
+        sq += t * t;
+    }
+    sq = wave_sum(sq);
+    const float rstd = 1.0f / sqrtf(sq / (float)d + 1e-5f);
+    float* xr = x + (long)row * d;
+    float* yr = y + (long)row * d;
+#pragma unroll
+    for (int i = 0; i < NPL; ++i) {
+        const int c = lane + 64 * i;
+        if (c < d) {
+            xr[c] = v[i];
+            yr[c] = (v[i] - mean) * rstd * g[i] + b[i];
+        }
+    }
+}
+
+void launch_embed_ln_prefill(const LaunchCtx& ctx, const StepBlock* host_block, const int* host_tokens, StepBlock* dev_block,
+                             int* tokens_dev, int* ring_row, int* beam_of_row, int* d_offset, const float* tok_emb,
+                             const float* pos_emb, const float* gamma, const float* beta, float* x, float* h, int n_tok, int d) {
+    if (n_tok <= 0) return;
+    if (d > 64 * kLnMaxPerLane) throw std::invalid_argument("layernorm: d too large");
+    KernelScope ks(ctx, "dec_embed_ln1");
+    const int npl = (d + 63) / 64;
+#define WLK_EMBED_LN(NPLv)                                                                                                   \
+    hipLaunchKernelGGL(embed_ln_prefill_kernel<NPLv>, dim3(n_tok), dim3(64), 0, ctx.stream, host_block, host_tokens, dev_block, \
+                       tokens_dev, ring_row, beam_of_row, d_offset, tok_emb, pos_emb, gamma, beta, x, h, d)
+    if (npl <= 8) WLK_EMBED_LN(8);
+    else if (npl <= 12) WLK_EMBED_LN(12);
+    else if (npl <= 16) WLK_EMBED_LN(16);
+    else if (npl <= 20) WLK_EMBED_LN(20);
+    else WLK_EMBED_LN(kLnMaxPerLane);
+#undef WLK_EMBED_LN
+    WLK_HIP(hipGetLastError());
+}
+
 template <typename... Args>
 static void launch_ln_x3_by_width(int d, dim3 grid, hipStream_t stream, Args... args) {
     const int npl = (d + 63) / 64;
diff --git a/whisperlivekit_amd/csrc/loop.hip b/whisperlivekit_amd/csrc/loop.hip
--- a/whisperlivekit_amd/csrc/loop.hip
+++ b/whisperlivekit_amd/csrc/loop.hip
@@ -562,6 +562,22 @@
         }
         int taken = first ? wlk_engine_prefill(s, feed, (int)job.seq.size(), p->sot_index) : 1;
         if (taken != WLK_OK && taken != 1) return taken;
+        if (first && taken == 1) {
+            job.adjustments(ids, deltas);
+            float prob = 0.f;
+            const int rc = wlk_prefill_select(s, feed, (int)job.seq.size(), p->sot_index, p->no_speech_token, ids.data(),
+                                              deltas.data(), (int)ids.size(), p->content_mel_len, &prob, lp, top, &frame);
+            if (rc == WLK_OK) {
+                if (p->no_speech_token >= 0 && job.no_speech(prob)) break;
+                if (!job.consume(lp, top, frame)) break;
+                if (wlk_engine_wants(s)) {
+                    if (int rc2 = wlk_engine_run_job(s, &job)) return rc2;
+                    break;
+                }
+                continue;
+            }
+            if (rc != 1) return rc;
+        }
         if (taken == 1)
             if (int rc = wlk_decode(s, feed, 1, first ? (int)job.seq.size() : 1, first ? 1 : 0, p->sot_index)) return rc;
         job.adjustments(ids, deltas);
diff --git a/whisperlivekit_amd/csrc/select.hip b/whisperlivekit_amd/csrc/select.hip
--- a/whisperlivekit_amd/csrc/select.hip
+++ b/whisperlivekit_amd/csrc/select.hip
@@ -53,6 +53,7 @@
     const float* ns_logits = nullptr;
     int ns_token = 0;
     float* ns_probs = nullptr;
+    float* ns_part = nullptr;
 };
 
 __device__ __forceinline__ void topk_stage1_stream(float* __restrict__ logits, int n_vocab, int k,
@@ -444,6 +445,72 @@
     if (tid == 0) probs[row] = expf(x[token] - mx) / sum;
 }
 
+constexpr int kNsGroups = kSelThreads / 256;
+constexpr int kNsPartFloats = kSelThreads / 64 + 1;
+static_assert(kNsPartFloats == kSelectNsPartFloats, "common.h sizes the scratch");
+__device__ __forceinline__ void token_prob_part_body(const float* __restrict__ logits, int n_vocab, float* __restrict__ part,
+                                                     int row, int q) {
+    __shared__ float red[16];
+    constexpr int kKeep = 64, kBatch = 26;
+    const int tid = threadIdx.x, lane = tid & 63, wave = tid >> 6;
+    const float* x = logits + (long)row * n_vocab;
+    const int vt = 256 * q + tid;
+    const bool keep = n_vocab <= kKeep * kSelThreads;
+    float v[kKeep];
+    if (keep) {
+#pragma unroll
+        for (int j = 0; j < kKeep; ++j) v[j] = x[min(vt + j * kSelThreads, n_vocab - 1)];
+    }
+    float mx = -INFINITY;
+    if ((n_vocab & 3) == 0 && (reinterpret_cast<size_t>(x) & 15) == 0) {
+        const float4* x4 = reinterpret_cast<const float4*>(x);
+        const int n4 = n_vocab >> 2;
+        for (int base = tid; base < n4; base += 256 * kBatch) {
+            float4 t[kBatch];
+#pragma unroll
+            for (int u = 0; u < kBatch; ++u) t[u] = x4[min(base + 256 * u, n4 - 1)];
+#pragma unroll
+            for (int u = 0; u < kBatch; ++u) pin_loaded(t[u]);
+            __builtin_amdgcn_sched_barrier(0);
+#pragma unroll
+            for (int u = 0; u < kBatch; ++u) mx = fmaxf(fmaxf(fmaxf(mx, t[u].x), fmaxf(t[u].y, t[u].z)), t[u].w);
+        }
+    } else {
+        for (int base = tid; base < n_vocab; base += 256 * 2 * kBatch) {
+            float t[2 * kBatch];
+#pragma unroll
+            for (int u = 0; u < 2 * kBatch; ++u) t[u] = x[min(base + 256 * u, n_vocab - 1)];
+#pragma unroll
+            for (int u = 0; u < 2 * kBatch; ++u) mx = fmaxf(mx, t[u]);
+        }
+    }
+    mx = block_max(mx, red);
+    float sum = 0.f;
+    if (keep) {
+#pragma unroll
+        for (int j = 0; j < kKeep; ++j)
+            if (vt + j * kSelThreads < n_vocab) sum += expf(v[j] - mx);
+    } else {
+        for (int i = vt; i < n_vocab; i += kSelThreads) sum += expf(x[i] - mx);
+    }
+    sum = wave_sum(sum);
+    float* out = part + (long)row * kNsPartFloats;
+    if (lane == 0) out[4 * q + wave] = sum;
+    if (q == 0 && tid == 0) out[kSelThreads / 64] = mx;
+}
+__device__ __forceinline__ float token_prob_finish(const float* __restrict__ logits, int n_vocab, int token,
+                                                   const float* __restrict__ part, int row) {
+    const float* p = part + (long)row * kNsPartFloats;
+    float w[kNsPartFloats];
+#pragma unroll
+    for (int i = 0; i < kNsPartFloats; ++i) w[i] = p[i];
+    const float xt = logits[(long)row * n_vocab + token];
+    float r = 0.f;
+#pragma unroll
+    for (int i = 0; i < kSelThreads / 64; ++i) r += w[i];
+    return expf(xt - w[kSelThreads / 64]) / r;
+}
+
 __global__ __launch_bounds__(kSelThreads) void token_prob_kernel(const float* __restrict__ logits, int n_vocab,
                                                                  int token, float* __restrict__ probs) {
     token_prob_body(logits, n_vocab, token, probs, blockIdx.x);
@@ -656,16 +723,16 @@
     }
 }
 
-__global__ __launch_bounds__(64) void select_stage2_early_kernel(TopkArgs t, AlignArgs a, int n_blk) {
-    asm volatile("" ::"s"(t.parts), "s"(t.k), "s"(t.top_vals), "s"(t.top_ids), "s"(t.host.result), "s"(t.host.seq), "s"(a.part),
-                 "s"(a.frames));
-    __builtin_amdgcn_sched_barrier(0);
+template <bool NS>
+__device__ __forceinline__ void select_stage2_early_body(const TopkArgs& t, const AlignArgs& a, int n_blk) {
     const int row = blockIdx.x, lane = threadIdx.x;
     unsigned seq = 0;
     if (t.host.result) seq = *t.host.seq;
     const float* slot = a.part + ((long)row * 64 + (lane < n_blk ? lane : 0)) * 2;
     float bv = slot[0];
     int bi = __float_as_int(slot[1]);
+    [[maybe_unused]] float ns = 0.f;
+    if constexpr (NS) ns = token_prob_finish(t.ns_logits, t.n_vocab, t.ns_token, t.ns_part, row);
     if (lane >= n_blk) { bv = -INFINITY; bi = 0x7fffffff; }
     topk_stage2_body(t.parts, t.k, t.top_vals, t.top_ids, row, t.host, seq, false);
     wave_argmax(bv, bi);
@@ -674,11 +741,45 @@
         a.frames[row] = frame;
         if (t.host.result) {
             t.host.result[row].frame = frame;
+            if constexpr (NS) {
+                t.ns_probs[row] = ns;
+                t.host.result[row].no_speech = ns;
+            }
             __threadfence_system();
             __hip_atomic_store(&t.host.result[row].flag_topk, seq, __ATOMIC_RELEASE, __HIP_MEMORY_SCOPE_SYSTEM);
             __hip_atomic_store(&t.host.result[row].flag_align, seq, __ATOMIC_RELEASE, __HIP_MEMORY_SCOPE_SYSTEM);
         }
     }
+}
+
+__global__ __launch_bounds__(64) void select_stage2_early_kernel(TopkArgs t, AlignArgs a, int n_blk) {
+    asm volatile("" ::"s"(t.parts), "s"(t.k), "s"(t.top_vals), "s"(t.top_ids), "s"(t.host.result), "s"(t.host.seq), "s"(a.part),
+                 "s"(a.frames));
+    __builtin_amdgcn_sched_barrier(0);
+    select_stage2_early_body<false>(t, a, n_blk);
+}
+
+__global__ __launch_bounds__(256) void select_stage1_first_kernel(TopkArgs t, AlignArgs a, int n_blk) {
+    WLK_PIN_SELECT_ARGS(t, a);
+    const int n_topk = kSelBlocks * t.n_rows, n_part = n_blk * a.n_beam;
+    if ((int)blockIdx.x < n_topk) {
+        const int n_adj = t.host.n_adj ? *t.host.n_adj : t.n_adj;
+        topk_stage1_body(t.logits, t.n_vocab, t.k, t.parts, t.adj_row, t.adj_ids, t.adj_deltas, n_adj,
+                         blockIdx.x % kSelBlocks, blockIdx.x / kSelBlocks);
+    } else if ((int)blockIdx.x < n_topk + n_part) {
+        const int i = blockIdx.x - n_topk;
+        align_median_part_body(a, i / n_blk, i % n_blk, n_blk);
+    } else {
+        const int i = blockIdx.x - n_topk - n_part;
+        token_prob_part_body(t.ns_logits, t.n_vocab, t.ns_part, i / kNsGroups, i % kNsGroups);
+    }
+}
+
+__global__ __launch_bounds__(64) void select_stage2_first_kernel(TopkArgs t, AlignArgs a, int n_blk) {
+    asm volatile("" ::"s"(t.parts), "s"(t.k), "s"(t.top_vals), "s"(t.top_ids), "s"(t.host.result), "s"(t.host.seq), "s"(a.part),
+                 "s"(a.frames), "s"(t.ns_probs), "s"(t.ns_part), "s"(t.ns_logits), "s"(t.n_vocab), "s"(t.ns_token));
+    __builtin_amdgcn_sched_barrier(0);
+    select_stage2_early_body<true>(t, a, n_blk);
 }
 
 bool select_early_z_enabled() {
@@ -698,7 +799,7 @@
 bool launch_select_fused(const LaunchCtx& ctx, float* logits, int n_vocab, int n_rows, int k, float* top_vals, int* top_ids,
                          void* scratch, const int* adj_row, const int* adj_ids, const float* adj_deltas, int n_adj,
                          const AlignArgs& a, const StepHostOut& host, const float* ns_logits, int ns_token, float* ns_probs,
-                         bool early_z) {
+                         bool early_z, float* ns_part) {
     const size_t lds = (size_t)a.n_align * a.T * sizeof(float);
     if (!select_fused_applicable(n_rows, k, a)) return false;
     static std::atomic<bool> attr_set[64];
@@ -710,19 +811,24 @@
         attr_set[dev].store(true, std::memory_order_release);
     }
     TopkArgs t{logits, n_vocab, k, n_rows, static_cast<SelPartial*>(scratch), adj_row, adj_ids, adj_deltas, n_adj, top_vals, top_ids,
-               host, ns_logits, ns_token, ns_probs};
+               host, ns_logits, ns_token, ns_probs, ns_part};
     const int zf = (a.T + 63) / 64;
     if (early_z) {
         const int n_blk = (a.T + kAlignPartFrames - 1) / kAlignPartFrames;
-        if (ns_logits || !a.part || n_blk > 64) throw std::invalid_argument("select: the early z-score form needs a.part, T <= 16384 and no no-speech block");
+        if (!a.part || n_blk > 64) throw std::invalid_argument("select: the early z-score form needs a.part and T <= 16384");
+        if (ns_logits && (!ns_probs || !ns_part || ns_token < 0 || ns_token >= n_vocab || !host.result))
+            throw std::invalid_argument("select: the early form's no-speech role needs its scratch, a host result and a token in range");
         {
             KernelScope ks(ctx, "sel_stage1", 0.0, 4.0 * 3.0 * n_rows * (double)n_vocab);
-            hipLaunchKernelGGL(select_stage1_early_kernel, dim3(kSelBlocks * n_rows + n_blk * a.n_beam), dim3(256), 0, ctx.stream, t, a, n_blk);
+            const dim3 grid(kSelBlocks * n_rows + n_blk * a.n_beam + (ns_logits ? kNsGroups * n_rows : 0));
+            if (ns_logits) hipLaunchKernelGGL(select_stage1_first_kernel, grid, dim3(256), 0, ctx.stream, t, a, n_blk);
+            else hipLaunchKernelGGL(select_stage1_early_kernel, grid, dim3(256), 0, ctx.stream, t, a, n_blk);
             WLK_HIP(hipGetLastError());
         }
         {
             KernelScope ks(ctx, "sel_stage2");
-            hipLaunchKernelGGL(select_stage2_early_kernel, dim3(n_rows), dim3(64), 0, ctx.stream, t, a, n_blk);
+            if (ns_logits) hipLaunchKernelGGL(select_stage2_first_kernel, dim3(n_rows), dim3(64), 0, ctx.stream, t, a, n_blk);
+            else hipLaunchKernelGGL(select_stage2_early_kernel, dim3(n_rows), dim3(64), 0, ctx.stream, t, a, n_blk);
             WLK_HIP(hipGetLastError());
         }
         return true;
```

Result: faster. 207.2 audio_s/s, median of 5 (+1.6%).
